# JinfengX/PointCloudPDF

Hardware: AMD Instinct MI355X
Metric: points/sec fwd+bwd (PT-v1 Seg50 + PDF U-decoder, 100k-pt scenes) (higher is better)
Workload: dtype f32

## Files before the change

include/pdfops.h:

```cpp
#ifndef PDFOPS_H
#define PDFOPS_H

#ifdef __cplusplus
extern "C" {
#endif

#define PDF_OK 0
#define PDF_ERR_BAD_ARG (-1)
#define PDF_ERR_NSAMPLE (-2)
#define PDF_ERR_UNSUPPORTED (-3)

#define PDF_ABI_VERSION 7
int pdf_abi_version(void);
const char *pdf_build_info(void);
int pdf_dist_fma_mode(void);
#define PDF_MMA_F32 0
#define PDF_MMA_F16 1
#define PDF_MMA_BF16 2

int pdf_knn_query(int m, int nsample, const float *xyz, const float *new_xyz,
                  const int *offset, const int *new_offset, int b,
                  int *idx, float *dist2, void *stream);

long pdf_knn_workspace_bytes(int b, int n, int m);
int pdf_knn_grid_supported(int nsample);
int pdf_knn_query_ws(int m, int nsample, int n, const float *xyz, const float *new_xyz, const int *offset,
                     const int *new_offset, int b, int *idx, float *dist2, void *workspace, long workspace_bytes,
                     void *stream);
int pdf_knn_grid_build(int n, const float *xyz, const int *offset, int b, void *workspace, long workspace_bytes, void *stream);
int pdf_knn_query_grid(int m, int nsample, int n, const float *xyz, const float *new_xyz, const int *offset, const int *new_offset, int b,
                       int *idx, float *dist2, void *workspace, long workspace_bytes, void *stream);
int pdf_knn_query_ws_counted(int m, int nsample, int n, const float *xyz, const float *new_xyz, const int *offset,
                             const int *new_offset, int b, int *idx, float *dist2, void *workspace, long workspace_bytes,
                             unsigned long long *pairs, void *stream);
int pdf_knn_query_list(int m, int nsample, const float *xyz, const float *new_xyz, const int *offset,
                       const int *new_offset, int b, int *idx, float *dist2, const int *qlist, const int *qcount,
                       void *stream);

int pdf_ball_query(int m, int nsample, float min_radius, float max_radius, const float *xyz, const float *new_xyz,
                   const int *offset, const int *new_offset, int b, int *idx, float *dist2, void *stream);

int pdf_random_ball_query(int m, int nsample, float min_radius, float max_radius, const int *order, const float *xyz,
                          const float *new_xyz, const int *offset, const int *new_offset, int b, int *idx, float *dist2,
                          void *stream);

int pdf_farthest_point_sampling(int b, int n, const float *xyz, const int *offset,
                                const int *new_offset, float *tmp, int *idx, void *stream);

int pdf_fps_reference_block_log2(int n);

long pdf_fps_workspace_bytes(int b, int n_total);
long pdf_fps_stats_offset(int b, int n_total);
int pdf_farthest_point_sampling_bucketed(int b, int n, int n_total, const float *xyz, const int *offset,
                                         const int *new_offset, void *workspace, long workspace_bytes,
                                         int *idx, void *stream);

int pdf_grouping_forward(int m, int nsample, int c, const float *input, const int *idx, float *output, void *stream);
int pdf_grouping_backward(int m, int nsample, int c, const float *grad_output, const int *idx, float *grad_input, void *stream);
int pdf_grouping_forward_ordered(int m, int nsample, int c, const float *input, const int *idx, const int *order, float *output, void *stream);
int pdf_group_forward_ordered(int m, int nsample, int c, int with_xyz, const float *feat, const float *xyz, const float *new_xyz,
                              const int *idx, const int *order, float *output, void *stream);
int pdf_interpolation_forward_ordered(int n, int c, int k, const float *input, const int *idx, const float *weight, const int *order,
                                      float *output, void *stream);
int pdf_subtraction_forward_ordered(int n, int nsample, int c, const float *input1, const float *input2, const int *idx, const int *order,
                                    float *output, void *stream);
int pdf_aggregation_forward_ordered(int n, int nsample, int c, int w_c, const float *input, const float *position, const float *weight,
                                    const int *idx, const int *order, float *output, void *stream);

int pdf_interpolation_forward(int n, int c, int k, const float *input, const int *idx, const float *weight, float *output, void *stream);
int pdf_interpolation_backward(int n, int c, int k, const float *grad_output, const int *idx, const float *weight, float *grad_input, void *stream);

int pdf_subtraction_forward(int n, int nsample, int c, const float *input1, const float *input2, const int *idx, float *output, void *stream);
int pdf_subtraction_backward(int n, int nsample, int c, const int *idx, const float *grad_output, float *grad_input1, float *grad_input2, void *stream);

int pdf_aggregation_forward(int n, int nsample, int c, int w_c, const float *input, const float *position,
                            const float *weight, const int *idx, float *output, void *stream);
int pdf_aggregation_backward(int n, int nsample, int c, int w_c, const float *input, const float *position,
                             const float *weight, const int *idx, const float *grad_output,
                             float *grad_input, float *grad_position, float *grad_weight, void *stream);

int pdf_attention_relation_step_forward(int m, int g, int c, const float *query, const float *key, const float *weight,
                                        const int *index_target, const int *index_refer, float *output, void *stream);
int pdf_attention_relation_step_backward(int m, int g, int c, const float *query, float *grad_query,
                                         const float *key, float *grad_key, const float *weight, float *grad_weight,
                                         const int *index_target, const int *index_refer, const float *grad_output, void *stream);
int pdf_attention_fusion_step_forward(int m, int g, int c, const float *weight, const float *value,
                                      const int *index_target, const int *index_refer, float *output, void *stream);
int pdf_attention_fusion_step_backward(int m, int g, int c, const float *weight, float *grad_weight,
                                       const float *value, float *grad_value,
                                       const int *index_target, const int *index_refer, const float *grad_output, void *stream);


int pdf_group_forward(int m, int nsample, int c, int with_xyz, const float *feat, const float *xyz,
                      const float *new_xyz, const int *idx, float *output, void *stream);
int pdf_group_backward(int m, int nsample, int c, int with_xyz, const float *grad_output, const int *idx,
                       float *grad_feat, void *stream);

int pdf_interpolation_weights(int n, int k, const float *dist2, float *weight, void *stream);

int pdf_pt_layer_supported(int nsample, int c);
long pdf_pt_layer_partial_floats(int n, int nsample, int c);
int pdf_pt_layer_forward(int n, int nsample, int c, const float *xq, const float *xk, const float *xv,
                         const float *p, const int *idx, const float *const *weights,
                         const float *const *bn_params, float *const *bn_buffers, int training, float eps,
                         float momentum, float *bn, float *saved, float *H, float *partial, float *out,
                         int storage_bf16, const int *order, void *stream);
int pdf_pt_layer_forward_m(int n, int nsample, int c, const float *xq, const float *xk, const float *xv,
                           const float *p, const int *idx, const float *const *weights,
                           const float *const *bn_params, float *const *bn_buffers, int training, float eps,
                           float momentum, float *bn, float *saved, float *H, float *partial, float *out,
                           int storage_bf16, const int *order, const double *moments, int *out_stat_rows, void *stream);

long pdf_pt_layer_bwd_partial_floats(int n, int nsample, int c);
long pdf_pt_layer_bwd_sums_floats(int c);
int pdf_pt_layer_backward(int n, int nsample, int c, const float *xq, const float *xk, const float *xv,
                          const float *p, const int *idx, const float *const *weights, const float *bn,
                          const float *saved, const float *H, const float *gout, float *gxq, float *gxk,
                          float *gxv, float *G2, float *G3, float *Wsm, float *GR, const int *inv_off, const int *inv_entry,
                          int entry_base, float *partial, float *sums, int storage_bf16, const int *order, const double *moments,
                          void *stream);

int pdf_bn_supported(int c);
long pdf_bn_partial_floats(long n, int c);
int pdf_bn_act_forward(long n, int c, const float *x, const float *res, const float *gamma, const float *beta,
                       float *running_mean, float *running_var, int training, float eps, float momentum, int relu,
                       float *coef, float *partial, float *y, void *stream);
int pdf_bn_act_backward(long n, int c, const float *gy, const float *x, const float *res, const float *coef,
                        int training, int relu, float *partial, float *sums, float *gx, float *gres, void *stream);
int pdf_bn_coef(long n, int c, const float *x, const float *gamma, const float *beta, float *running_mean,
                float *running_var, int training, float eps, float momentum, float *coef, float *partial, void *stream);
int pdf_bn_apply(long n, int c, const float *x, const float *res, const float *coef, int relu, float *y, void *stream);

long pdf_rowlin_partial_floats(long n, int o);
int pdf_rowlin_partial_rows(long n, int k, int o);
int pdf_rowlin_forward(long n, int k, int o, const float *x, long ldx, const float *w, int transpose_w,
                       const float *bias, const float *scale, const float *shift, int relu, float *y, long ldy,
                       int accumulate, float *partial, int mma_input, void *stream);
long pdf_rowlin_wgrad_ws_floats(long n, int k, int o, int ng);
int pdf_rowlin_wgrad(long n, int k, int o, const float *g, long ldg, const float *x, long ldx,
                     const float *scale, const float *shift, int relu, float *dw, float *db, float *ws, int mma_input, void *stream);
int pdf_bn_coef_from_partial(const float *partial, int rows, long n, int c, const float *gamma, const float *beta,
                             float *running_mean, float *running_var, float eps, float momentum, float *coef, void *stream);

int pdf_rowlin_multi(long n, int k, int o, int nin, int nout, const float *const *x, long ldx, const float *const *w,
                     int transpose_w, const float *const *bias, const float *scale, const float *shift, int relu,
                     float *const *y, long ldy, int accumulate, int mma_input, void *stream);
int pdf_rowlin_wgrad_multi(long n, int k, int o, int ng, const float *const *g, long ldg, const float *x, long ldx,
                           const float *scale, const float *shift, int relu, float *const *dw, float *const *db, float *ws, int mma_input, void *stream);
int pdf_rowlin_wgrad_group(long n, int k, int o, int ng, const float *const *g, long ldg, const float *const *x, long ldx,
                           const float *const *scale, const float *const *shift, const int *relu, float *const *dw,
                           float *const *db, float *ws, int mma_input, void *stream);

int pdf_kpconv_supported(int kp, int cin);
int pdf_kpconv_gather(int n, int m, int kp, int cin, const float *query, const float *support, const int *neighbors, const float *x,
                      const float *k_points, float extent, float *weighted, void *stream);
int pdf_kpconv_scatter(int n, int m, int kp, int cin, const float *query, const float *support, const int *neighbors,
                       const float *grad_weighted, const float *k_points, float extent, float *grad_x, void *stream);
int pdf_rowlin_dgrad_bstats(long n, int k, int o, int nin, const float *const *x, long ldx, const float *const *w, float *y, long ldy,
                            const float *bx, long ldb, const float *bcoef, int brelu, float *partial, int *partial_rows,
                            int mma_input, void *stream);
int pdf_rowlin_forward_bn(long n, int k, int o, const float *x, long ldx, const float *w, const float *bias, const float *scale,
                          const float *shift, int relu, float *y, long ldy, float *partial, const float *gamma, const float *beta,
                          float *running_mean, float *running_var, float eps, float momentum, float *coef, int mma_input, void *stream);
int pdf_bn_act_backward_presummed(long n, int c, const float *gy, const float *x, const float *coef, int training, int relu,
                                  const float *partial, int partial_rows, float *sums, float *gx, void *stream);

int pdf_bn_coef_eval_or_partial(const float *partial, int rows, long n, int c, const float *gamma, const float *beta,
                                float *running_mean, float *running_var, int training, float eps, float momentum,
                                float *coef, void *stream);
int pdf_block_pre_forward(long n, int c, void *const *p, int training, float eps, float momentum, int mma_input, void *stream);
int pdf_block_pre_backward(long n, int c, void *const *p, int training, int mma_input, void *stream);
int pdf_block_post_forward(long n, int c, void *const *p, int training, float eps, float momentum, int mma_input, void *stream);
int pdf_block_post_backward(long n, int c, void *const *p, int training, int mma_input, void *stream);
int pdf_bottleneck_forward(long n, int nsample, int c, void *const *p, int training, float eps, float momentum, int storage_bf16, int mma_input, void *stream);
int pdf_bottleneck_backward(long n, int nsample, int c, void *const *p, int training, int entry_base, int storage_bf16, int mma_input, void *stream);
int pdf_linbn_forward(long n, int k, int o, void *const *p, int training, int relu, float eps, float momentum, int mma_input, void *stream);
int pdf_linbn_backward(long n, int k, int o, void *const *p, int training, int relu, int mma_input, void *stream);

int pdf_rowlin_forward_roww(long n, int k, int o, const float *x, long ldx, const float *w, int transpose_w, float *y, long ldy,
                            int accumulate, const float *roww, long rws, int mma_input, void *stream);
int pdf_rowlin_wgrad_roww(long n, int k, int o, const float *g, long ldg, const float *x, long ldx, float *dw, const float *roww,
                          long rws, float *ws, int mma_input, void *stream);
int pdf_bn_bwd_sums(long n, int c, const float *gy, const float *x, const float *coef, int relu, float *partial, float *sums,
                    void *stream);

int pdf_td_supported(int nsample, int cin, int cout);
int pdf_td_tables(long m, int b, const float *p_src, const float *p_new, const int *idx, const int *new_offset, float *rel4, float *Z,
                  float *scene_sums, long n, const int *inv_off, const int *inv_entry, int entry_base,
                  void *stream);
long pdf_td_gram_floats(int cin);
long pdf_td_fwd_scratch_floats(long n, int cin);
long pdf_td_bwd_scratch_floats(long m, int cin, int cout);
int pdf_td_forward(long n, long m, int cin, int cout, void *const *p, int training, float eps, float momentum, int mma_input, void *stream);
int pdf_td_backward(long n, long m, int cin, int cout, void *const *p, int entry_base, int mma_input, void *stream);

int pdf_seg_sum_rows(long n, int c, const float *src, const int *inv_off, const int *inv_entry, int entry_base, float scale, float *out,
                     void *stream);
int pdf_seg_sum_rows_own(long n, int c, int nsample, const float *src, const int *inv_off, const int *inv_entry, int entry_base, float scale,
                         const int *order, float *out, float *out_own, void *stream);
int pdf_seg_sum_rows_strided(long n, int c, const float *src, long src_stride, const int *inv_off, const int *inv_entry, int entry_base,
                             float scale, float *out, void *stream);
int pdf_seg_sum_rows_x(long n, int c, const float *src, long src_stride, int src_bf16, const int *inv_off, const int *inv_entry, int entry_base,
                       float scale, float *out, void *stream);
int pdf_seg_sum_weighted_x(long n, int c, int nsample, int w_c, const float *src, const float *w, int w_bf16, const int *inv_off,
                           const int *inv_entry, int entry_base, const int *order, float *out, void *stream);
int pdf_seg_sum_weighted_ordered(long n, int c, int nsample, int w_c, const float *src, const float *w, const int *inv_off,
                                 const int *inv_entry, int entry_base, const int *order, float *out, void *stream);
int pdf_seg_sum_weighted(long n, int c, int nsample, int w_c, const float *src, const float *w, const int *inv_off, const int *inv_entry,
                         int entry_base, float *out, void *stream);

long pdf_ce_workspace_floats(void);
int pdf_ce_forward(long n, int c, const float *logits, const long *target, long ignore, float *grad, float *acc, float *loss,
                   void *stream);
int pdf_ce_backward(long n, int c, const float *dlogits, const float *acc, const float *gy, float *grad_out, void *stream);

long pdf_incr_kl_workspace_floats(void);
int pdf_incr_kl_forward(long n, int cs, int ct, const float *student, const float *teacher, const long *labels, long ignore, float inv_tp,
                        float inv_tt, float *grad, float *acc, float *loss, void *stream);
int pdf_incr_kl_backward(long n, int cs, const float *dgrad, const float *acc, const float *gy, float *grad_out, void *stream);

long pdf_knn_rel_moments_ws_doubles(int b, long m);
int pdf_knn_rel_moments(int b, long n, int nsample, const float *xyz, const int *offset, const int *idx, double *out, double *ws, void *stream);
int pdf_knn_rel_moments_q(int b, long m, int nsample, const float *xyz, const float *new_xyz, const int *new_offset, const int *idx,
                          double *out, double *ws, void *stream);

int pdf_scene_morton_keys(long n, int b, const float *xyz, const int *offset, float *bounds, long long *keys, void *stream);

int pdf_sgd_chunk(void);
int pdf_sgd_step(int nchunks, const void *tab, const int *chunks, float lr, float momentum, float weight_decay, const float *found_inf,
                 void *stream);
int pdf_grad_unscale(int nchunks, const void *tab, const int *chunks, const float *inv_scale, float *found_inf, void *stream);
int pdf_scaler_update(float *scale, float *inv_scale, int *growth_tracker, float *found_inf, float growth_factor, float backoff_factor,
                      int growth_interval, void *stream);
int pdf_adam_step(int nchunks, int ntensors, const void *tab, const int *chunks, double lr, double beta1, double beta2, double eps,
                  double weight_decay, int decoupled, const float *found_inf, void *stream);
int pdf_adam_grad_unscale(int nchunks, const void *tab, const int *chunks, const float *inv_scale, float *found_inf, void *stream);

int pdf_attention_step1_forward_v2(int N, int M, int h, int C, unsigned n_max, const float *q, const float *k,
                                   const int *index0_offsets, const int *index1, float *attn, void *stream);
int pdf_attention_step1_backward_v2(int N, int M, int h, int C, unsigned n_max, const float *grad_out, const int *index0_offsets,
                                    const int *index1, const float *q, const float *k, float *grad_q, float *grad_k, void *stream);
int pdf_dot_prod_with_idx_forward_v3(int N, int M, int h, int hdim, unsigned n_max, const float *q, const int *index_q_offsets,
                                     const float *k, const int *index_k, const float *table_q, const float *table_k,
                                     const int *rel_idx, float *output, void *stream);
int pdf_dot_prod_with_idx_backward_v3(int N, int M, int h, int hdim, unsigned n_max, const float *grad_out, const float *q,
                                      const int *index_q_offsets, const float *k, const int *index_k, const float *table_q,
                                      const float *table_k, const int *rel_idx, float *grad_q, float *grad_k, float *grad_table_q,
                                      float *grad_table_k, void *stream);
int pdf_attention_step2_with_rel_pos_value_forward_v2(int N, int M, int h, int hdim, unsigned n_max, const float *attn, const float *v,
                                                      const int *index0_offsets, const int *index1, const float *table,
                                                      const int *rel_idx, float *output, void *stream);
int pdf_attention_step2_with_rel_pos_value_backward_v2(int N, int M, int h, int hdim, unsigned n_max, const float *grad_out,
                                                       const int *index0_offsets, const int *index1, const float *attn, const float *v,
                                                       const float *table, const int *rel_idx, float *grad_attn, float *grad_v,
                                                       float *grad_table, void *stream);

int pdf_dot_prod_with_idx_forward_v3_l(int N, int M, int h, int hdim, int L, const float *q, const int *index_q_offsets, const float *k,
                                       const int *index_k, const float *table_q, const float *table_k, const int *rel_idx, float *output,
                                       void *stream);
int pdf_dot_prod_with_idx_backward_v3_l(int N, int M, int h, int hdim, int L, const float *grad_out, const float *q,
                                        const int *index_q_offsets, const float *k, const int *index_k, const float *table_q,
                                        const float *table_k, const int *rel_idx, float *grad_q, float *grad_k, float *grad_table_q,
                                        float *grad_table_k, void *stream);
int pdf_attention_step2_with_rel_pos_value_backward_v2_l(int N, int M, int h, int hdim, int L, const float *grad_out,
                                                         const int *index0_offsets, const int *index1, const float *attn, const float *v,
                                                         const float *table, const int *rel_idx, float *grad_attn, float *grad_v,
                                                         float *grad_table, void *stream);

int pdf_grid_hash(long n, int b, const float *coord, const int *offset, double gx, double gy, double gz, int f32,
                  const long long *min_grid, long long *grid, unsigned long long *key, void *stream);
int pdf_grid_hash_f64(long n, int b, const double *coord, const int *offset, double gx, double gy, double gz,
                      const long long *min_grid, long long *grid, unsigned long long *key, void *stream);

int pdf_philox4x64(long n, long key0, long key1, long ctr0, unsigned long long *out, void *stream);
int pdf_aug_bounds_workspace_doubles(int b);
int pdf_aug_bounds(int b, const long long *offset, const double *coord, const double *color, double *part, double *bounds, void *stream);
int pdf_aug_points(int b, long n, const long long *offset, int nop, const double *table, const double *bounds, const double *rec,
                   double *coord, double *color, double *normal, void *stream);
int pdf_aug_keys(int b, long n, const long long *offset, const unsigned long long *scene_keys, long stream_id, unsigned long long *out,
                 void *stream);
int pdf_aug_elastic_noise(int b, long total, const long long *vinfo, const unsigned long long *scene_keys, long stream_id, float *vol,
                          void *stream);
int pdf_aug_elastic_blur(int b, long total, const long long *vinfo, const float *in, float *out, int axis, void *stream);
int pdf_aug_elastic_apply(int b, long n, const long long *offset, const long long *vinfo, const double *axes, const float *vol,
                          const double *params, double magnitude, double *coord, double *disp, void *stream);

int pdf_vote_accumulate(long n, int c, const float *logits, const float *score, const long *index, float *pred,
                        float *score_sum, float *score_cnt, void *stream);

int pdf_radius_neighbors_self(int n, int nsample, float radius, const float *xyz, const int *offset, int b, int *idx, float *dist2,
                              void *workspace, long workspace_bytes, void *stream);

long pdf_graph_forest_workspace_bytes(long n, long E, long n_nodes);
int pdf_graph_forest(long n, int E, const long long *u, const long long *v, const float *w, const unsigned char *active,
                     const long long *nodes, int n_nodes, int *comp, unsigned char *chosen, void *workspace, long workspace_bytes,
                     void *stream);

int pdf_gmm2_1d(int m, const float *sorted_x, double *resp, double *out, int iters, double tol, double reg, void *stream);

int pdf_segment_softmax_forward(int N, int M, int h, const int *index0_offsets, const float *x, float *y, void *stream);
int pdf_segment_softmax_backward(int N, int M, int h, const int *index0_offsets, const float *y, const float *grad_y, float *grad_x,
                                 void *stream);

int pdf_wa_segment_rows(int N, int h, int d, int L, const int *seg_off, const int *seg_edge, const int *other, const int *rel,
                        const float *w, const float *X, long ldx, float xscale, const float *table, float *out, long ldo, float oscale, void *stream);
int pdf_wa_segment_rows_ordered(int N, int h, int d, int L, const int *seg_off, const int *seg_edge, const int *other, const int *rel,
                                const float *w, const float *X, long ldx, float xscale, const float *table, float *out, long ldo, float oscale,
                                const int *order, void *stream);
long pdf_wa_table_grad_ws_floats(int N, int h, int L);
int pdf_wa_table_grad(int N, int h, int d, int L, const int *seg_off, const int *seg_edge, const int *rel, const float *w,
                      const float *x, long ldx, float xscale, float *ws, float *grad_table, void *stream);
int pdf_wa_grad_attn(int N, int M, int h, int d, int L, const float *grad_out, long ldg, const int *offsets, const int *index1, const float *v,
                     long ldv, const float *table, const int *rel, float *grad_attn, void *stream);
int pdf_wa_logits_forward(int N, int M, int h, int d, int L, const float *q, const float *k, long ld, float qscale, const int *offsets,
                          const int *index1, const float *table_q, const float *table_k, const int *rel, float *out, void *stream);
int pdf_wa_permute_edges(int M, int h, const float *src, const int *edge, float *dst, void *stream);
int pdf_wa_logits_forward_ordered(int N, int M, int h, int d, int L, const float *q, const float *k, long ld, float qscale, const int *offsets,
                                  const int *index1, const float *table_q, const float *table_k, const int *rel, float *out, const int *order,
// ... 65 lines not shown
```

pointcloudpdf_amd/_native.py:

```python
import ctypes
import os
import threading

import torch

_HERE = os.path.dirname(os.path.abspath(__file__))
DIST_FMA = int(os.environ.get("PDFOPS_DIST_FMA", "0") or 0)
if DIST_FMA not in (0, 1, 2):
    raise RuntimeError(f"PDFOPS_DIST_FMA={DIST_FMA}: expected 0 (as written), 1 or 2 (csrc/pdfops_common.h)")


def library_path(dist_fma=0):
    return os.path.join(_HERE, "lib", "libpdfops.so" if not dist_fma else f"libpdfops_fma{int(dist_fma)}.so")


LIB_PATH = library_path(DIST_FMA)
ABI_VERSION = 7

c_int = ctypes.c_int
c_long = ctypes.c_long
c_void_p = ctypes.c_void_p
c_float = ctypes.c_float
c_double = ctypes.c_double

_PROTOS = {
    "knn_query": "iippppipp",
    "ball_query": "iiffppppipp",
    "random_ball_query": "iiffpppppipp",
    "farthest_point_sampling": "iippppp",
    "grouping_forward": "iiippp",
    "grouping_backward": "iiippp",
    "interpolation_forward": "iiipppp",
    "interpolation_backward": "iiipppp",
    "subtraction_forward": "iiipppp",
    "subtraction_backward": "iiipppp",
    "aggregation_forward": "iiiippppp",
    "aggregation_backward": "iiiipppppppp",
    "attention_relation_step_forward": "iiipppppp",
    "attention_relation_step_backward": "iiippppppppp",
    "attention_fusion_step_forward": "iiippppp",
    "attention_fusion_step_backward": "iiippppppp",
    "attention_step1_forward_v2": "iiiiippppp",
    "attention_step1_backward_v2": "iiiiippppppp",
    "dot_prod_with_idx_forward_v3": "iiiiipppppppp",
    "dot_prod_with_idx_backward_v3": "iiiiipppppppppppp",
    "attention_step2_with_rel_pos_value_forward_v2": "iiiiippppppp",
    "attention_step2_with_rel_pos_value_backward_v2": "iiiiipppppppppp",
    "segment_softmax_forward": "iiippp",
    "segment_softmax_backward": "iiipppp",
}
_HIP_ONLY_PROTOS = {
    "grid_hash": "lippdddippp",
    "grid_hash_f64": "lippdddppp",
    "philox4x64": "llllp",
    "aug_bounds": "ippppp",
    "aug_points": "ilpipppppp",
    "aug_keys": "ilpplp",
    "aug_elastic_noise": "ilpplp",
    "aug_elastic_blur": "ilpppi",
    "aug_elastic_apply": "ilpppppdpp",
    "radius_neighbors_self": "iifppipppl",
    "vote_accumulate": "lipppppp",
    "graph_forest": "lipppppipppl",
    "gmm2_1d": "ipppidd",
    "dot_prod_with_idx_forward_v3_l": "iiiiipppppppp",
    "dot_prod_with_idx_backward_v3_l": "iiiiipppppppppppp",
    "attention_step2_with_rel_pos_value_backward_v2_l": "iiiiipppppppppp",
    "scene_sum_rows": "ipiplip",
    "scene_repeat_rows": "iplipip",
    "region_stats": "ippppifppp",
    "region_seeds": "ippppip",
    "region_grow": "ippipppipiipppp",
    "region_edges": "ipppppippppppppppppl",
    "sort_floats_dev": "ipppppp",
    "gmm2_weak_dev": "ippppppppidd",
    "region_mask": "ippppppp",
    "region_tree": "ippipppppppp",
    "graph_forest_dev": "lipppppippppl",
    "gmm2_1d_dev": "ippppidd",
    "graph_forest_batch_dev": "ippippppppipppl",
    "wa_segment_rows": "iiiipppppplfpplf",
    "wa_segment_rows_ordered": "iiiipppppplfpplfp",
    "wa_table_grad": "iiiippppplfpp",
    "wa_grad_attn": "iiiiiplppplppp",
    "wa_logits_forward": "iiiiipplfpppppp",
    "wa_permute_edges": "iippp",
    "wa_logits_forward_ordered": "iiiiipplfppppppp",
    "wa_grad_attn_ordered": "iiiiiplppplpppp",
    "window_keys": "ippippfippp",
    "window_edges_count": "ippipppppp",
    "window_edges_fill": "ipppppppffipppp",
    "group_forward": "iiiippppp",
    "group_backward": "iiiippp",
    "interpolation_weights": "iipp",
    "farthest_point_sampling_bucketed": "iiipppplp",
    "grouping_forward_ordered": "iiipppp",
    "group_forward_ordered": "iiiipppppp",
    "interpolation_forward_ordered": "iiippppp",
    "subtraction_forward_ordered": "iiippppp",
    "aggregation_forward_ordered": "iiiipppppp",
    "seg_sum_rows": "lipppifp",
    "seg_sum_rows_strided": "liplppifp",
    "seg_sum_rows_own": "liipppifppp",
    "seg_sum_weighted": "liiippppip",
    "seg_sum_weighted_ordered": "liiippppipp",
}
_KIND = {"i": c_int, "l": c_long, "f": c_float, "d": c_double, "p": c_void_p}


class PdfOpsError(RuntimeError):
    pass


_RAW_STREAM = getattr(torch._C, "_cuda_getCurrentRawStream", None) if os.environ.get("PDFOPS_RAW_STREAM", "1") != "0" else None


def raw_stream():
    dev = torch.cuda.current_device()
    return _RAW_STREAM(dev) if _RAW_STREAM is not None else torch.cuda.current_stream().cuda_stream


def cu_masked_stream(first_cu, n_cus, device=None):
    if first_cu % 8 or n_cus % 8 or n_cus < 8:
        raise PdfOpsError("cu_masked_stream: first_cu and n_cus must be multiples of 8 (one CU of every XCD per step of 8)")
    dev = torch.cuda.current_device() if device is None else torch.device(device).index
    total = torch.cuda.get_device_properties(dev).multi_processor_count
    if first_cu + n_cus > total:
        raise PdfOpsError(f"cu_masked_stream: CUs [{first_cu}, {first_cu + n_cus}) of {total}")
    hip = ctypes.CDLL("libamdhip64.so")
    words = (total + 31) // 32
    mask = (ctypes.c_uint32 * words)()
    for cu in range(first_cu, first_cu + n_cus):
        mask[cu // 32] |= 1 << (cu % 32)
    handle = ctypes.c_void_p()
    with torch.cuda.device(dev):
        rc = hip.hipExtStreamCreateWithCUMask(ctypes.byref(handle), ctypes.c_uint32(words), mask)
    if rc != 0:
        raise PdfOpsError(f"hipExtStreamCreateWithCUMask failed with status {rc}")
    return torch.cuda.ExternalStream(handle.value, device=torch.device("cuda", dev))


def require_current_device(*tensors):
    cur = None
    for t in tensors:
        if t is None or not t.is_cuda:
            continue
        if cur is None:
            cur = torch.cuda.current_device()
        if t.device.index != cur:
            raise PdfOpsError(f"pointcloudpdf_amd: tensor on {t.device} but the current device is cuda:{cur}; call "
                              "torch.cuda.set_device(...) or wrap the call in torch.cuda.device(...)")


_INV = "_pdf_inverse"


def attach_inverse(idx, n, table):
    setattr(idx, _INV, (idx.data_ptr(), idx._version, int(n), table))
    return table


def inverse_table(idx, n):
    cached = getattr(idx, _INV, None)
    if cached is not None and cached[0] == idx.data_ptr() and cached[1] == idx._version and cached[2] == int(n):
        return cached[3]
    flat = idx.reshape(-1)
    vals, perm = torch.sort(flat, stable=True)
    off = torch.searchsorted(vals, torch.arange(int(n) + 1, device=idx.device, dtype=vals.dtype), out_int32=True)
    return attach_inverse(idx, n, (off, perm.to(torch.int32), 0))

# ... 349 lines not shown

    def attention_step2_with_rel_pos_value_v2_backward(self, grad_out, attn, v, offsets, n_max, index1, table, rel_idx):
        _check(grad_out, torch.float32, "grad_output")
        m, h = attn.shape
        n, _, d = v.shape
        ga = self._new(v, (m, h), torch.float32, zero=True)
        gv = self._new(v, (n, h, d), torch.float32, zero=True)
        gt = self._new(v, tuple(table.shape), torch.float32, zero=True)
        name, x = (("attention_step2_with_rel_pos_value_backward_v2_l", int(table.shape[0])) if self.use_stream
                   else ("attention_step2_with_rel_pos_value_backward_v2", int(n_max)))
        self._call(name, n, m, h, d, x, grad_out, offsets, index1, attn, v, table, rel_idx, ga, gv, gt)
        return ga, gv, gt


    def segment_softmax(self, x, offsets):
        _check(x, torch.float32, "src"); _check(offsets, torch.int32, "index0_offsets")
        m, h = x.shape
        if h > 64:
            raise ValueError("segment_softmax: at most 64 heads")
        y = self._new(x, (m, h), torch.float32)
        self._call("segment_softmax_forward", offsets.shape[0] - 1, m, h, offsets, x, y)
        return y

    def segment_softmax_backward(self, y, grad_y, offsets):
        _check(grad_y, torch.float32, "grad_output")
        m, h = y.shape
        gx = self._new(y, (m, h), torch.float32)
        self._call("segment_softmax_backward", offsets.shape[0] - 1, m, h, offsets, y, grad_y, gx)
        return gx


class HipBackend(CBackend):

    overwrites_outputs = True

    def __init__(self, lib):
        super().__init__(lib, "pdf_", "cuda", True, extra_protos=tuple(_HIP_ONLY_PROTOS))
        lib.pdf_fps_workspace_bytes.restype = c_long
        lib.pdf_fps_workspace_bytes.argtypes = [c_int, c_int]
        lib.pdf_wa_table_grad_ws_floats.restype = c_long
        lib.pdf_wa_table_grad_ws_floats.argtypes = [c_int, c_int, c_int]
        lib.pdf_layernorm_supported.restype = c_int
        lib.pdf_layernorm_supported.argtypes = [c_int]
        lib.pdf_layernorm_partial_floats.restype = c_long
        lib.pdf_layernorm_partial_floats.argtypes = [c_long, c_int]
        lib.pdf_layernorm_forward.restype = c_int
        lib.pdf_layernorm_forward.argtypes = [c_long, c_int, c_void_p, c_void_p, c_void_p, ctypes.c_float, c_void_p, c_void_p, c_void_p, c_void_p]
        lib.pdf_layernorm_backward.restype = c_int
        lib.pdf_layernorm_backward.argtypes = [c_long, c_int] + [c_void_p] * 10
        lib.pdf_fps_stats_offset.restype = c_long
        lib.pdf_fps_stats_offset.argtypes = [c_int, c_int]
        self.collect_fps_stats = False
        self.last_fps_stats = None
        lib.pdf_aug_bounds_workspace_doubles.restype = c_int
        lib.pdf_aug_bounds_workspace_doubles.argtypes = [c_int]
        lib.pdf_abi_version.restype = c_int
        lib.pdf_build_info.restype = ctypes.c_char_p
        got = int(lib.pdf_abi_version())
        if got != ABI_VERSION:
            raise PdfOpsError(f"libpdfops ABI {got} != {ABI_VERSION} expected by pointcloudpdf_amd/_native.py (include/pdfops.h: PDF_ABI_VERSION): "
                              "stale library -- rebuild with `python -m pointcloudpdf_amd.build --force`")
        for nm in ("pre_forward", "post_forward"):
            f = getattr(lib, "pdf_block_" + nm)
            f.restype = c_int
            f.argtypes = [c_long, c_int, c_void_p, c_int, ctypes.c_float, ctypes.c_float, c_int, c_void_p]
        lib.pdf_td_tables.restype = c_int
        lib.pdf_td_tables.argtypes = [c_long, c_int, c_void_p, c_void_p, c_void_p, c_void_p, c_void_p, c_void_p, c_void_p, c_long, c_void_p, c_void_p,
                                      c_int, c_void_p]
        lib.pdf_td_supported.restype = c_int
        lib.pdf_td_supported.argtypes = [c_int, c_int, c_int]
        lib.pdf_td_gram_floats.restype = c_long
        lib.pdf_td_gram_floats.argtypes = [c_int]
        lib.pdf_td_fwd_scratch_floats.restype = c_long
        lib.pdf_td_fwd_scratch_floats.argtypes = [c_long, c_int]
        lib.pdf_td_bwd_scratch_floats.restype = c_long
        lib.pdf_td_bwd_scratch_floats.argtypes = [c_long, c_int, c_int]
        lib.pdf_td_forward.restype = c_int
        lib.pdf_td_forward.argtypes = [c_long, c_long, c_int, c_int, c_void_p, c_int, ctypes.c_float, ctypes.c_float, c_int, c_void_p]
        lib.pdf_td_backward.restype = c_int
        lib.pdf_td_backward.argtypes = [c_long, c_long, c_int, c_int, c_void_p, c_int, c_int, c_void_p]
        lib.pdf_ce_workspace_floats.restype = c_long
        lib.pdf_ce_workspace_floats.argtypes = []
        lib.pdf_ce_forward.restype = c_int
        lib.pdf_ce_forward.argtypes = [c_long, c_int, c_void_p, c_void_p, c_long, c_void_p, c_void_p, c_void_p, c_void_p]
        lib.pdf_ce_backward.restype = c_int
        lib.pdf_ce_backward.argtypes = [c_long, c_int, c_void_p, c_void_p, c_void_p, c_void_p, c_void_p]
        lib.pdf_incr_kl_workspace_floats.restype = c_long
        lib.pdf_incr_kl_workspace_floats.argtypes = []
        lib.pdf_incr_kl_forward.restype = c_int
        lib.pdf_incr_kl_forward.argtypes = [c_long, c_int, c_int, c_void_p, c_void_p, c_void_p, c_long, ctypes.c_float, ctypes.c_float,
                                            c_void_p, c_void_p, c_void_p, c_void_p]
        lib.pdf_incr_kl_backward.restype = c_int
        lib.pdf_incr_kl_backward.argtypes = [c_long, c_int, c_void_p, c_void_p, c_void_p, c_void_p, c_void_p]
        lib.pdf_knn_rel_moments.restype = c_int
        lib.pdf_knn_rel_moments.argtypes = [c_int, c_long, c_int, c_void_p, c_void_p, c_void_p, c_void_p, c_void_p, c_void_p]
        lib.pdf_knn_rel_moments_ws_doubles.restype = c_long
        lib.pdf_knn_rel_moments_ws_doubles.argtypes = [c_int, c_long]
        lib.pdf_knn_rel_moments_q.restype = c_int
        lib.pdf_knn_rel_moments_q.argtypes = [c_int, c_long, c_int, c_void_p, c_void_p, c_void_p, c_void_p, c_void_p, c_void_p, c_void_p]
        class CopySeg(ctypes.Structure):
            _fields_ = [("src", c_void_p), ("dst", c_void_p), ("nbytes", c_long), ("src_offset", c_void_p), ("sub", c_void_p),
                        ("sub_const", c_int), ("src_elems", c_int)]

        self.CopySeg = CopySeg
        lib.pdf_stage_copy.restype = c_int
        lib.pdf_stage_copy.argtypes = [c_int, c_void_p, c_void_p]
        lib.pdf_scene_morton_keys.restype = c_int
        lib.pdf_scene_morton_keys.argtypes = [c_long, c_int, c_void_p, c_void_p, c_void_p, c_void_p, c_void_p]
        lib.pdf_sgd_chunk.restype = c_int
        lib.pdf_sgd_chunk.argtypes = []
        lib.pdf_sgd_step.restype = c_int
        lib.pdf_sgd_step.argtypes = [c_int, c_void_p, c_void_p, ctypes.c_float, ctypes.c_float, ctypes.c_float, c_void_p, c_void_p]
        lib.pdf_grad_unscale.restype = c_int
        lib.pdf_grad_unscale.argtypes = [c_int, c_void_p, c_void_p, c_void_p, c_void_p, c_void_p]
        lib.pdf_scaler_update.restype = c_int
        lib.pdf_scaler_update.argtypes = [c_void_p, c_void_p, c_void_p, c_void_p, ctypes.c_float, ctypes.c_float, c_int, c_void_p]
        lib.pdf_adam_step.restype = c_int
        lib.pdf_adam_step.argtypes = [c_int, c_int, c_void_p, c_void_p, ctypes.c_double, ctypes.c_double, ctypes.c_double, ctypes.c_double,
                                      ctypes.c_double, c_int, c_void_p, c_void_p]
        lib.pdf_adam_grad_unscale.restype = c_int
        lib.pdf_adam_grad_unscale.argtypes = [c_int, c_void_p, c_void_p, c_void_p, c_void_p, c_void_p]
        lib.pdf_linbn_forward.restype = c_int
        lib.pdf_linbn_forward.argtypes = [c_long, c_int, c_int, c_void_p, c_int, c_int, ctypes.c_float, ctypes.c_float, c_int, c_void_p]
        lib.pdf_linbn_backward.restype = c_int
        lib.pdf_linbn_backward.argtypes = [c_long, c_int, c_int, c_void_p, c_int, c_int, c_int, c_void_p]
        lib.pdf_bottleneck_forward.restype = c_int
        lib.pdf_bottleneck_forward.argtypes = [c_long, c_int, c_int, c_void_p, c_int, ctypes.c_float, ctypes.c_float, c_int, c_int, c_void_p]
        lib.pdf_bottleneck_backward.restype = c_int
        lib.pdf_bottleneck_backward.argtypes = [c_long, c_int, c_int, c_void_p, c_int, c_int, c_int, c_int, c_void_p]
        for nm in ("pre_backward", "post_backward"):
            f = getattr(lib, "pdf_block_" + nm)
            f.restype = c_int
            f.argtypes = [c_long, c_int, c_void_p, c_int, c_int, c_void_p]
        lib.pdf_rowlin_multi.restype = c_int
        lib.pdf_rowlin_multi.argtypes = [c_long, c_int, c_int, c_int, c_int, c_void_p, c_long, c_void_p, c_int, c_void_p, c_void_p, c_void_p,
                                         c_int, c_void_p, c_long, c_int, c_int, c_void_p]
        lib.pdf_kpconv_supported.restype = c_int
        lib.pdf_kpconv_supported.argtypes = [c_int, c_int]
        for nm in ("pdf_kpconv_gather", "pdf_kpconv_scatter"):
            f = getattr(lib, nm)
            f.restype = c_int
            f.argtypes = [c_int, c_int, c_int, c_int, c_void_p, c_void_p, c_void_p, c_void_p, c_void_p, ctypes.c_float, c_void_p, c_void_p]
        lib.pdf_rowlin_wgrad_group.restype = c_int
        lib.pdf_rowlin_wgrad_group.argtypes = [c_long, c_int, c_int, c_int, c_void_p, c_long, c_void_p, c_long, c_void_p, c_void_p, c_void_p,
                                               c_void_p, c_void_p, c_void_p, c_int, c_void_p]
        lib.pdf_rowlin_wgrad_multi.restype = c_int
        lib.pdf_rowlin_wgrad_multi.argtypes = [c_long, c_int, c_int, c_int, c_void_p, c_long, c_void_p, c_long, c_void_p, c_void_p, c_int,
                                               c_void_p, c_void_p, c_void_p, c_int, c_void_p]
        lib.pdf_rowlin_wgrad_ws_floats.restype = c_long
        lib.pdf_rowlin_wgrad_ws_floats.argtypes = [c_long, c_int, c_int, c_int]
        lib.pdf_rowlin_dgrad_bstats.restype = c_int
        lib.pdf_rowlin_dgrad_bstats.argtypes = [c_long, c_int, c_int, c_int, c_void_p, c_long, c_void_p, c_void_p, c_long, c_void_p, c_long,
                                                c_void_p, c_int, c_void_p, ctypes.POINTER(c_int), c_int, c_void_p]
        lib.pdf_bn_act_backward_presummed.restype = c_int
        lib.pdf_bn_act_backward_presummed.argtypes = [c_long, c_int, c_void_p, c_void_p, c_void_p, c_int, c_int, c_void_p, c_int, c_void_p,
                                                      c_void_p, c_void_p]
        lib.pdf_rowlin_partial_floats.restype = c_long
        lib.pdf_rowlin_partial_floats.argtypes = [c_long, c_int]
        lib.pdf_rowlin_partial_rows.restype = c_int
        lib.pdf_rowlin_partial_rows.argtypes = [c_long, c_int, c_int]
        lib.pdf_rowlin_forward.restype = c_int
        lib.pdf_rowlin_forward.argtypes = [c_long, c_int, c_int, c_void_p, c_long, c_void_p, c_int, c_void_p, c_void_p, c_void_p,
                                           c_int, c_void_p, c_long, c_int, c_void_p, c_int, c_void_p]
        lib.pdf_rowlin_wgrad.restype = c_int
        lib.pdf_rowlin_wgrad.argtypes = [c_long, c_int, c_int, c_void_p, c_long, c_void_p, c_long, c_void_p, c_void_p, c_int,
                                         c_void_p, c_void_p, c_void_p, c_int, c_void_p]
        lib.pdf_bn_coef_from_partial.restype = c_int
        lib.pdf_bn_coef_from_partial.argtypes = [c_void_p, c_int, c_long, c_int, c_void_p, c_void_p, c_void_p, c_void_p,
                                                 ctypes.c_float, ctypes.c_float, c_void_p, c_void_p]
        lib.pdf_bn_coef.restype = c_int
        lib.pdf_bn_coef.argtypes = [c_long, c_int, c_void_p, c_void_p, c_void_p, c_void_p, c_void_p, c_int, ctypes.c_float,
                                    ctypes.c_float, c_void_p, c_void_p, c_void_p]
        lib.pdf_bn_apply.restype = c_int
        lib.pdf_bn_apply.argtypes = [c_long, c_int, c_void_p, c_void_p, c_void_p, c_int, c_void_p, c_void_p]
        lib.pdf_bn_supported.restype = c_int
        lib.pdf_bn_supported.argtypes = [c_int]
        lib.pdf_bn_partial_floats.restype = c_long
        lib.pdf_bn_partial_floats.argtypes = [c_long, c_int]
        lib.pdf_bn_act_forward.restype = c_int
        lib.pdf_bn_act_forward.argtypes = [c_long, c_int] + [c_void_p] * 6 + [c_int, ctypes.c_float, ctypes.c_float, c_int] + [c_void_p] * 4
        lib.pdf_bn_act_backward.restype = c_int
        lib.pdf_bn_act_backward.argtypes = [c_long, c_int] + [c_void_p] * 4 + [c_int, c_int] + [c_void_p] * 5
        lib.pdf_pt_layer_supported.restype = c_int
        lib.pdf_pt_layer_supported.argtypes = [c_int, c_int]
        for fn in (lib.pdf_pt_layer_partial_floats, lib.pdf_pt_layer_bwd_partial_floats):
            fn.restype = c_long
            fn.argtypes = [c_int, c_int, c_int]
        lib.pdf_pt_layer_bwd_sums_floats.restype = c_long
        lib.pdf_pt_layer_bwd_sums_floats.argtypes = [c_int]
        lib.pdf_pt_layer_forward.restype = c_int
        lib.pdf_pt_layer_forward.argtypes = [c_int, c_int, c_int] + [c_void_p] * 8 + [c_int, ctypes.c_float, ctypes.c_float] + [c_void_p] * 5 + [c_int, c_void_p, c_void_p]
        lib.pdf_knn_grid_build.restype = c_int
        lib.pdf_knn_grid_build.argtypes = [c_int, c_void_p, c_void_p, c_int, c_void_p, c_long, c_void_p]
        lib.pdf_knn_query_grid.restype = c_int
        lib.pdf_knn_query_grid.argtypes = [c_int, c_int, c_int, c_void_p, c_void_p, c_void_p, c_void_p, c_int, c_void_p, c_void_p, c_void_p, c_long, c_void_p]
        lib.pdf_pt_layer_backward.restype = c_int
        lib.pdf_pt_layer_backward.argtypes = [c_int, c_int, c_int] + [c_void_p] * 19 + [c_int] + [c_void_p] * 2 + [c_int, c_void_p, c_void_p, c_void_p]
        self.fps_mode = os.environ.get("PDFOPS_FPS", "bucketed")
        self.knn_mode = os.environ.get("PDFOPS_KNN", "grid")
        lib.pdf_knn_workspace_bytes.restype = c_long
        lib.pdf_knn_workspace_bytes.argtypes = [c_int, c_int, c_int]
        lib.pdf_graph_forest_workspace_bytes.restype = c_long
        lib.pdf_region_grow_list_points.restype = c_long
        lib.pdf_region_grow_list_points.argtypes = []
        lib.pdf_graph_forest_workspace_bytes.argtypes = [c_long, c_long, c_long]
        lib.pdf_knn_grid_supported.restype = c_int
        lib.pdf_knn_grid_supported.argtypes = [c_int]
        lib.pdf_knn_query_ws.restype = c_int
        lib.pdf_knn_query_ws.argtypes = [c_int, c_int, c_int] + [c_void_p] * 4 + [c_int] + [c_void_p] * 3 + [c_long, c_void_p]
        lib.pdf_knn_query_ws_counted.restype = c_int
        lib.pdf_knn_query_ws_counted.argtypes = [c_int, c_int, c_int] + [c_void_p] * 4 + [c_int] + [c_void_p] * 3 + [c_long, c_void_p, c_void_p]

    KNN_GRID_MAX_SCENES = 64
    use_inverse = os.environ.get("PDFOPS_INVERSE", "1") != "0"
    storage_bf16 = os.environ.get("PDFOPS_STORAGE", "f32") == "bf16"

    def set_storage(self, kind):
        if kind not in ("f32", "bf16"):
            raise ValueError("storage: 'f32' or 'bf16'")
        self.storage_bf16 = kind == "bf16"

    def grouping_forward(self, input, idx):
        _check(input, torch.float32, "input"); _check(idx, torch.int32, "idx")
        m, ns = idx.shape
        c = input.shape[1]
        out = self._new(input, (m, ns, c), torch.float32)
        self._call("grouping_forward_ordered", m, ns, c, input, idx, order_of(idx), out)
        return out

    def interpolation_forward(self, input, idx, weight):
        _check(input, torch.float32, "input"); _check(idx, torch.int32, "idx"); _check(weight, torch.float32, "weight")
        n, k = idx.shape
        c = input.shape[1]
        out = self._new(input, (n, c), torch.float32)
        self._call("interpolation_forward_ordered", n, c, k, input, idx, weight, order_of(idx), out)
        return out

    def subtraction_forward(self, input1, input2, idx):
        _check(input1, torch.float32, "input1"); _check(input2, torch.float32, "input2"); _check(idx, torch.int32, "idx")
        n, c = input1.shape
        ns = idx.shape[-1]
        out = self._new(input1, (n, ns, c), torch.float32)
        self._call("subtraction_forward_ordered", n, ns, c, input1, input2, idx, order_of(idx), out)
        return out

    def aggregation_forward(self, input, position, weight, idx):
        for t, nm in ((input, "input"), (position, "position"), (weight, "weight")):
            _check(t, torch.float32, nm)
        _check(idx, torch.int32, "idx")
        n, ns, c = position.shape
        out = self._new(input, (n, c), torch.float32)
        self._call("aggregation_forward_ordered", n, ns, c, weight.shape[-1], input, position, weight, idx, order_of(idx), out)
        return out

    def grouping_backward(self, grad_output, idx, n):
        if not self.use_inverse:
            return super().grouping_backward(grad_output, idx, n)
        _check(grad_output, torch.float32, "grad_output"); _check(idx, torch.int32, "idx")
        m, ns, c = grad_output.shape
        if grad_output.numel() == 0 or n == 0:
            return self._new(grad_output, (n, c), torch.float32, zero=True)
        off, ent, base = inverse_table(idx, n)
        gi = self._new(grad_output, (n, c), torch.float32)
        self._call("seg_sum_rows", n, c, grad_output, off, ent, base, 1.0, gi)
        return gi

    def interpolation_backward(self, grad_output, idx, weight, m):
        if not self.use_inverse:
            return super().interpolation_backward(grad_output, idx, weight, m)
        _check(grad_output, torch.float32, "grad_output"); _check(idx, torch.int32, "idx"); _check(weight, torch.float32, "weight")
        n, c = grad_output.shape
        if grad_output.numel() == 0 or m == 0:
            return self._new(grad_output, (m, c), torch.float32, zero=True)
        off, ent, base = inverse_table(idx, m)
        gi = self._new(grad_output, (m, c), torch.float32)
        self._call("seg_sum_weighted_ordered", m, c, idx.shape[1], 1, grad_output, weight, off, ent, base, src_order_of(idx, m), gi)
        return gi

    def subtraction_backward(self, idx, grad_output, n2=None):
        if not self.use_inverse:
            return super().subtraction_backward(idx, grad_output, n2)
        _check(grad_output, torch.float32, "grad_output"); _check(idx, torch.int32, "idx")
        n, ns, c = grad_output.shape
        n2 = n if n2 is None else n2
        if grad_output.numel() == 0 or n2 == 0:
            return super().subtraction_backward(idx, grad_output, n2)
        off, ent, base = inverse_table(idx, n2)
        g2 = self._new(grad_output, (n2, c), torch.float32)
        if n == n2 and c % 4 == 0 and self.fuse_own_rows:
            g1 = self._new(grad_output, (n, c), torch.float32)
            self._call("seg_sum_rows_own", n2, c, ns, grad_output, off, ent, base, -1.0, src_order_of(idx, n2), g2, g1)
            return g1, g2
        g1 = self._new(grad_output, (n, c), torch.float32, zero=True)
        self._call("subtraction_backward", n, ns, c, idx, grad_output, g1, None)
        self._call("seg_sum_rows", n2, c, grad_output, off, ent, base, -1.0, g2)
        return g1, g2

    fuse_own_rows = os.environ.get("PDFOPS_FUSE_OWN_ROWS", "1") != "0"

    def aggregation_backward(self, input, position, weight, idx, grad_output):
        if not self.use_inverse:
            return super().aggregation_backward(input, position, weight, idx, grad_output)
        _check(grad_output, torch.float32, "grad_output")
        n, ns, c = position.shape
        w_c = weight.shape[-1]
        if position.numel() == 0 or input.shape[0] == 0:
# ... 284 lines not shown
        count = torch.empty(n, **i32)
        seg = torch.empty((n, 4), **i32)
        self._call("window_edges_count", n, kf_sorted, kf, m, kcd_sorted, kc, wk, wkd, count, seg)
        offsets = torch.zeros(n + 1, **i32)
        torch.cumsum(count, 0, dtype=torch.int32, out=offsets[1:])
        e, n_max = (int(v) for v in torch.stack([offsets[-1], count.max() if n else offsets[-1]]).tolist())
        index0 = torch.empty(e, dtype=torch.int64, device=dev)
        index1 = torch.empty(e, **i32)
        rel = torch.empty((e, 3), **i32)
        flag = torch.zeros(1, **i32)
        order32 = order_f.int()
        self._call("window_edges_fill", n, offsets, seg, order32, order_cd.int(), wk, wkd, xyz.contiguous(), float(c2w), float(qs), int(vmax),
                   index0, index1, rel, flag)
        setattr(offsets, _WORDER, (offsets.data_ptr(), offsets._version, order32))
        return index0, index1, offsets, n_max, rel, flag

    def window_logits_supported(self, q, k, table_q):
        return self.wa_atomic_free and q.shape[0] == k.shape[0] and self._wa_ok(q.shape[2], int(table_q.shape[0]), q, k)

    def window_logits(self, q, k, index1, offsets, table_q, table_k, rel_idx):
        n, h, d = q.shape
        m = index1.shape[0]
        out = torch.empty((m, h), dtype=torch.float32, device=q.device)
        self._call("wa_logits_forward", n, m, h, d, int(table_q.shape[0]), q, k, h * d, 1.0, offsets, index1, table_q, table_k, rel_idx, out)
        return out

    def window_logits_backward(self, g, q, k, index1, offsets, table_q, table_k, rel_idx):
        n, h, d = q.shape
        L = int(table_q.shape[0])
        key_off, key_edge, key_q, key_rel = window_csc(index1, offsets, rel_idx, n_keys=n)
        g_key = self._wa_permute(g, key_edge)
        gq, gk = torch.empty_like(q), torch.empty_like(k)
        self._wa_rows(n, h, d, L, offsets, None, index1, rel_idx, g, k, table_q, gq)
        self._wa_rows(n, h, d, L, key_off, None, key_q, key_rel, g_key, q, table_k, gk)
        gtq = self._wa_table_grad(n, h, d, L, offsets, None, rel_idx, g, q, q)
        gtk = self._wa_table_grad(n, h, d, L, key_off, None, key_rel, g_key, k, q)
        return gq, gk, gtq, gtk

    def attention_step2_with_rel_pos_value_v2_backward(self, grad_out, attn, v, offsets, n_max, index1, table, rel_idx):
        m, h = attn.shape
        n, _, d = v.shape
        L = int(table.shape[0])
        if m == 0 or offsets.shape[0] != n + 1 or not self._wa_ok(d, L, v, grad_out):
            return super().attention_step2_with_rel_pos_value_v2_backward(grad_out, attn, v, offsets, n_max, index1, table, rel_idx)
        _check(grad_out, torch.float32, "grad_output")
        c = h * d
        key_off, key_edge, key_q = window_csc(index1, offsets, n_keys=n)
        ga = torch.empty((m, h), dtype=torch.float32, device=v.device)
        gv = torch.empty_like(v)
        self._call("wa_grad_attn", n, m, h, d, L, grad_out, c, offsets, index1, v, c, table, rel_idx, ga)
        self._wa_rows(n, h, d, 0, key_off, key_edge, key_q, None, attn, grad_out, None, gv)
        gt = self._wa_table_grad(n, h, d, L, offsets, None, rel_idx, attn, grad_out, v)
        return ga, gv, gt

    wa_core = os.environ.get("PDFOPS_WA_CORE", "1") != "0"

    def window_attention_core_supported(self, qkv, table_q, table_k, table_v):
        L, h, d, _ = table_q.shape
        return (self.wa_core and self.wa_atomic_free and qkv.dim() == 2 and qkv.shape[1] == 3 * h * d and table_k.shape == table_q.shape == table_v.shape
                and qkv.dtype == torch.float32 and qkv.is_contiguous() and self._wa_ok(d, L, qkv) and (h * d) % 4 == 0)

    def window_attention_core(self, qkv, index1, offsets, table_q, table_k, table_v, rel_idx, scale):
        n = qkv.shape[0]
        L, h, d, _ = table_q.shape
        c, m = h * d, index1.shape[0]
        q, k, v = qkv[:, :c], qkv[:, c:2 * c], qkv[:, 2 * c:]
        logits = torch.empty((m, h), dtype=torch.float32, device=qkv.device)
        self._call("wa_logits_forward_ordered", n, m, h, d, L, q, k, 3 * c, float(scale), offsets, index1, table_q, table_k, rel_idx, logits,
                   self._wa_order(offsets))
        attn = self.segment_softmax(logits, offsets)
        out = torch.empty((n, c), dtype=torch.float32, device=qkv.device)
        self._wa_rows(n, h, d, L, offsets, None, index1, rel_idx, attn, v, table_v, out, ldx=3 * c, order=self._wa_order(offsets))
        return out, attn

    def window_attention_core_backward(self, go, qkv, attn, index1, offsets, table_q, table_k, table_v, rel_idx, scale):
        n = qkv.shape[0]
        L, h, d, _ = table_q.shape
        c, m = h * d, index1.shape[0]
        q, k, v = qkv[:, :c], qkv[:, c:2 * c], qkv[:, 2 * c:]
        key_off, key_edge, key_q, key_rel = window_csc(index1, offsets, rel_idx, n_keys=n)
        gqkv = torch.empty_like(qkv)
        ga = torch.empty((m, h), dtype=torch.float32, device=qkv.device)
        order = self._wa_order(offsets)
        self._call("wa_grad_attn_ordered", n, m, h, d, L, go, c, offsets, index1, v, 3 * c, table_v, rel_idx, ga, order)
        attn_key = self._wa_permute(attn, key_edge)
        korder = window_key_order(index1) if self.wa_window_order else None
        self._wa_rows(n, h, d, 0, key_off, None, key_q, None, attn_key, go, None, gqkv[:, 2 * c:], ldo=3 * c, order=korder)
        gtv = self._wa_table_grad(n, h, d, L, offsets, None, rel_idx, attn, go, qkv)
        g = self.segment_softmax_backward(attn, ga, offsets)
        g_key = self._wa_permute(g, key_edge)
        self._wa_rows(n, h, d, L, offsets, None, index1, rel_idx, g, k, table_q, gqkv[:, :c], ldx=3 * c, ldo=3 * c, oscale=scale, order=order)
        self._wa_rows(n, h, d, L, key_off, None, key_q, key_rel, g_key, q, table_k, gqkv[:, c:2 * c], ldx=3 * c, xscale=scale, ldo=3 * c, order=korder)
        gtq = self._wa_table_grad(n, h, d, L, offsets, None, rel_idx, g, q, qkv, ldx=3 * c, xscale=scale)
        gtk = self._wa_table_grad(n, h, d, L, key_off, None, key_rel, g_key, k, qkv, ldx=3 * c)
        return gqkv, gtq, gtk, gtv

    def _stream(self):
        return c_void_p(raw_stream())

    def rowlin(self, x, w, bias=None, coef=None, relu=False, transpose_w=False, out=None, accumulate=False, stats=False):
        n, k = x.shape
        o = w.shape[1] if transpose_w else w.shape[0]
        y = out if out is not None else torch.empty((n, o), dtype=torch.float32, device=x.device)
        partial = None
        if stats:
            partial = torch.empty((int(self.lib.pdf_rowlin_partial_floats(n, o)),), dtype=torch.float32, device=x.device)
            partial._pdf_rows = int(self.lib.pdf_rowlin_partial_rows(n, k, o))
        rc = self.lib.pdf_rowlin_forward(n, k, o, x.data_ptr(), x.stride(0), w.data_ptr(), int(transpose_w),
                                         None if bias is None else bias.data_ptr(),
                                         None if coef is None else coef.data_ptr(),
                                         None if coef is None else coef.data_ptr() + 4 * k, int(relu), y.data_ptr(), y.stride(0),
                                         int(accumulate), None if partial is None else partial.data_ptr(), current_mma_input(), self._stream())
        if rc != 0:
            raise PdfOpsError(f"pdf_rowlin_forward failed with status {rc}")
        return y, partial

    @staticmethod
    def _ptrs(tensors, n=3):
        return (c_void_p * n)(*[t.data_ptr() if t is not None else None for t in list(tensors) + [None] * (n - len(tensors))])

    def rowlin_multi(self, xs, ws, biases=None, coef=None, relu=False, transpose_w=False, nout=1):
        n, k = xs[0].shape
        o = ws[0].shape[1] if transpose_w else ws[0].shape[0]
        ys = [torch.empty((n, o), dtype=torch.float32, device=xs[0].device) for _ in range(nout)]
        rc = self.lib.pdf_rowlin_multi(n, k, o, len(xs), nout, self._ptrs(xs), xs[0].stride(0), self._ptrs(ws), int(transpose_w),
                                       None if biases is None else self._ptrs(biases),
                                       None if coef is None else coef.data_ptr(), None if coef is None else coef.data_ptr() + 4 * k,
                                       int(relu), self._ptrs(ys), o, 0, current_mma_input(), self._stream())
        if rc != 0:
            raise PdfOpsError(f"pdf_rowlin_multi failed with status {rc}")
        return ys

    def rowlin_dgrad_bn_backward(self, gs, ws, bx, coef, training=True, relu=True):
        n, k = gs[0].shape
        o = ws[0].shape[1]
        require_current_device(bx, *gs)
        dy = self._new(bx, (n, o), torch.float32)
        partial = self._new(bx, (int(self.lib.pdf_rowlin_partial_floats(n, o)),), torch.float32)
        rows = c_int(0)
        sums = self._new(bx, (2 * o,), torch.float32)
        rc = self.lib.pdf_rowlin_dgrad_bstats(n, k, o, len(gs), self._ptrs(gs), gs[0].stride(0), self._ptrs(ws), dy.data_ptr(), o,
                                              bx.data_ptr(), bx.stride(0), coef.data_ptr(), int(bool(relu)), partial.data_ptr(),
                                              ctypes.byref(rows), current_mma_input(), self._stream())
        if rc == -3:
            return None
        if rc != 0:
            raise PdfOpsError(f"pdf_rowlin_dgrad_bstats failed with status {rc}")
        rc = self.lib.pdf_bn_act_backward_presummed(n, o, dy.data_ptr(), bx.data_ptr(), coef.data_ptr(), int(bool(training)), int(bool(relu)),
                                                    partial.data_ptr(), rows.value, sums.data_ptr(), dy.data_ptr(), self._stream())
        if rc != 0:
            raise PdfOpsError(f"pdf_bn_act_backward_presummed failed with status {rc}")
        return dy, sums[o:], sums[:o]

    def wgrad_workspace(self, n, k, o, ng, device):
        return torch.empty((max(int(self.lib.pdf_rowlin_wgrad_ws_floats(int(n), int(k), int(o), int(ng))), 1),), dtype=torch.float32, device=device)

    def rowlin_wgrad_multi(self, gs, x, coef, relu):
        n, o = gs[0].shape
        k = x.shape[1]
        dws = [torch.empty((o, k), dtype=torch.float32, device=x.device) for _ in gs]
        dbs = [torch.empty((o,), dtype=torch.float32, device=x.device) for _ in gs]
        ws = self.wgrad_workspace(n, k, o, len(gs), x.device)
        rc = self.lib.pdf_rowlin_wgrad_multi(n, k, o, len(gs), self._ptrs(gs), gs[0].stride(0), x.data_ptr(), x.stride(0),
                                             None if coef is None else coef.data_ptr(), None if coef is None else coef.data_ptr() + 4 * k,
                                             int(relu), self._ptrs(dws), self._ptrs(dbs), ws.data_ptr(), current_mma_input(), self._stream())
        if rc != 0:
            raise PdfOpsError(f"pdf_rowlin_wgrad_multi failed with status {rc}")
        return dws, dbs

    def kpconv_supported(self, kp, cin):
        return bool(self.lib.pdf_kpconv_supported(int(kp), int(cin)))

    def kpconv_gather(self, query, support, neighbors, x, k_points, extent):
        n, m = neighbors.shape
        kp, cin = k_points.shape[0], x.shape[1]
        out = torch.empty((n, kp * cin), dtype=torch.float32, device=x.device)
        rc = self.lib.pdf_kpconv_gather(n, m, kp, cin, query.data_ptr(), support.data_ptr(), neighbors.data_ptr(), x.data_ptr(),
                                        k_points.data_ptr(), ctypes.c_float(extent), out.data_ptr(), self._stream())
        if rc != 0:
            raise PdfOpsError(f"pdf_kpconv_gather failed with status {rc}")
        return out

    def kpconv_scatter(self, query, support, neighbors, grad_weighted, k_points, extent, rows, cin):
        n, m = neighbors.shape
        gx = torch.zeros((rows, cin), dtype=torch.float32, device=grad_weighted.device)
        rc = self.lib.pdf_kpconv_scatter(n, m, k_points.shape[0], cin, query.data_ptr(), support.data_ptr(), neighbors.data_ptr(),
                                         grad_weighted.data_ptr(), k_points.data_ptr(), ctypes.c_float(extent), gx.data_ptr(), self._stream())
        if rc != 0:
            raise PdfOpsError(f"pdf_kpconv_scatter failed with status {rc}")
        return gx

    def rowlin_wgrad_group(self, gs, xs, coefs, relus, need_bias):
        n, o = gs[0].shape
        k = xs[0].shape[1]
        dev = gs[0].device
        dws = [torch.empty((o, k), dtype=torch.float32, device=dev) for _ in gs]
        dbs = [torch.empty((o,), dtype=torch.float32, device=dev) if nb else None for nb in need_bias]
        ws = self.wgrad_workspace(n, k, o, len(gs), dev)
        P = lambda ts: (c_void_p * len(ts))(*[None if t is None else (t if isinstance(t, int) else t.data_ptr()) for t in ts])
        sc = [None if cf is None else cf.data_ptr() for cf in coefs]
        sh = [None if cf is None else cf.data_ptr() + 4 * k for cf in coefs]
        rc = self.lib.pdf_rowlin_wgrad_group(n, k, o, len(gs), P(gs), gs[0].stride(0), P(xs), xs[0].stride(0), P(sc), P(sh),
                                             (c_int * len(gs))(*[int(bool(r)) for r in relus]), P(dws), P(dbs), ws.data_ptr(), current_mma_input(), self._stream())
        if rc == -3:
            return None
        if rc != 0:
            raise PdfOpsError(f"pdf_rowlin_wgrad_group failed with status {rc}")
        return dws, dbs

    def rowlin_wgrad(self, g, x, coef, relu, need_bias):
        n, o = g.shape
        k = x.shape[1]
        dw = torch.empty((o, k), dtype=torch.float32, device=x.device)
        db = torch.empty((o,), dtype=torch.float32, device=x.device) if need_bias else None
        ws = self.wgrad_workspace(n, k, o, 1, x.device)
        rc = self.lib.pdf_rowlin_wgrad(n, k, o, g.data_ptr(), g.stride(0), x.data_ptr(), x.stride(0),
                                       None if coef is None else coef.data_ptr(),
                                       None if coef is None else coef.data_ptr() + 4 * k, int(relu), dw.data_ptr(),
                                       None if db is None else db.data_ptr(), ws.data_ptr(), current_mma_input(), self._stream())
        if rc != 0:
            raise PdfOpsError(f"pdf_rowlin_wgrad failed with status {rc}")
        return dw, db

    def bn_coef_from_partial(self, partial, n, c, bn, training):
        coef = torch.empty((4 * c,), dtype=torch.float32, device=partial.device if partial is not None else bn.weight.device)
        if training:
            rows = partial._pdf_rows
            rc = self.lib.pdf_bn_coef_from_partial(partial.data_ptr(), rows, n, c, bn.weight.data_ptr(), bn.bias.data_ptr(),
                                                   bn.running_mean.data_ptr(), bn.running_var.data_ptr(), ctypes.c_float(bn.eps),
                                                   ctypes.c_float(bn.momentum),
                                                   coef.data_ptr(), self._stream())
            if rc != 0:
                raise PdfOpsError(f"pdf_bn_coef_from_partial failed with status {rc}")
        else:
            rstd = torch.rsqrt(bn.running_var + bn.eps)
            sc = bn.weight.detach() * rstd
            coef = torch.cat([sc, bn.bias.detach() - bn.running_mean * sc, bn.running_mean, rstd])
        return coef

    def bn_coef(self, x, bn, training):
        n, c = x.shape
        coef = torch.empty((4 * c,), dtype=torch.float32, device=x.device)
        partial = torch.empty((int(self.lib.pdf_bn_partial_floats(n, c)),), dtype=torch.float32, device=x.device) if training else None
        rc = self.lib.pdf_bn_coef(n, c, x.data_ptr(), bn.weight.data_ptr(), bn.bias.data_ptr(), bn.running_mean.data_ptr(),
                                  bn.running_var.data_ptr(), int(bool(training)), ctypes.c_float(bn.eps),
                                  ctypes.c_float(bn.momentum), coef.data_ptr(),
                                  None if partial is None else partial.data_ptr(), self._stream())
        if rc != 0:
            raise PdfOpsError(f"pdf_bn_coef failed with status {rc}")
        return coef

    def bn_apply(self, x, res, coef, relu):
        n, c = x.shape
        y = torch.empty_like(x)
        rc = self.lib.pdf_bn_apply(n, c, x.data_ptr(), None if res is None else res.data_ptr(), coef.data_ptr(), int(relu),
                                   y.data_ptr(), self._stream())
        if rc != 0:
            raise PdfOpsError(f"pdf_bn_apply failed with status {rc}")
        return y

    def td_tables(self, p_src, p_new, idx, new_offset, inverse=None):
        m, n, b = p_new.shape[0], p_src.shape[0], new_offset.shape[0]
        rel4 = torch.empty((m, 16, 4), dtype=torch.float32, device=p_src.device)
        Z = torch.zeros((n, 32), dtype=torch.float32, device=p_src.device)
        sums = torch.zeros((b, 16), dtype=torch.float32, device=p_src.device)
        off, ent, base = inverse if inverse is not None else (None, None, 0)
        rc = self.lib.pdf_td_tables(m, b, p_src.data_ptr(), p_new.data_ptr(), idx.data_ptr(), new_offset.data_ptr(), rel4.data_ptr(), Z.data_ptr(),
                                    sums.data_ptr(), n, None if off is None else off.data_ptr(), None if ent is None else ent.data_ptr(), int(base),
                                    self._stream())
        if rc != 0:
            raise PdfOpsError(f"pdf_td_tables failed with status {rc}")
        return rel4, Z, sums

    def bottleneck_forward(self, n, k, c, ptrs, training, eps, momentum, storage_bf16=0):
        rc = self.lib.pdf_bottleneck_forward(n, k, c, (c_void_p * len(ptrs))(*ptrs), int(training), ctypes.c_float(eps),
                                             ctypes.c_float(momentum), self.layer_flags(storage_bf16), current_mma_input(), self._stream())
        if rc != 0:
            raise PdfOpsError(f"pdf_bottleneck_forward failed with status {rc}")

    def bottleneck_backward(self, n, k, c, ptrs, training, entry_base=0, storage_bf16=0):
        rc = self.lib.pdf_bottleneck_backward(n, k, c, (c_void_p * len(ptrs))(*ptrs), int(training), int(entry_base), self.layer_flags(storage_bf16), current_mma_input(), self._stream())
        if rc != 0:
            raise PdfOpsError(f"pdf_bottleneck_backward failed with status {rc}")

    def _ptable(self, tensors):
        return (c_void_p * len(tensors))(*[None if t is None else t.data_ptr() for t in tensors])

    def block_call(self, name, n, c, tensors, training, eps=None, momentum=None):
        fn = getattr(self.lib, "pdf_block_" + name)
        if eps is None:
            rc = fn(n, c, self._ptable(tensors), int(bool(training)), current_mma_input(), self._stream())
        else:
            rc = fn(n, c, self._ptable(tensors), int(bool(training)), ctypes.c_float(eps), ctypes.c_float(momentum), current_mma_input(), self._stream())
        if rc != 0:
            raise PdfOpsError(f"pdf_block_{name} failed with status {rc}")

    def bn_supported(self, c):
        return bool(self.lib.pdf_bn_supported(int(c)))

    def bn_act_forward(self, x, res, gamma, beta, running_mean, running_var, training, eps, momentum, relu):
        n, c = x.shape
        require_current_device(x, res, gamma)
        coef = self._new(x, (4 * c,), torch.float32)
        partial = self._new(x, (int(self.lib.pdf_bn_partial_floats(n, c)),), torch.float32)
        y = self._new(x, (n, c), torch.float32)
        P = lambda t: None if t is None else self._ptr(t)
# ... 278 lines not shown
```

pointcloudpdf_amd/csrc/block.hip:

```cpp
#include "pdfops_common.h"

namespace {
struct Err {
    int rc = 0;
    Err &operator<<(int r) { if (rc == 0 && r != 0) rc = r; return *this; }
};

}

extern "C" int pdf_bn_coef_eval_or_partial(const float *partial, int rows, long n, int c, const float *gamma, const float *beta,
                                           float *running_mean, float *running_var, int training, float eps, float momentum,
                                           float *coef, void *stream) {
    if (training) return pdf_bn_coef_from_partial(partial, rows, n, c, gamma, beta, running_mean, running_var, eps, momentum, coef, stream);
    return pdf_bn_coef(n, c, nullptr, gamma, beta, running_mean, running_var, 0, eps, momentum, coef, nullptr, stream);
}

extern "C" int pdf_block_pre_forward(long n, int c, void *const *p, int training, float eps, float momentum, int mma_input, void *stream) {
    if (n < 1 || !p) return PDF_ERR_BAD_ARG;
    if (!pdf_bn_supported(c)) return PDF_ERR_UNSUPPORTED;
    const float *x = (const float *)p[0], *W1 = (const float *)p[1], *g1 = (const float *)p[2], *b1 = (const float *)p[3];
    float *rm1 = (float *)p[4], *rv1 = (float *)p[5];
    float *z1 = (float *)p[12], *coef1 = (float *)p[13], *partial = (float *)p[17];
    Err e;
    if (training) {
        e << pdf_rowlin_forward_bn(n, c, c, x, c, W1, nullptr, nullptr, nullptr, 0, z1, c, partial, g1, b1, rm1, rv1, eps, momentum, coef1, mma_input, stream);
    } else {
        e << pdf_rowlin_forward(n, c, c, x, c, W1, 0, nullptr, nullptr, nullptr, 0, z1, c, 0, nullptr, mma_input, stream);
        e << pdf_bn_coef_eval_or_partial(partial, 0, n, c, g1, b1, rm1, rv1, 0, eps, momentum, coef1, stream);
    }
    const float *xs[1] = {z1}, *ws[3] = {(const float *)p[6], (const float *)p[8], (const float *)p[10]};
    const float *bs[3] = {(const float *)p[7], (const float *)p[9], (const float *)p[11]};
    float *ys[3] = {(float *)p[14], (float *)p[15], (float *)p[16]};
    e << pdf_rowlin_multi(n, c, c, 1, 3, xs, c, ws, 0, bs, coef1, coef1 + c, 1, ys, c, 0, mma_input, stream);
    return e.rc;
}

static bool inkernel_bn() {
    static const bool on = [] { const char *v = getenv("PDFOPS_INKERNEL_BN"); return !(v && v[0] == '0'); }();
    return on;
}
static bool dgrad_bstats() {
    static const bool on = [] { const char *v = getenv("PDFOPS_DGRAD_BSTATS"); return !(v && v[0] == '0'); }();
    return on;
}

static int block_pre_backward(long n, int c, void *const *p, int training, int accumulate_gx, int mma_input, void *stream, bool defer_wgrad = false) {
    if (n < 1 || !p || !p[14]) return PDF_ERR_BAD_ARG;
    const float *x = (const float *)p[0], *z1 = (const float *)p[1], *coef1 = (const float *)p[2], *W1 = (const float *)p[3];
    float *gx = (float *)p[10], *grads = (float *)p[11], *dy = (float *)p[12], *partial = (float *)p[13], *wslab = (float *)p[14];
    const long cc = (long)c * c;
    float *dW1 = grads, *db1 = grads + cc, *dqkv = db1 + 2 * c;
    Err e;
    const float *gs[3] = {(const float *)p[7], (const float *)p[8], (const float *)p[9]};
    const float *ws[3] = {(const float *)p[4], (const float *)p[5], (const float *)p[6]};
    float *dws[3] = {dqkv, dqkv + (cc + c), dqkv + 2 * (cc + c)}, *dbs[3] = {dqkv + cc, dqkv + (cc + c) + cc, dqkv + 2 * (cc + c) + cc};
    float *ys[1] = {dy};
    if (!defer_wgrad) e << pdf_rowlin_wgrad_multi(n, c, c, 3, gs, c, z1, c, coef1, coef1 + c, 1, dws, dbs, wslab, mma_input, stream);
    int prow = 0;
    const int rc1 = dgrad_bstats() ? pdf_rowlin_dgrad_bstats(n, c, c, 3, gs, c, ws, dy, c, z1, c, coef1, 1, partial, &prow, mma_input, stream) : PDF_ERR_UNSUPPORTED;
    if (rc1 == PDF_ERR_UNSUPPORTED) {
        e << pdf_rowlin_multi(n, c, c, 3, 1, gs, c, ws, 1, nullptr, nullptr, nullptr, 0, ys, c, 0, mma_input, stream);
        e << pdf_bn_act_backward(n, c, dy, z1, nullptr, coef1, training, 1, partial, db1, dy, nullptr, stream);
    } else {
        e << rc1;
        e << pdf_bn_act_backward_presummed(n, c, dy, z1, coef1, training, 1, partial, prow, db1, dy, stream);
    }
    if (!defer_wgrad) e << pdf_rowlin_wgrad(n, c, c, dy, c, x, c, nullptr, nullptr, 0, dW1, nullptr, wslab, mma_input, stream);
    e << pdf_rowlin_forward(n, c, c, dy, c, W1, 1, nullptr, nullptr, nullptr, 0, gx, c, accumulate_gx, nullptr, mma_input, stream);
    return e.rc;
}

extern "C" int pdf_block_pre_backward(long n, int c, void *const *p, int training, int mma_input, void *stream) {
    return block_pre_backward(n, c, p, training, 0, mma_input, stream, false);
}

static int block_post_forward(long n, int c, void *const *p, int training, float eps, float momentum, int t_stat_rows, int mma_input, void *stream) {
    if (n < 1 || !p) return PDF_ERR_BAD_ARG;
    if (!pdf_bn_supported(c)) return PDF_ERR_UNSUPPORTED;
    const float *t = (const float *)p[0], *x = (const float *)p[1];
    float *coef2 = (float *)p[11], *z3 = (float *)p[12], *coef3 = (float *)p[13], *y = (float *)p[14], *partial = (float *)p[15];
    Err e;
    if (training && t_stat_rows > 0)
        e << pdf_bn_coef_from_partial(partial, t_stat_rows, n, c, (const float *)p[2], (const float *)p[3], (float *)p[4], (float *)p[5], eps, momentum, coef2, stream);
    else
        e << pdf_bn_coef(n, c, t, (const float *)p[2], (const float *)p[3], (float *)p[4], (float *)p[5], training, eps, momentum, coef2, partial, stream);
    bool applied = false;
    if (training && inkernel_bn()) {
        int rows = 0;
        const int rc = pdf_rowlin_forward_stats_ho(n, c, c, t, c, (const float *)p[6], nullptr, coef2, coef2 + c, 1, z3, c, partial + PDF_HO_FLOATS, partial,
                                                   &rows, mma_input, stream);
        if (rc == PDF_OK) {
            e << pdf_bn_apply_rows(n, c, z3, x, partial + PDF_HO_FLOATS, rows, (const float *)p[7], (const float *)p[8], (float *)p[9], (float *)p[10], eps,
                                   momentum, coef3, partial, 1, y, stream);
            applied = true;
        } else if (rc != PDF_ERR_UNSUPPORTED) {
            e << rc;
        }
    }
    if (applied) return e.rc;
    if (training) {
        e << pdf_rowlin_forward_bn(n, c, c, t, c, (const float *)p[6], nullptr, coef2, coef2 + c, 1, z3, c, partial, (const float *)p[7], (const float *)p[8],
                                   (float *)p[9], (float *)p[10], eps, momentum, coef3, mma_input, stream);
    } else {
        e << pdf_rowlin_forward(n, c, c, t, c, (const float *)p[6], 0, nullptr, coef2, coef2 + c, 1, z3, c, 0, nullptr, mma_input, stream);
        e << pdf_bn_coef_eval_or_partial(partial, 0, n, c, (const float *)p[7], (const float *)p[8], (float *)p[9], (float *)p[10], 0, eps, momentum, coef3, stream);
    }
    e << pdf_bn_apply(n, c, z3, x, coef3, 1, y, stream);
    return e.rc;
}
extern "C" int pdf_block_post_forward(long n, int c, void *const *p, int training, float eps, float momentum, int mma_input, void *stream) {
    return block_post_forward(n, c, p, training, eps, momentum, 0, mma_input, stream);
}

static int block_post_backward(long n, int c, void *const *p, int training, int mma_input, void *stream, bool defer_wgrad = false) {
    if (n < 1 || !p || !p[12]) return PDF_ERR_BAD_ARG;
    const float *gy = (const float *)p[0], *t = (const float *)p[1], *x = (const float *)p[2], *z3 = (const float *)p[3];
    const float *coef2 = (const float *)p[4], *coef3 = (const float *)p[5], *W3 = (const float *)p[6];
    float *gt = (float *)p[7], *gres = (float *)p[8], *grads = (float *)p[9], *da = (float *)p[10], *partial = (float *)p[11];
    const long cc = (long)c * c;
    float *dW3 = grads, *db2 = grads + cc, *db3 = db2 + 2 * c;
    Err e;
    e << pdf_bn_act_backward(n, c, gy, z3, x, coef3, training, 1, partial, db3, da, gres, stream);
    if (!defer_wgrad) e << pdf_rowlin_wgrad(n, c, c, da, c, t, c, coef2, coef2 + c, 1, dW3, nullptr, (float *)p[12], mma_input, stream);
    int prow = 0;
    const float *das[1] = {da}, *w3s[1] = {W3};
    const int rc2 = dgrad_bstats() ? pdf_rowlin_dgrad_bstats(n, c, c, 1, das, c, w3s, gt, c, t, c, coef2, 1, partial, &prow, mma_input, stream) : PDF_ERR_UNSUPPORTED;
    if (rc2 == PDF_ERR_UNSUPPORTED) {
        e << pdf_rowlin_forward(n, c, c, da, c, W3, 1, nullptr, nullptr, nullptr, 0, gt, c, 0, nullptr, mma_input, stream);
        e << pdf_bn_act_backward(n, c, gt, t, nullptr, coef2, training, 1, partial, db2, gt, nullptr, stream);
    } else {
        e << rc2;
        e << pdf_bn_act_backward_presummed(n, c, gt, t, coef2, training, 1, partial, prow, db2, gt, stream);
    }
    return e.rc;
}

extern "C" int pdf_block_post_backward(long n, int c, void *const *p, int training, int mma_input, void *stream) {
    return block_post_backward(n, c, p, training, mma_input, stream, false);
}

extern "C" int pdf_bottleneck_forward(long n, int nsample, int c, void *const *p, int training, float eps, float momentum, int storage_bf16, int mma_input, void *stream) {
    if (n < 1 || !p) return PDF_ERR_BAD_ARG;
    Err e;
    void *pre[18] = {p[0], p[1], p[2], p[3], p[4], p[5], p[6], p[7], p[8], p[9], p[10], p[11], p[43], p[44], p[45], p[46], p[47], p[56]};
    e << pdf_block_pre_forward(n, c, pre, training, eps, momentum, mma_input, stream);
    const float *weights[8], *bn_params[6];
    float *bn_buffers[6];
    for (int i = 0; i < 8; ++i) weights[i] = (const float *)p[14 + i];
    for (int i = 0; i < 6; ++i) { bn_params[i] = (const float *)p[22 + i]; bn_buffers[i] = (float *)p[28 + i]; }
    static const bool p4_stats = [] { const char *v = getenv("PDFOPS_P4_STATS"); return !(v && v[0] == '0'); }();
    int t_rows = 0;
    e << pdf_pt_layer_forward_m((int)n, nsample, c, (const float *)p[45], (const float *)p[46], (const float *)p[47], (const float *)p[12],
                                (const int *)p[13], weights, bn_params, bn_buffers, training, eps, momentum, (float *)p[48], (float *)p[49],
                                (float *)p[50], (float *)p[56], (float *)p[51], storage_bf16, (const int *)p[57], (const double *)p[58],
                                p4_stats ? &t_rows : nullptr, stream);
    void *post[16] = {p[51], p[0], p[34], p[35], p[36], p[37], p[38], p[39], p[40], p[41], p[42], p[52], p[53], p[54], p[55], p[56]};
    e << block_post_forward(n, c, post, training, eps, momentum, e.rc == 0 ? t_rows : 0, mma_input, stream);
    return e.rc;
}

extern "C" int pdf_bottleneck_backward(long n, int nsample, int c, void *const *p, int training, int entry_base, int storage_bf16, int mma_input, void *stream) {
    if (n < 1 || !p) return PDF_ERR_BAD_ARG;
    Err e;
    if (!p[50]) return PDF_ERR_BAD_ARG;
    static const bool group = [] { const char *v = getenv("PDFOPS_WGRAD_GROUP"); return !(v && v[0] == '0'); }();
    float *ws_post = (float *)p[50], *ws_pre = ws_post + pdf_rowlin_wgrad_ws_floats(n, c, c, 1);
    void *post[13] = {p[0], p[24], p[1], p[25], p[26], p[27], p[28], p[33], p[29], p[31], p[34], p[40], ws_post};
    e << block_post_backward(n, c, post, training, mma_input, stream, group);
    const float *weights[8];
    for (int i = 0; i < 8; ++i) weights[i] = (const float *)p[10 + i];
    e << pdf_pt_layer_backward((int)n, nsample, c, (const float *)p[21], (const float *)p[22], (const float *)p[23], (const float *)p[8],
                               (const int *)p[9], weights, (const float *)p[18], (const float *)p[19], (const float *)p[20],
                               (const float *)p[33], (float *)p[35], (float *)p[36], (float *)p[37], (float *)p[38], (float *)p[39],
                               (float *)p[41], (float *)p[42], (const int *)p[43], (const int *)p[44], entry_base,
                               (float *)p[40], (float *)p[32], storage_bf16, (const int *)p[49], (const double *)p[46], stream);
    void *pre[15] = {p[1], p[2], p[3], p[4], p[5], p[6], p[7], p[35], p[36], p[37], p[29], p[30], p[45], p[40], ws_pre};
    e << block_pre_backward(n, c, pre, training, 1, mma_input, stream, group);
    if (group && e.rc == 0) {
        const long cc = (long)c * c;
        float *gpre = (float *)p[30], *gpost = (float *)p[31];
        float *dW1 = gpre, *dqkv = gpre + cc + 2 * c, *dW3 = gpost;
        const float *coef1 = (const float *)p[3], *coef2 = (const float *)p[26];
        const float *g[5] = {(const float *)p[34], (const float *)p[35], (const float *)p[36], (const float *)p[37], (const float *)p[45]};
        const float *x[5] = {(const float *)p[24], (const float *)p[2], (const float *)p[2], (const float *)p[2], (const float *)p[1]};
        const float *sc[5] = {coef2, coef1, coef1, coef1, nullptr}, *sh[5] = {coef2 + c, coef1 + c, coef1 + c, coef1 + c, nullptr};
        const int relu[5] = {1, 1, 1, 1, 0};
        float *dw[5] = {dW3, dqkv, dqkv + (cc + c), dqkv + 2 * (cc + c), dW1};
        float *db[5] = {nullptr, dqkv + cc, dqkv + (cc + c) + cc, dqkv + 2 * (cc + c) + cc, nullptr};
        const int rc = pdf_rowlin_wgrad_group(n, c, c, 5, g, c, x, c, sc, sh, relu, dw, db, ws_post, mma_input, stream);
        if (rc == PDF_ERR_UNSUPPORTED) {
            e << pdf_rowlin_wgrad(n, c, c, g[0], c, x[0], c, sc[0], sh[0], 1, dw[0], nullptr, ws_post, mma_input, stream);
            e << pdf_rowlin_wgrad_multi(n, c, c, 3, g + 1, c, x[1], c, sc[1], sh[1], 1, dw + 1, db + 1, ws_pre, mma_input, stream);
            e << pdf_rowlin_wgrad(n, c, c, g[4], c, x[4], c, nullptr, nullptr, 0, dw[4], nullptr, ws_pre, mma_input, stream);
        } else {
            e << rc;
        }
    }
    return e.rc;
}

extern "C" int pdf_linbn_forward(long n, int k, int o, void *const *p, int training, int relu, float eps, float momentum, int mma_input, void *stream) {
    if (n < 1 || !p) return PDF_ERR_BAD_ARG;
    if (!pdf_bn_supported(o)) return PDF_ERR_UNSUPPORTED;
    Err e;
    float *z = (float *)p[7], *coef = (float *)p[8], *partial = (float *)p[10];
    if (training) {
        e << pdf_rowlin_forward_bn(n, k, o, (const float *)p[0], k, (const float *)p[1], (const float *)p[2], nullptr, nullptr, 0, z, o, partial,
                                   (const float *)p[3], (const float *)p[4], (float *)p[5], (float *)p[6], eps, momentum, coef, mma_input, stream);
    } else {
        e << pdf_rowlin_forward(n, k, o, (const float *)p[0], k, (const float *)p[1], 0, (const float *)p[2], nullptr, nullptr, 0, z, o, 0, nullptr, mma_input, stream);
        e << pdf_bn_coef_eval_or_partial(partial, 0, n, o, (const float *)p[3], (const float *)p[4], (float *)p[5], (float *)p[6], 0, eps, momentum, coef, stream);
    }
    e << pdf_bn_apply(n, o, z, nullptr, coef, relu, (float *)p[9], stream);
    return e.rc;
}

extern "C" int pdf_linbn_backward(long n, int k, int o, void *const *p, int training, int relu, int mma_input, void *stream) {
    if (n < 1 || !p || !p[9]) return PDF_ERR_BAD_ARG;
    float *grads = (float *)p[6], *gz = (float *)p[7];
    const long ok = (long)o * k;
    Err e;
    e << pdf_bn_act_backward(n, o, (const float *)p[0], (const float *)p[2], nullptr, (const float *)p[3], training, relu, (float *)p[8],
                             grads + ok + o, gz, nullptr, stream);
    if (p[5]) e << pdf_rowlin_forward(n, o, k, gz, o, (const float *)p[4], 1, nullptr, nullptr, nullptr, 0, (float *)p[5], k, 0, nullptr, mma_input, stream);
    e << pdf_rowlin_wgrad(n, k, o, gz, o, (const float *)p[1], k, nullptr, nullptr, 0, grads, grads + ok, (float *)p[9], mma_input, stream);
    return e.rc;
}
```

pointcloudpdf_amd/csrc/pdfops_common.h:

```cpp
#pragma once
#include <hip/hip_runtime.h>
#include <stdint.h>
#include <atomic>
#include "../../include/pdfops.h"

#define PDF_WAVE 64
#define PDF_MAX_DEVICES_LDS 64

static inline int pdf_launch_status() {
    hipError_t e = hipGetLastError();
    return e == hipSuccess ? PDF_OK : (int)e;
}

struct PdfLdsLimit { std::atomic<int> state[PDF_MAX_DEVICES_LDS]; };
static inline bool pdf_lds_limit_raised(PdfLdsLimit &site, const void *kernel, int bytes) {
    int dev = 0;
    if (hipGetDevice(&dev) != hipSuccess || dev < 0 || dev >= PDF_MAX_DEVICES_LDS) return hipFuncSetAttribute(kernel, hipFuncAttributeMaxDynamicSharedMemorySize, bytes) == hipSuccess;
    int st = site.state[dev].load(std::memory_order_acquire);
    if (st == 0) {
        st = hipFuncSetAttribute(kernel, hipFuncAttributeMaxDynamicSharedMemorySize, bytes) == hipSuccess ? 1 : 2;
        if (st == 2) (void)hipGetLastError();
        site.state[dev].store(st, std::memory_order_release);
    }
    return st == 1;
}

static inline int pdf_divup(long a, long b) { return (int)((a + b - 1) / b); }

#define PDF_MAX_BLOCKS 2048

__device__ __forceinline__ int pdf_lane() { return (int)(threadIdx.x & 63); }

__device__ __forceinline__ int pdf_wave_min_i32(int v) {
#pragma unroll
    for (int o = 32; o >= 1; o >>= 1) v = min(v, __shfl_xor(v, o, 64));
    return v;
}
__device__ __forceinline__ int pdf_wave_max_i32(int v) {
#pragma unroll
    for (int o = 32; o >= 1; o >>= 1) v = max(v, __shfl_xor(v, o, 64));
    return v;
}
__device__ __forceinline__ unsigned long long pdf_wave_max_u64(unsigned long long v) {
#pragma unroll
    for (int o = 32; o >= 1; o >>= 1) {
        unsigned long long w = __shfl_xor(v, o, 64);
        v = w > v ? w : v;
    }
    return v;
}
__device__ __forceinline__ float pdf_wave_sum_f32(float v) {
#pragma unroll
    for (int o = 32; o >= 1; o >>= 1) v += __shfl_xor(v, o, 64);
    return v;
}

#ifndef PDF_DIST_FMA
#define PDF_DIST_FMA 0
#endif
__host__ __device__ __forceinline__ float pdf_sqdist3(float dx, float dy, float dz) {
#if PDF_DIST_FMA == 1
    return __builtin_fmaf(dz, dz, __builtin_fmaf(dy, dy, dx * dx));
#elif PDF_DIST_FMA == 2
    return __builtin_fmaf(dz, dz, __builtin_fmaf(dx, dx, dy * dy));
#else
    return dx * dx + dy * dy + dz * dz;
#endif
}

__device__ __forceinline__ unsigned pdf_f32_ordered(float f) {
    unsigned u = __float_as_uint(f);
    return (u & 0x80000000u) ? ~u : (u | 0x80000000u);
}

__device__ __forceinline__ void pdf_atomic_add(float *p, float v) {
    __hip_atomic_fetch_add(p, v, __ATOMIC_RELAXED, __HIP_MEMORY_SCOPE_AGENT);
}

#define PDF_XCDS 8
__device__ __forceinline__ unsigned pdf_xcd_chunked_block(unsigned b, unsigned g) {
    const unsigned q = g / PDF_XCDS, r = g % PDF_XCDS, x = b % PDF_XCDS;
    return (x < r ? x * (q + 1) : r * (q + 1) + (x - r) * q) + b / PDF_XCDS;
}

struct PdfRowsBn {
    const float *rows; int nrows; int c; double count;
    const float *gamma, *beta; float *running_mean, *running_var; float eps, momentum;
    float *coef;
    unsigned long long *gran;
    unsigned *sync;
};
#define PDF_HO_WORDS(c) (2 * (size_t)(c) * 2 + 4)
#define PDF_HO_FLOATS PDF_HO_WORDS(1024)
int pdf_rowlin_forward_stats_ho(long n, int k, int o, const float *x, long ldx, const float *w, const float *bias, const float *scale,
                                const float *shift, int relu, float *y, long ldy, float *rows_out, void *handoff, int *rows, int mma_input,
                                void *stream);
int pdf_bn_apply_rows(long n, int c, const float *x, const float *res, const float *rows, int nrows, const float *gamma, const float *beta,
                      float *running_mean, float *running_var, float eps, float momentum, float *coef, void *handoff, int relu, float *y,
                      void *stream);

__device__ __forceinline__ void pdf_handoff_zero(unsigned long long *gran, int c, unsigned *sync) {
    for (int e = threadIdx.x; e < 2 * c; e += blockDim.x) gran[e] = 0ull;
    if (threadIdx.x == 0) sync[0] = 0u;
}

template <int NT>
__device__ __forceinline__ void pdf_bn_reduce_slice(const PdfRowsBn &b, int sl, double *lds_red) {
    constexpr int RL = NT / 16;
    const int c = b.c, cl = threadIdx.x & 15, rl = threadIdx.x >> 4;
    const int ch = sl * 16 + cl;
    double s = 0.0, ss = 0.0;
    if (ch < c) {
        const float *p0 = b.rows + ch, *p1 = b.rows + c + ch;
        const size_t stride = 2 * (size_t)c;
        for (int r = rl; r < b.nrows; r += 8 * RL) {
            float v0[8], v1[8];
#pragma unroll
            for (int t = 0; t < 8; ++t) {
                const int rr = r + t * RL < b.nrows ? r + t * RL : b.nrows - 1;
                v0[t] = p0[(size_t)rr * stride]; v1[t] = p1[(size_t)rr * stride];
            }
#pragma unroll
            for (int t = 0; t < 8; ++t) {
                const bool ok = r + t * RL < b.nrows;
                s += ok ? (double)v0[t] : 0.0; ss += ok ? (double)v1[t] : 0.0;
            }
        }
    }
    __syncthreads();
    lds_red[(0 * RL + rl) * 17 + cl] = s;
    lds_red[(1 * RL + rl) * 17 + cl] = ss;
    __syncthreads();
    if (rl == 0 && ch < c) {
        double a = 0.0, q = 0.0;
        for (int k = 0; k < RL; ++k) { a += lds_red[(0 * RL + k) * 17 + cl]; q += lds_red[(1 * RL + k) * 17 + cl]; }
        const double mean = a / b.count;
        double var = q / b.count - mean * mean;
        if (var < 0.0) var = 0.0;
        const float rstd = (float)(1.0 / sqrt(var + (double)b.eps));
        const float sc = b.gamma[ch] * rstd, sh = b.beta[ch] - (float)mean * sc;
        b.coef[ch] = sc; b.coef[c + ch] = sh; b.coef[2 * c + ch] = (float)mean; b.coef[3 * c + ch] = rstd;
        if (b.running_mean && b.sync != nullptr) {
            const double unbiased = b.count > 1.0 ? var * b.count / (b.count - 1.0) : var;
            b.running_mean[ch] = (1.f - b.momentum) * b.running_mean[ch] + b.momentum * (float)mean;
            b.running_var[ch] = (1.f - b.momentum) * b.running_var[ch] + b.momentum * (float)unbiased;
        }
        __hip_atomic_store(b.gran + ch, (1ull << 32) | (unsigned long long)__float_as_uint(sc), __ATOMIC_RELAXED, __HIP_MEMORY_SCOPE_AGENT);
        __hip_atomic_store(b.gran + c + ch, (1ull << 32) | (unsigned long long)__float_as_uint(sh), __ATOMIC_RELAXED, __HIP_MEMORY_SCOPE_AGENT);
    }
}

template <int NT>
__device__ __forceinline__ void pdf_bn_coef_inkernel(const PdfRowsBn &b, float *lds_coef, double *lds_red, unsigned *lds_word) {
    (void)lds_word;
    const int c = b.c, nsl = (c + 15) / 16;
    const unsigned me = blockIdx.x + gridDim.x * (blockIdx.y + gridDim.y * blockIdx.z), nblk = gridDim.x * gridDim.y * gridDim.z;
    for (unsigned sl = me; sl < (unsigned)nsl; sl += nblk) pdf_bn_reduce_slice<NT>(b, (int)sl, lds_red);
    for (unsigned spins = 0;; ++spins) {
        bool ok = true;
        for (int e = threadIdx.x; e < 2 * c; e += NT) {
            const unsigned long long g = __hip_atomic_load(b.gran + e, __ATOMIC_RELAXED, __HIP_MEMORY_SCOPE_AGENT);
            ok = ok && (g >> 32) == 1ull;
            lds_coef[e] = __uint_as_float((unsigned)g);
        }
        if (__syncthreads_and(ok)) break;
        if (spins == (1u << 14)) {
            PdfRowsBn mine = b;
            mine.sync = nullptr;
            for (int sl = 0; sl < nsl; ++sl) pdf_bn_reduce_slice<NT>(mine, sl, lds_red);
        }
        __builtin_amdgcn_s_sleep(8);
    }
}
```

pointcloudpdf_amd/csrc/pointwise.hip:

```cpp
#include "pdfops_common.h"
#include <cstdlib>

namespace pw {

constexpr int PB = 256;
constexpr int MAXB = 1024;

static inline int grid_rows(long n, int c) {
    const long rows_per_block = (long)PB * 4 / c > 0 ? (long)PB * 4 / c : 1;
    static const int short_rows = [] { const char *v = getenv("PDFOPS_BN_ROWS_SHORT"); const int x = v ? atoi(v) : 0; return x > 0 ? x : 4; }();
    const long per = n * c >= (1L << 22) ? 8 : short_rows;
    long g = (n + rows_per_block * per - 1) / (rows_per_block * per);
    if (g > MAXB) g = MAXB;
    if (g < 1) g = 1;
    return (int)g;
}

__global__ __launch_bounds__(PB) void k_bn_stats(long n, int c, const float *__restrict__ x, float *partial) {
    extern __shared__ float red[];
    const int tpr = c / 4;
    const int rpb = PB / tpr;
    const int tr = threadIdx.x / tpr, tc = threadIdx.x % tpr;
    float s[4] = {0.f, 0.f, 0.f, 0.f}, ss[4] = {0.f, 0.f, 0.f, 0.f};
    if (tr < rpb) {
        for (long r = (long)blockIdx.x * rpb + tr; r < n; r += (long)gridDim.x * rpb) {
            const float4 v = *reinterpret_cast<const float4 *>(x + r * c + tc * 4);
            s[0] += v.x; s[1] += v.y; s[2] += v.z; s[3] += v.w;
            ss[0] += v.x * v.x; ss[1] += v.y * v.y; ss[2] += v.z * v.z; ss[3] += v.w * v.w;
        }
    }
#pragma unroll
    for (int k = 0; k < 4; ++k) { red[threadIdx.x * 8 + k] = s[k]; red[threadIdx.x * 8 + 4 + k] = ss[k]; }
    __syncthreads();
    if (threadIdx.x < tpr) {
#pragma unroll
        for (int k = 0; k < 8; ++k) {
            float a = 0.f;
            for (int rr = 0; rr < rpb; ++rr) a += red[(rr * tpr + threadIdx.x) * 8 + k];
            const int ch = threadIdx.x * 4 + (k & 3);
            partial[(size_t)blockIdx.x * 2 * c + (k < 4 ? ch : c + ch)] = a;
        }
    }
}

template <bool RES>
__global__ __launch_bounds__(PB) void k_bn_apply(long n4, int c4, const float4 *__restrict__ x, const float4 *__restrict__ scale,
                                                 const float4 *__restrict__ shift, const float4 *__restrict__ res, int relu,
                                                 float4 *__restrict__ y) {
    for (long e = (long)blockIdx.x * PB + threadIdx.x; e < n4; e += (long)gridDim.x * PB) {
        const int cc = (int)(e % c4);
        const float4 v = x[e], sc = scale[cc], sh = shift[cc];
        const float4 r = RES ? res[e] : make_float4(0.f, 0.f, 0.f, 0.f);
        float4 o = make_float4(v.x * sc.x + sh.x + r.x, v.y * sc.y + sh.y + r.y, v.z * sc.z + sh.z + r.z, v.w * sc.w + sh.w + r.w);
        if (relu) { o.x = fmaxf(o.x, 0.f); o.y = fmaxf(o.y, 0.f); o.z = fmaxf(o.z, 0.f); o.w = fmaxf(o.w, 0.f); }
        y[e] = o;
    }
}

template <bool RES>
__global__ __launch_bounds__(PB) void k_bn_apply_rows(long n4, int c4, const float4 *__restrict__ x, PdfRowsBn b, const float4 *__restrict__ res,
                                                      int relu, float4 *__restrict__ y) {
    extern __shared__ __attribute__((aligned(16))) float lds[];
    const int c = 4 * c4;
    double *red = reinterpret_cast<double *>(lds + 2 * c);
    unsigned *word = reinterpret_cast<unsigned *>(red + 2 * (PB / 16) * 17);
    pdf_bn_coef_inkernel<PB>(b, lds, red, word);
    const float4 *scale = reinterpret_cast<const float4 *>(lds), *shift = reinterpret_cast<const float4 *>(lds + c);
    for (long e = (long)blockIdx.x * PB + threadIdx.x; e < n4; e += (long)gridDim.x * PB) {
        const int cc = (int)(e % c4);
        const float4 v = x[e], sc = scale[cc], sh = shift[cc];
        const float4 r = RES ? res[e] : make_float4(0.f, 0.f, 0.f, 0.f);
        float4 o = make_float4(v.x * sc.x + sh.x + r.x, v.y * sc.y + sh.y + r.y, v.z * sc.z + sh.z + r.z, v.w * sc.w + sh.w + r.w);
        if (relu) { o.x = fmaxf(o.x, 0.f); o.y = fmaxf(o.y, 0.f); o.z = fmaxf(o.z, 0.f); o.w = fmaxf(o.w, 0.f); }
        y[e] = o;
    }
}

template <bool RES>
__global__ __launch_bounds__(PB) void k_bn_bwd_reduce(long n, int c, const float *__restrict__ gy, const float *__restrict__ x,
                                                      const float *__restrict__ res, const float *__restrict__ scale,
                                                      const float *__restrict__ shift, const float *__restrict__ mean,
                                                      const float *__restrict__ rstd, int relu, float *partial) {
    extern __shared__ float red[];
    const int tpr = c / 4, rpb = PB / tpr;
    const int tr = threadIdx.x / tpr, tc = threadIdx.x % tpr;
    float s[4] = {0.f, 0.f, 0.f, 0.f}, sx[4] = {0.f, 0.f, 0.f, 0.f};
    if (tr < rpb) {
        float sc[4], sh[4], mu[4], rs[4];
#pragma unroll
        for (int k = 0; k < 4; ++k) { sc[k] = scale[tc * 4 + k]; sh[k] = shift[tc * 4 + k]; mu[k] = mean[tc * 4 + k]; rs[k] = rstd[tc * 4 + k]; }
        for (long r = (long)blockIdx.x * rpb + tr; r < n; r += (long)gridDim.x * rpb) {
            const float4 g4 = *reinterpret_cast<const float4 *>(gy + r * c + tc * 4);
            const float4 x4 = *reinterpret_cast<const float4 *>(x + r * c + tc * 4);
            const float4 r4 = RES ? *reinterpret_cast<const float4 *>(res + r * c + tc * 4) : make_float4(0.f, 0.f, 0.f, 0.f);
            const float g[4] = {g4.x, g4.y, g4.z, g4.w}, xv[4] = {x4.x, x4.y, x4.z, x4.w}, rv[4] = {r4.x, r4.y, r4.z, r4.w};
#pragma unroll
            for (int k = 0; k < 4; ++k) {
                const float pre = xv[k] * sc[k] + sh[k] + rv[k];
                const float gm = (!relu || pre > 0.f) ? g[k] : 0.f;
                s[k] += gm;
                sx[k] += gm * ((xv[k] - mu[k]) * rs[k]);
            }
        }
    }
#pragma unroll
    for (int k = 0; k < 4; ++k) { red[threadIdx.x * 8 + k] = s[k]; red[threadIdx.x * 8 + 4 + k] = sx[k]; }
    __syncthreads();
    if (threadIdx.x < tpr) {
#pragma unroll
        for (int k = 0; k < 8; ++k) {
            float a = 0.f;
            for (int rr = 0; rr < rpb; ++rr) a += red[(rr * tpr + threadIdx.x) * 8 + k];
            const int ch = threadIdx.x * 4 + (k & 3);
            partial[(size_t)blockIdx.x * 2 * c + (k < 4 ? ch : c + ch)] = a;
        }
    }
}

template <bool RES>
__global__ __launch_bounds__(PB) void k_bn_bwd_apply(long n4, int c4, const float4 *__restrict__ gy, const float4 *__restrict__ x,
                                                     const float4 *__restrict__ res, const float4 *__restrict__ scale,
                                                     const float4 *__restrict__ shift, const float4 *__restrict__ mean,
                                                     const float4 *__restrict__ rstd, const float4 *__restrict__ sums, float inv_n,
                                                     int relu, float4 *__restrict__ gx, float4 *__restrict__ gres) {
    for (long e = (long)blockIdx.x * PB + threadIdx.x; e < n4; e += (long)gridDim.x * PB) {
        const int cc = (int)(e % c4);
        const float4 g4 = gy[e], x4 = x[e], sc = scale[cc], sh = shift[cc], mu = mean[cc], rs = rstd[cc];
        const float4 s1 = sums[cc], s2 = sums[c4 + cc];
        const float4 r4 = RES ? res[e] : make_float4(0.f, 0.f, 0.f, 0.f);
        float4 gm, o;
#define PW_ONE(f)                                                                     \
        {                                                                             \
            const float pre = x4.f * sc.f + sh.f + r4.f;                              \
            gm.f = (!relu || pre > 0.f) ? g4.f : 0.f;                                 \
            const float xh = (x4.f - mu.f) * rs.f;                                    \
            o.f = sc.f * (gm.f - s1.f * inv_n - xh * s2.f * inv_n);                   \
        }
        PW_ONE(x) PW_ONE(y) PW_ONE(z) PW_ONE(w)
#undef PW_ONE
        gx[e] = o;
        if (gres) gres[e] = gm;
    }
}

template <bool RES>
__global__ __launch_bounds__(PB) void k_bn_bwd_eval(long n4, int c4, const float4 *__restrict__ gy, const float4 *__restrict__ x,
                                                    const float4 *__restrict__ res, const float4 *__restrict__ scale,
                                                    const float4 *__restrict__ shift, int relu, float4 *__restrict__ gx,
                                                    float4 *__restrict__ gres) {
    for (long e = (long)blockIdx.x * PB + threadIdx.x; e < n4; e += (long)gridDim.x * PB) {
        const int cc = (int)(e % c4);
        const float4 g4 = gy[e], x4 = x[e], sc = scale[cc], sh = shift[cc];
        const float4 r4 = RES ? res[e] : make_float4(0.f, 0.f, 0.f, 0.f);
        float4 gm;
        gm.x = (!relu || x4.x * sc.x + sh.x + r4.x > 0.f) ? g4.x : 0.f;
        gm.y = (!relu || x4.y * sc.y + sh.y + r4.y > 0.f) ? g4.y : 0.f;
        gm.z = (!relu || x4.z * sc.z + sh.z + r4.z > 0.f) ? g4.z : 0.f;
        gm.w = (!relu || x4.w * sc.w + sh.w + r4.w > 0.f) ? g4.w : 0.f;
        gx[e] = make_float4(gm.x * sc.x, gm.y * sc.y, gm.z * sc.z, gm.w * sc.w);
        if (gres) gres[e] = gm;
    }
}

static inline int grid_elems(long n4) {
    long g = (n4 + PB - 1) / PB;
    if (g > 2048) g = 2048;
    if (g < 1) g = 1;
    return (int)g;
}

}

namespace fl {
void launch_bn_finalize(const float *partial, int rows, int nch, double count, const float *gamma, const float *beta, float eps,
                        float momentum, float *running_mean, float *running_var, float *scale, float *shift, float *mean_out,
                        float *rstd_out, hipStream_t s);
void launch_bn_eval(int nch, const float *gamma, const float *beta, float eps, const float *running_mean, const float *running_var,
                    float *scale, float *shift, float *mean_out, float *rstd_out, hipStream_t s);
void launch_colsum(const float *partial, int rows, int width, float *out, hipStream_t s);
}

extern "C" int pdf_bn_supported(int c) { return c >= 4 && c % 4 == 0 && c <= 1024 && (1024 % c == 0); }
extern "C" long pdf_bn_partial_floats(long n, int c) { return (long)pw::grid_rows(n, c) * 2 * c + (long)PDF_HO_FLOATS; }

extern "C" int pdf_bn_act_forward(long n, int c, const float *x, const float *res, const float *gamma, const float *beta,
                                  float *running_mean, float *running_var, int training, float eps, float momentum,
                                  int relu, float *coef, float *partial, float *y, void *stream) {
    if (n < 1 || !x || !gamma || !beta || !coef || !y) return PDF_ERR_BAD_ARG;
    if (!pdf_bn_supported(c)) return PDF_ERR_UNSUPPORTED;
    hipStream_t s = static_cast<hipStream_t>(stream);
    float *scale = coef, *shift = coef + c, *mean = coef + 2 * c, *rstd = coef + 3 * c;
    if (training) {
        if (!partial) return PDF_ERR_BAD_ARG;
        const int g = pw::grid_rows(n, c);
        pw::k_bn_stats<<<g, pw::PB, pw::PB * 8 * sizeof(float), s>>>(n, c, x, partial);
        fl::launch_bn_finalize(partial, g, c, (double)n, gamma, beta, eps, momentum, running_mean, running_var, scale, shift, mean, rstd, s);
    } else {
        if (!running_mean || !running_var) return PDF_ERR_BAD_ARG;
        fl::launch_bn_eval(c, gamma, beta, eps, running_mean, running_var, scale, shift, mean, rstd, s);
    }
    const long n4 = n * (c / 4);
    (res ? pw::k_bn_apply<true> : pw::k_bn_apply<false>)<<<pw::grid_elems(n4), pw::PB, 0, s>>>(n4, c / 4, reinterpret_cast<const float4 *>(x),
                                                        reinterpret_cast<const float4 *>(scale), reinterpret_cast<const float4 *>(shift),
                                                        reinterpret_cast<const float4 *>(res), relu, reinterpret_cast<float4 *>(y));
    return pdf_launch_status();
}

static int bn_act_backward(long n, int c, const float *gy, const float *x, const float *res, const float *coef,
                           int training, int relu, float *partial, float *sums, int sums_zeroed, float *gx, float *gres, void *stream,
                           int presummed = 0) {
    (void)sums_zeroed;
    if (n < 1 || !gy || !x || !coef || !partial || !sums || !gx) return PDF_ERR_BAD_ARG;
    if (!pdf_bn_supported(c)) return PDF_ERR_UNSUPPORTED;
    hipStream_t s = static_cast<hipStream_t>(stream);
    const float *scale = coef, *shift = coef + c, *mean = coef + 2 * c, *rstd = coef + 3 * c;
    const int g = pw::grid_rows(n, c);
    const long n4 = n * (c / 4);
    if (presummed > 0) {
        fl::launch_colsum(partial, presummed, 2 * c, sums, s);
    } else {
        (res ? pw::k_bn_bwd_reduce<true> : pw::k_bn_bwd_reduce<false>)<<<g, pw::PB, pw::PB * 8 * sizeof(float), s>>>(
            n, c, gy, x, res, scale, shift, mean, rstd, relu, partial);
        fl::launch_colsum(partial, g, 2 * c, sums, s);
    }
#define F4(p) reinterpret_cast<const float4 *>(p)
    if (training)
        (res ? pw::k_bn_bwd_apply<true> : pw::k_bn_bwd_apply<false>)<<<pw::grid_elems(n4), pw::PB, 0, s>>>(n4, c / 4, F4(gy), F4(x), F4(res), F4(scale), F4(shift), F4(mean), F4(rstd),
                                                                F4(sums), (float)(1.0 / (double)n), relu, reinterpret_cast<float4 *>(gx),
                                                                reinterpret_cast<float4 *>(gres));
    else
        (res ? pw::k_bn_bwd_eval<true> : pw::k_bn_bwd_eval<false>)<<<pw::grid_elems(n4), pw::PB, 0, s>>>(n4, c / 4, F4(gy), F4(x), F4(res), F4(scale), F4(shift), relu,
                                                               reinterpret_cast<float4 *>(gx), reinterpret_cast<float4 *>(gres));
#undef F4
    return pdf_launch_status();
}

extern "C" int pdf_bn_act_backward(long n, int c, const float *gy, const float *x, const float *res, const float *coef,
                                   int training, int relu, float *partial, float *sums, float *gx, float *gres, void *stream) {
    return bn_act_backward(n, c, gy, x, res, coef, training, relu, partial, sums, 0, gx, gres, stream);
}
extern "C" int pdf_bn_act_backward_presummed(long n, int c, const float *gy, const float *x, const float *coef, int training, int relu,
                                             const float *partial, int partial_rows, float *sums, float *gx, void *stream) {
    if (partial_rows < 1 || !partial) return PDF_ERR_BAD_ARG;
    return bn_act_backward(n, c, gy, x, nullptr, coef, training, relu, const_cast<float *>(partial), sums, 0, gx, nullptr, stream, partial_rows);
}
extern "C" int pdf_bn_coef_from_partial(const float *partial, int rows, long n, int c, const float *gamma, const float *beta,
                                        float *running_mean, float *running_var, float eps, float momentum, float *coef,
                                        void *stream) {
    if (!partial || rows < 1 || n < 1 || c < 1 || !gamma || !beta || !coef) return PDF_ERR_BAD_ARG;
    fl::launch_bn_finalize(partial, rows, c, (double)n, gamma, beta, eps, momentum, running_mean, running_var, coef, coef + c,
                           coef + 2 * c, coef + 3 * c, static_cast<hipStream_t>(stream));
    return pdf_launch_status();
}

extern "C" int pdf_bn_apply(long n, int c, const float *x, const float *res, const float *coef, int relu, float *y, void *stream) {
    if (n < 1 || !x || !coef || !y) return PDF_ERR_BAD_ARG;
    if (!pdf_bn_supported(c)) return PDF_ERR_UNSUPPORTED;
    const long n4 = n * (c / 4);
    (res ? pw::k_bn_apply<true> : pw::k_bn_apply<false>)<<<pw::grid_elems(n4), pw::PB, 0, static_cast<hipStream_t>(stream)>>>(
        n4, c / 4, reinterpret_cast<const float4 *>(x), reinterpret_cast<const float4 *>(coef), reinterpret_cast<const float4 *>(coef + c),
        reinterpret_cast<const float4 *>(res), relu, reinterpret_cast<float4 *>(y));
    return pdf_launch_status();
}

int pdf_bn_apply_rows(long n, int c, const float *x, const float *res, const float *rows, int nrows, const float *gamma, const float *beta,
                      float *running_mean, float *running_var, float eps, float momentum, float *coef, void *handoff, int relu, float *y,
                      void *stream) {
    if (n < 1 || !x || !rows || nrows < 1 || !gamma || !beta || !coef || !handoff || !y) return PDF_ERR_BAD_ARG;
    if (!pdf_bn_supported(c)) return PDF_ERR_UNSUPPORTED;
    PdfRowsBn b;
    b.rows = rows; b.nrows = nrows; b.c = c; b.count = (double)n; b.gamma = gamma; b.beta = beta; b.running_mean = running_mean;
    b.running_var = running_var; b.eps = eps; b.momentum = momentum; b.coef = coef;
    b.gran = static_cast<unsigned long long *>(handoff); b.sync = reinterpret_cast<unsigned *>(b.gran + 2 * (size_t)c);
    const long n4 = n * (c / 4);
    const size_t lds = sizeof(float) * 2 * c + sizeof(double) * 2 * (pw::PB / 16) * 17 + 16;
    (res ? pw::k_bn_apply_rows<true> : pw::k_bn_apply_rows<false>)<<<pw::grid_elems(n4), pw::PB, lds, static_cast<hipStream_t>(stream)>>>(
        n4, c / 4, reinterpret_cast<const float4 *>(x), b, reinterpret_cast<const float4 *>(res), relu, reinterpret_cast<float4 *>(y));
    return pdf_launch_status();
}

extern "C" int pdf_bn_coef(long n, int c, const float *x, const float *gamma, const float *beta, float *running_mean,
                           float *running_var, int training, float eps, float momentum, float *coef, float *partial, void *stream) {
    if (n < 1 || !gamma || !beta || !coef) return PDF_ERR_BAD_ARG;
    if (!pdf_bn_supported(c)) return PDF_ERR_UNSUPPORTED;
    hipStream_t s = static_cast<hipStream_t>(stream);
    if (training) {
        if (!partial || !x) return PDF_ERR_BAD_ARG;
        const int g = pw::grid_rows(n, c);
        pw::k_bn_stats<<<g, pw::PB, pw::PB * 8 * sizeof(float), s>>>(n, c, x, partial);
        fl::launch_bn_finalize(partial, g, c, (double)n, gamma, beta, eps, momentum, running_mean, running_var, coef, coef + c, coef + 2 * c, coef + 3 * c, s);
    } else {
        if (!running_mean || !running_var) return PDF_ERR_BAD_ARG;
        fl::launch_bn_eval(c, gamma, beta, eps, running_mean, running_var, coef, coef + c, coef + 2 * c, coef + 3 * c, s);
    }
    return pdf_launch_status();
}

extern "C" int pdf_bn_bwd_sums(long n, int c, const float *gy, const float *x, const float *coef, int relu, float *partial, float *sums,
                               void *stream) {
    if (n < 1 || !gy || !x || !coef || !partial || !sums) return PDF_ERR_BAD_ARG;
    if (!pdf_bn_supported(c)) return PDF_ERR_UNSUPPORTED;
    hipStream_t s = static_cast<hipStream_t>(stream);
    const int g = pw::grid_rows(n, c);
    pw::k_bn_bwd_reduce<false><<<g, pw::PB, pw::PB * 8 * sizeof(float), s>>>(n, c, gy, x, nullptr, coef, coef + c, coef + 2 * c, coef + 3 * c, relu, partial);
    fl::launch_colsum(partial, g, 2 * c, sums, s);
    return pdf_launch_status();
}
```

pointcloudpdf_amd/csrc/rowlin.hip:

```cpp
#include "pdfops_common.h"
#include <cstdlib>

namespace rl {

typedef float f32x16 __attribute__((ext_vector_type(16)));
constexpr int BM = 128, BN = 64, BK = 32, LDT = 33;

struct FwdArgs {
    long N;
    int K, O;
    const float *X; long ldx;
    const float *W; long wso, wsk;
    const float *bias;
    const float *scale, *shift;
    int relu;
    float *Y; long ldy;
    int accumulate;
    float *partial;
};

template <bool PRE, bool STATS>
__global__ __launch_bounds__(256) void k_rowlin(FwdArgs a) {
    __shared__ float xs[BM * LDT];
    __shared__ float ws[BN * LDT];
    __shared__ float red[4][2][BN];
    const int tid = threadIdx.x, lane = tid & 63, wave = tid >> 6;
    const long row0 = (long)blockIdx.x * BM;
    const int o0 = blockIdx.y * BN;
    f32x16 acc0, acc1;
#pragma unroll
    for (int r = 0; r < 16; ++r) { acc0[r] = 0.f; acc1[r] = 0.f; }
    const int kk = tid & 31, rr = tid >> 5;
    for (int k0 = 0; k0 < a.K; k0 += BK) {
        const int k = k0 + kk;
        float sc = 1.f, sh = 0.f;
        if (PRE && k < a.K) { sc = a.scale[k]; sh = a.shift[k]; }
#pragma unroll
        for (int i = 0; i < BM / 8; ++i) {
            const int r = rr + 8 * i;
            const long row = row0 + r;
            float v = 0.f;
            if (row < a.N && k < a.K) {
                v = a.X[row * a.ldx + k];
                if (PRE) { v = v * sc + sh; if (a.relu) v = fmaxf(v, 0.f); }
            }
            xs[r * LDT + kk] = v;
        }
#pragma unroll
        for (int i = 0; i < BN / 8; ++i) {
            const int o = rr + 8 * i;
            float v = 0.f;
            if (o0 + o < a.O && k < a.K) v = a.W[(long)(o0 + o) * a.wso + (long)k * a.wsk];
            ws[o * LDT + kk] = v;
        }
        __syncthreads();
        const float *xa = xs + (wave * 32 + (lane & 31)) * LDT + (lane >> 5);
        const float *wb0 = ws + (lane & 31) * LDT + (lane >> 5);
        const float *wb1 = ws + (32 + (lane & 31)) * LDT + (lane >> 5);
#pragma unroll
        for (int q = 0; q < BK; q += 2) {
            const float av = xa[q];
            acc0 = __builtin_amdgcn_mfma_f32_32x32x2f32(av, wb0[q], acc0, 0, 0, 0);
            acc1 = __builtin_amdgcn_mfma_f32_32x32x2f32(av, wb1[q], acc1, 0, 0, 0);
        }
        __syncthreads();
    }
#pragma unroll
    for (int half = 0; half < 2; ++half) {
        const int col = o0 + half * 32 + (lane & 31);
        const float bv = (a.bias && col < a.O) ? a.bias[col] : 0.f;
        float s = 0.f, ss = 0.f;
#pragma unroll
        for (int r = 0; r < 16; ++r) {
            const int i = (r & 3) + 8 * (r >> 2) + 4 * (lane >> 5);
            const long row = row0 + wave * 32 + i;
            if (row < a.N && col < a.O) {
                float v = (half ? acc1[r] : acc0[r]) + bv;
                float *dst = a.Y + row * a.ldy + col;
                if (a.accumulate) v += *dst;
                *dst = v;
                s += v;
                ss += v * v;
            }
        }
        if (STATS) {
            s += __shfl_xor(s, 32, 64);
            ss += __shfl_xor(ss, 32, 64);
            if (lane < 32) { red[wave][0][half * 32 + lane] = s; red[wave][1][half * 32 + lane] = ss; }
        }
    }
    if (STATS) {
        __syncthreads();
        if (tid < BN && o0 + tid < a.O) {
            const float s = red[0][0][tid] + red[1][0][tid] + red[2][0][tid] + red[3][0][tid];
            const float ss = red[0][1][tid] + red[1][1][tid] + red[2][1][tid] + red[3][1][tid];
            a.partial[(size_t)blockIdx.x * 2 * a.O + o0 + tid] = s;
            a.partial[(size_t)blockIdx.x * 2 * a.O + a.O + o0 + tid] = ss;
        }
    }
}

struct WArgs {
    long N;
    int K, O;
    const float *G; long ldg;
    const float *X; long ldx;
    const float *scale, *shift;
    int relu;
    float *dW;
    float *db;
    long rows_per_block;
    float *slab;
    float *bslab;
};

template <bool PRE>
__global__ __launch_bounds__(256) void k_wgrad(WArgs a) {
    const int lane = threadIdx.x & 63, wave = threadIdx.x >> 6;
    const int kblocks = (a.K + 31) / 32;
    const int o0 = (blockIdx.y / kblocks) * 32, c0 = (blockIdx.y % kblocks) * 32;
    const int ch = lane & 31, par = lane >> 5;
    const int oc = o0 + ch, cc = c0 + ch;
    const bool ov = oc < a.O, cv = cc < a.K;
    float sc = 1.f, sh = 0.f;
    if (PRE && cv) { sc = a.scale[cc]; sh = a.shift[cc]; }
    const long rb = (long)blockIdx.x * a.rows_per_block;
    const long re = min(rb + a.rows_per_block, a.N);
    f32x16 acc;
#pragma unroll
    for (int r = 0; r < 16; ++r) acc[r] = 0.f;
    float gsum = 0.f;
    for (long r0 = rb + 8 * wave; r0 < re; r0 += 32) {
        float g[4], x[4];
#pragma unroll
        for (int u = 0; u < 4; ++u) {
            const long r = r0 + 2 * u + par;
            g[u] = (r < re && ov) ? a.G[r * a.ldg + oc] : 0.f;
            float v = 0.f;
            if (r < re && cv) {
                v = a.X[r * a.ldx + cc];
                if (PRE) { v = v * sc + sh; if (a.relu) v = fmaxf(v, 0.f); }
            }
            x[u] = v;
        }
#pragma unroll
        for (int u = 0; u < 4; ++u) {
            acc = __builtin_amdgcn_mfma_f32_32x32x2f32(g[u], x[u], acc, 0, 0, 0);
            gsum += g[u];
        }
    }
    __shared__ float comb[4][1024 + 32];
#pragma unroll
    for (int r = 0; r < 16; ++r) {
        const int i = (r & 3) + 8 * (r >> 2) + 4 * (lane >> 5);
        comb[wave][i * 32 + ch] = acc[r];
    }
    gsum += __shfl_xor(gsum, 32, 64);
    if (lane < 32) comb[wave][1024 + ch] = gsum;
    __syncthreads();
    const size_t sidx = blockIdx.x, nsl = gridDim.x;
    float *slab = a.slab + ((size_t)blockIdx.y * nsl + sidx) * 1024;
#pragma unroll
    for (int e = threadIdx.x; e < 1024; e += 256) slab[e] = ((comb[0][e] + comb[1][e]) + comb[2][e]) + comb[3][e];
    if (a.db && c0 == 0 && threadIdx.x < 32)
        a.bslab[((size_t)(o0 / 32) * nsl + sidx) * 32 + threadIdx.x] =
            ((comb[0][1024 + threadIdx.x] + comb[1][1024 + threadIdx.x]) + comb[2][1024 + threadIdx.x]) + comb[3][1024 + threadIdx.x];
}

}

namespace rl2 {
int try_forward(long n, int k, int o, int nin, int nout, const float *const *x, long ldx, const float *const *w, int transpose_w,
                const float *const *bias, const float *scale, const float *shift, int relu, float *const *y, long ldy,
                int accumulate, float *partial, int mma, hipStream_t s, const float *roww = nullptr, long rws = 0, const float *bx = nullptr,
                long ldb = 0, const float *bcoef = nullptr, int brelu = 0, int *partial_rows = nullptr, long ldw = 0, void *handoff = nullptr);
long stats_rows_floats(long n, int o);
int try_wgrad(long n, int k, int o, int ng, const float *const *g, long ldg, const float *x, long ldx, const float *scale,
              const float *shift, int relu, float *const *dw, float *const *db, float *ws, int mma, hipStream_t s, const float *roww = nullptr, long rws = 0);
long wgrad_ws_floats(long n, int k, int o, int ng);
constexpr int WG_MAXG = 5;
struct RArgs {
    const float *slab, *bslab;
    float *dW[WG_MAXG], *db[WG_MAXG];
    int B, tiles_k, tiles, otiles, split, K, O;
};
int try_wgrad_group(long n, int k, int o, int ng, const float *const *g, long ldg, const float *const *x, long ldx, const float *const *scale,
                    const float *const *shift, const int *relu, float *const *dw, float *const *db, float *ws, int mma, hipStream_t s);
void launch_slab_reduce(const RArgs &a, int ng, bool any_bias, hipStream_t s);
int stats_rows(long n);
}

static inline void tiled_wg_plan(long n, int k, int o, int *blocks_oc, long *split, long *rows_per_block) {
    *blocks_oc = ((o + 31) / 32) * ((k + 31) / 32);
    long sp = (2048 + *blocks_oc - 1) / *blocks_oc;
    const long max_split = (n + 255) / 256;
    if (sp > max_split) sp = max_split;
    if (sp < 1) sp = 1;
    *rows_per_block = ((n + sp - 1) / sp + 31) / 32 * 32;
    *split = (n + *rows_per_block - 1) / *rows_per_block;
}

static inline bool rowlin_streams(int k, int o) {
    return (k == 32 || k == 64 || k == 128 || k == 256 || k == 512) && o % 16 == 0 && getenv("PDFOPS_ROWLIN_TILED") == nullptr;
}

extern "C" int pdf_rowlin_partial_rows(long n, int k, int o) {
    return rowlin_streams(k, o) ? rl2::stats_rows(n) : (int)((n + rl::BM - 1) / rl::BM);
}
extern "C" long pdf_rowlin_partial_floats(long n, int o) {
    const long a = (n + rl::BM - 1) / rl::BM * 2 * (long)o, b = rl2::stats_rows_floats(n, o);
    return (a > b ? a : b) + (long)PDF_HO_FLOATS;
}

extern "C" int pdf_rowlin_forward(long n, int k, int o, const float *x, long ldx, const float *w, int transpose_w,
                                  const float *bias, const float *scale, const float *shift, int relu, float *y, long ldy,
                                  int accumulate, float *partial, int mma_input, void *stream) {
    if (mma_input < 0 || mma_input > 2) return PDF_ERR_BAD_ARG;
    if (n < 1 || k < 1 || o < 1 || !x || !w || !y || ldx < k || ldy < o) return PDF_ERR_BAD_ARG;
    if (rowlin_streams(k, o)) {
        if (rl2::try_forward(n, k, o, 1, 1, &x, ldx, &w, transpose_w, &bias, scale, shift, relu, &y, ldy, accumulate, partial,
                             mma_input, static_cast<hipStream_t>(stream)))
            return pdf_launch_status();
        if (partial) return PDF_ERR_BAD_ARG;
    }
    if (!transpose_w && !partial && !scale && k == 1024 && rowlin_streams(512, o) && !(ldx & 3) && !(ldy & 3)) {
        const float *xs[2] = {x, x + 512}, *ws[2] = {w, w + 512};
        if (rl2::try_forward(n, 512, o, 2, 1, xs, ldx, ws, 0, &bias, nullptr, nullptr, 0, &y, ldy, accumulate, nullptr, mma_input, static_cast<hipStream_t>(stream),
                             nullptr, 0, nullptr, 0, nullptr, 0, nullptr, k))
            return pdf_launch_status();
    }
    rl::FwdArgs a;
    a.N = n; a.K = k; a.O = o; a.X = x; a.ldx = ldx; a.W = w;
    a.wso = transpose_w ? 1 : k; a.wsk = transpose_w ? o : 1;
    a.bias = bias; a.scale = scale; a.shift = shift; a.relu = relu; a.Y = y; a.ldy = ldy; a.accumulate = accumulate;
    a.partial = partial;
    const dim3 grid((unsigned)((n + rl::BM - 1) / rl::BM), (unsigned)((o + rl::BN - 1) / rl::BN));
    hipStream_t s = static_cast<hipStream_t>(stream);
    const bool pre = scale != nullptr, stats = partial != nullptr;
    if (pre && stats) rl::k_rowlin<true, true><<<grid, 256, 0, s>>>(a);
    else if (pre) rl::k_rowlin<true, false><<<grid, 256, 0, s>>>(a);
    else if (stats) rl::k_rowlin<false, true><<<grid, 256, 0, s>>>(a);
    else rl::k_rowlin<false, false><<<grid, 256, 0, s>>>(a);
    return pdf_launch_status();
}

extern "C" long pdf_rowlin_wgrad_ws_floats(long n, int k, int o, int ng) {
    if (n < 1 || k < 1 || o < 1 || ng < 1) return 0;
    int blocks_oc; long split, rpb;
    tiled_wg_plan(n, k, o, &blocks_oc, &split, &rpb);
    const long tiled = (long)blocks_oc * split * 4 * 1024 + (long)((o + 31) / 32) * split * 4 * 32;
    const long streaming = rowlin_streams(k, o) ? rl2::wgrad_ws_floats(n, k, o, ng) : 0;
    return tiled > streaming ? tiled : streaming;
}

extern "C" int pdf_bn_coef_from_partial(const float *partial, int rows, long n, int c, const float *gamma, const float *beta,
                                        float *running_mean, float *running_var, float eps, float momentum, float *coef, void *stream);

extern "C" int pdf_rowlin_forward_bn(long n, int k, int o, const float *x, long ldx, const float *w, const float *bias, const float *scale,
                                     const float *shift, int relu, float *y, long ldy, float *partial, const float *gamma, const float *beta,
                                     float *running_mean, float *running_var, float eps, float momentum, float *coef, int mma_input, void *stream) {
    if (mma_input < 0 || mma_input > 2) return PDF_ERR_BAD_ARG;
    if (n < 1 || k < 1 || o < 1 || !x || !w || !y || !partial || !gamma || !beta || !coef || ldx < k || ldy < o) return PDF_ERR_BAD_ARG;
    if (rowlin_streams(k, o)) {
        int rows = 0;
        if (rl2::try_forward(n, k, o, 1, 1, &x, ldx, &w, 0, &bias, scale, shift, relu, &y, ldy, 0, partial, mma_input, static_cast<hipStream_t>(stream),
                             nullptr, 0, nullptr, 0, nullptr, 0, &rows)) {
            return pdf_bn_coef_from_partial(partial, rows, n, o, gamma, beta, running_mean, running_var, eps, momentum, coef, stream);
        }
    }
    const int rc = pdf_rowlin_forward(n, k, o, x, ldx, w, 0, bias, scale, shift, relu, y, ldy, 0, partial, mma_input, stream);
    if (rc) return rc;
    return pdf_bn_coef_from_partial(partial, pdf_rowlin_partial_rows(n, k, o), n, o, gamma, beta, running_mean, running_var, eps, momentum, coef, stream);
}

int pdf_rowlin_forward_stats_ho(long n, int k, int o, const float *x, long ldx, const float *w, const float *bias, const float *scale,
                                const float *shift, int relu, float *y, long ldy, float *rows_out, void *handoff, int *rows, int mma_input,
                                void *stream) {
    if (!rowlin_streams(k, o)) return PDF_ERR_UNSUPPORTED;
    if (!rl2::try_forward(n, k, o, 1, 1, &x, ldx, &w, 0, &bias, scale, shift, relu, &y, ldy, 0, rows_out, mma_input, static_cast<hipStream_t>(stream),
                          nullptr, 0, nullptr, 0, nullptr, 0, rows, 0, handoff))
        return PDF_ERR_UNSUPPORTED;
    return pdf_launch_status();
}

extern "C" int pdf_rowlin_wgrad(long n, int k, int o, const float *g, long ldg, const float *x, long ldx,
                                const float *scale, const float *shift, int relu, float *dw, float *db, float *ws, int mma_input, void *stream) {
    if (mma_input < 0 || mma_input > 2) return PDF_ERR_BAD_ARG;
    if (n < 1 || k < 1 || o < 1 || !g || !x || !dw || !ws || ldg < o || ldx < k) return PDF_ERR_BAD_ARG;
    if (rowlin_streams(k, o) && rl2::try_wgrad(n, k, o, 1, &g, ldg, x, ldx, scale, shift, relu, &dw, &db, ws, mma_input, static_cast<hipStream_t>(stream)))
        return pdf_launch_status();
    rl::WArgs a;
    a.N = n; a.K = k; a.O = o; a.G = g; a.ldg = ldg; a.X = x; a.ldx = ldx; a.scale = scale; a.shift = shift; a.relu = relu;
    a.dW = dw; a.db = db;
    int blocks_oc; long split;
    tiled_wg_plan(n, k, o, &blocks_oc, &split, &a.rows_per_block);
    a.slab = ws;
    a.bslab = ws + (size_t)blocks_oc * split * 1024;
    const dim3 grid((unsigned)split, (unsigned)blocks_oc);
    hipStream_t s = static_cast<hipStream_t>(stream);
    if (scale) rl::k_wgrad<true><<<grid, 256, 0, s>>>(a);
    else rl::k_wgrad<false><<<grid, 256, 0, s>>>(a);
    rl2::RArgs r;
    r.slab = a.slab; r.bslab = a.bslab; r.B = 32; r.tiles_k = (k + 31) / 32; r.tiles = blocks_oc; r.otiles = (o + 31) / 32; r.split = (int)split;
    r.K = k; r.O = o;
    r.dW[0] = dw; r.db[0] = db; r.dW[1] = r.dW[2] = nullptr; r.db[1] = r.db[2] = nullptr;
    rl2::launch_slab_reduce(r, 1, db != nullptr, s);
    return pdf_launch_status();
}

extern "C" int pdf_rowlin_multi(long n, int k, int o, int nin, int nout, const float *const *x, long ldx, const float *const *w,
                                int transpose_w, const float *const *bias, const float *scale, const float *shift, int relu,
                                float *const *y, long ldy, int accumulate, int mma_input, void *stream) {
    if (mma_input < 0 || mma_input > 2) return PDF_ERR_BAD_ARG;
    if (n < 1 || k < 1 || o < 1 || !x || !w || !y || nin < 1 || nout < 1 || nin > 3 || nout > 3 || (nin > 1 && nout > 1)) return PDF_ERR_BAD_ARG;
    if (rowlin_streams(k, o) && rl2::try_forward(n, k, o, nin, nout, x, ldx, w, transpose_w, bias, scale, shift, relu, y, ldy, accumulate,
                                                 nullptr, mma_input, static_cast<hipStream_t>(stream)))
        return pdf_launch_status();
    int rc = 0;
    if (nin == 1) {
        for (int i = 0; i < nout && rc == 0; ++i)
            rc = pdf_rowlin_forward(n, k, o, x[0], ldx, w[i], transpose_w, bias ? bias[i] : nullptr, scale, shift, relu, y[i], ldy, accumulate, nullptr, mma_input, stream);
    } else {
        for (int i = 0; i < nin && rc == 0; ++i)
            rc = pdf_rowlin_forward(n, k, o, x[i], ldx, w[i], transpose_w, (i == 0 && bias) ? bias[0] : nullptr, scale, shift, relu, y[0], ldy,
                                    accumulate || i > 0, nullptr, mma_input, stream);
    }
    return rc;
}

extern "C" int pdf_rowlin_dgrad_bstats(long n, int k, int o, int nin, const float *const *x, long ldx, const float *const *w, float *y, long ldy,
                                       const float *bx, long ldb, const float *bcoef, int brelu, float *partial, int *partial_rows,
                                       int mma_input, void *stream) {
    if (mma_input < 0 || mma_input > 2) return PDF_ERR_BAD_ARG;
    if (n < 1 || k < 1 || o < 1 || !x || !w || !y || nin < 1 || nin > 3 || !bx || !bcoef || !partial || !partial_rows) return PDF_ERR_BAD_ARG;
    if (!rowlin_streams(k, o)) return PDF_ERR_UNSUPPORTED;
    float *ys[1] = {y};
    if (!rl2::try_forward(n, k, o, nin, 1, x, ldx, w, 1, nullptr, nullptr, nullptr, 0, ys, ldy, 0, partial, mma_input, static_cast<hipStream_t>(stream),
                          nullptr, 0, bx, ldb, bcoef, brelu, partial_rows))
        return PDF_ERR_UNSUPPORTED;
    return pdf_launch_status();
}

extern "C" int pdf_rowlin_wgrad_multi(long n, int k, int o, int ng, const float *const *g, long ldg, const float *x, long ldx,
                                      const float *scale, const float *shift, int relu, float *const *dw, float *const *db,
                                      float *ws, int mma_input, void *stream) {
    if (mma_input < 0 || mma_input > 2) return PDF_ERR_BAD_ARG;
    if (n < 1 || k < 1 || o < 1 || ng < 1 || ng > 3 || !g || !x || !dw || !ws) return PDF_ERR_BAD_ARG;
    if (rowlin_streams(k, o) && rl2::try_wgrad(n, k, o, ng, g, ldg, x, ldx, scale, shift, relu, dw, db, ws, mma_input, static_cast<hipStream_t>(stream)))
        return pdf_launch_status();
    int rc = 0;
    for (int i = 0; i < ng && rc == 0; ++i) rc = pdf_rowlin_wgrad(n, k, o, g[i], ldg, x, ldx, scale, shift, relu, dw[i], db ? db[i] : nullptr, ws, mma_input, stream);
    return rc;
}

extern "C" int pdf_rowlin_wgrad_group(long n, int k, int o, int ng, const float *const *g, long ldg, const float *const *x, long ldx,
                                      const float *const *scale, const float *const *shift, const int *relu, float *const *dw,
                                      float *const *db, float *ws, int mma_input, void *stream) {
    if (mma_input < 0 || mma_input > 2) return PDF_ERR_BAD_ARG;
    if (n < 1 || k < 1 || o < 1 || ng < 1 || ng > rl2::WG_MAXG || !g || !x || !scale || !shift || !relu || !dw || !ws) return PDF_ERR_BAD_ARG;
    for (int i = 0; i < ng; ++i) if (!g[i] || !x[i] || !dw[i] || (scale[i] && !shift[i])) return PDF_ERR_BAD_ARG;
    if (!rowlin_streams(k, o) || !rl2::try_wgrad_group(n, k, o, ng, g, ldg, x, ldx, scale, shift, relu, dw, db, ws, mma_input, static_cast<hipStream_t>(stream)))
        return PDF_ERR_UNSUPPORTED;
    return pdf_launch_status();
}

extern "C" int pdf_rowlin_forward_roww(long n, int k, int o, const float *x, long ldx, const float *w, int transpose_w, float *y, long ldy,
                                       int accumulate, const float *roww, long rws, int mma_input, void *stream) {
    if (mma_input < 0 || mma_input > 2) return PDF_ERR_BAD_ARG;
    if (n < 1 || !x || !w || !y || !rowlin_streams(k, o)) return PDF_ERR_UNSUPPORTED;
    const float *bias = nullptr;
    if (!rl2::try_forward(n, k, o, 1, 1, &x, ldx, &w, transpose_w, &bias, nullptr, nullptr, 0, &y, ldy, accumulate, nullptr,
                          mma_input, static_cast<hipStream_t>(stream), roww, rws))
        return PDF_ERR_UNSUPPORTED;
    return pdf_launch_status();
}
extern "C" int pdf_rowlin_wgrad_roww(long n, int k, int o, const float *g, long ldg, const float *x, long ldx, float *dw, const float *roww,
                                     long rws, float *ws, int mma_input, void *stream) {
    if (mma_input < 0 || mma_input > 2) return PDF_ERR_BAD_ARG;
    if (n < 1 || !g || !x || !dw || !ws || !rowlin_streams(k, o)) return PDF_ERR_UNSUPPORTED;
    float *db = nullptr;
    if (!rl2::try_wgrad(n, k, o, 1, &g, ldg, x, ldx, nullptr, nullptr, 0, &dw, &db, ws, mma_input, static_cast<hipStream_t>(stream), roww, rws))
        return PDF_ERR_UNSUPPORTED;
    return pdf_launch_status();
}
```

pointcloudpdf_amd/csrc/rowlin2.hip:

```cpp
#define RL2_MAIN_TU
#include "rowlin2_impl.h"

namespace rl2 {
template int try_forward_mp<0>(long, int, int, int, int, const float *const *, long, const float *const *, int, const float *const *, const float *,
                               const float *, int, float *const *, long, int, float *, hipStream_t, const float *, long, const float *, long,
                               const float *, int, int *, long, void *);
template int try_wgrad_mp<0>(long, int, int, int, const float *const *, long, const float *, long, const float *, const float *, int,
                             float *const *, float *const *, float *, hipStream_t, const float *, long);
template int try_wgrad_group_mp<0>(long, int, int, int, const float *const *, long, const float *const *, long, const float *const *, const float *const *, const int *,
                                   float *const *, float *const *, float *, hipStream_t);
extern template int try_wgrad_group_mp<1>(long, int, int, int, const float *const *, long, const float *const *, long, const float *const *, const float *const *, const int *,
                                   float *const *, float *const *, float *, hipStream_t);
extern template int try_wgrad_group_mp<2>(long, int, int, int, const float *const *, long, const float *const *, long, const float *const *, const float *const *, const int *,
                                   float *const *, float *const *, float *, hipStream_t);
extern template int try_forward_mp<1>(long, int, int, int, int, const float *const *, long, const float *const *, int, const float *const *, const float *,
                                      const float *, int, float *const *, long, int, float *, hipStream_t, const float *, long, const float *, long,
                                      const float *, int, int *, long, void *);
extern template int try_forward_mp<2>(long, int, int, int, int, const float *const *, long, const float *const *, int, const float *const *, const float *,
                                      const float *, int, float *const *, long, int, float *, hipStream_t, const float *, long, const float *, long,
                                      const float *, int, int *, long, void *);
extern template int try_wgrad_mp<1>(long, int, int, int, const float *const *, long, const float *, long, const float *, const float *, int,
                                    float *const *, float *const *, float *, hipStream_t, const float *, long);
extern template int try_wgrad_mp<2>(long, int, int, int, const float *const *, long, const float *, long, const float *, const float *, int,
                                    float *const *, float *const *, float *, hipStream_t, const float *, long);

int try_forward(long n, int k, int o, int nin, int nout, const float *const *x, long ldx, const float *const *w, int transpose_w,
                const float *const *bias, const float *scale, const float *shift, int relu, float *const *y, long ldy,
                int accumulate, float *partial, int mma, hipStream_t s, const float *roww, long rws, const float *bx, long ldb, const float *bcoef,
                int brelu, int *partial_rows, long ldw, void *handoff) {
#define RL2_FWD(MP_) try_forward_mp<MP_>(n, k, o, nin, nout, x, ldx, w, transpose_w, bias, scale, shift, relu, y, ldy, accumulate, partial, s, roww, rws, \
                                         bx, ldb, bcoef, brelu, partial_rows, ldw, handoff)
    switch (mma) {
    case 1: return RL2_FWD(1);
    case 2: return RL2_FWD(2);
    default: return RL2_FWD(0);
    }
#undef RL2_FWD
}

int try_wgrad(long n, int k, int o, int ng, const float *const *g, long ldg, const float *x, long ldx, const float *scale,
              const float *shift, int relu, float *const *dw, float *const *db, float *ws, int mma, hipStream_t s, const float *roww, long rws) {
    switch (mma) {
    case 1: return try_wgrad_mp<1>(n, k, o, ng, g, ldg, x, ldx, scale, shift, relu, dw, db, ws, s, roww, rws);
    case 2: return try_wgrad_mp<2>(n, k, o, ng, g, ldg, x, ldx, scale, shift, relu, dw, db, ws, s, roww, rws);
    default: return try_wgrad_mp<0>(n, k, o, ng, g, ldg, x, ldx, scale, shift, relu, dw, db, ws, s, roww, rws);
    }
}

int try_wgrad_group(long n, int k, int o, int ng, const float *const *g, long ldg, const float *const *x, long ldx, const float *const *scale,
                    const float *const *shift, const int *relu, float *const *dw, float *const *db, float *ws, int mma, hipStream_t s) {
    switch (mma) {
    case 1: return try_wgrad_group_mp<1>(n, k, o, ng, g, ldg, x, ldx, scale, shift, relu, dw, db, ws, s);
    case 2: return try_wgrad_group_mp<2>(n, k, o, ng, g, ldg, x, ldx, scale, shift, relu, dw, db, ws, s);
    default: return try_wgrad_group_mp<0>(n, k, o, ng, g, ldg, x, ldx, scale, shift, relu, dw, db, ws, s);
    }
}
}
```

pointcloudpdf_amd/csrc/rowlin2_bf16.hip:

```cpp
#include "rowlin2_impl.h"

namespace rl2 {
template int try_forward_mp<2>(long, int, int, int, int, const float *const *, long, const float *const *, int, const float *const *, const float *,
                               const float *, int, float *const *, long, int, float *, hipStream_t, const float *, long, const float *, long,
                               const float *, int, int *, long, void *);
template int try_wgrad_mp<2>(long, int, int, int, const float *const *, long, const float *, long, const float *, const float *, int,
                             float *const *, float *const *, float *, hipStream_t, const float *, long);
template int try_wgrad_group_mp<2>(long, int, int, int, const float *const *, long, const float *const *, long, const float *const *, const float *const *, const int *,
                                   float *const *, float *const *, float *, hipStream_t);
}
```

pointcloudpdf_amd/csrc/rowlin2_f16.hip:

```cpp
#include "rowlin2_impl.h"

namespace rl2 {
template int try_forward_mp<1>(long, int, int, int, int, const float *const *, long, const float *const *, int, const float *const *, const float *,
                               const float *, int, float *const *, long, int, float *, hipStream_t, const float *, long, const float *, long,
                               const float *, int, int *, long, void *);
template int try_wgrad_mp<1>(long, int, int, int, const float *const *, long, const float *, long, const float *, const float *, int,
                             float *const *, float *const *, float *, hipStream_t, const float *, long);
template int try_wgrad_group_mp<1>(long, int, int, int, const float *const *, long, const float *const *, long, const float *const *, const float *const *, const int *,
                                   float *const *, float *const *, float *, hipStream_t);
}
```

pointcloudpdf_amd/csrc/rowlin2_impl.h:

```cpp
#pragma once
#include "pdfops_common.h"
#include <algorithm>
#include <cstdlib>

namespace rl2 {

typedef float f32x4 __attribute__((ext_vector_type(4)));

typedef _Float16 h16x4 __attribute__((ext_vector_type(4)));
typedef __bf16 b16x4 __attribute__((ext_vector_type(4)));
typedef short s16x4 __attribute__((ext_vector_type(4)));
template <int MP> struct Mma;
template <> struct Mma<0> {
    typedef f32x4 frag;
    static __device__ __forceinline__ frag cvt(f32x4 v) { return v; }
};
template <> struct Mma<1> {
    typedef h16x4 frag;
    static __device__ __forceinline__ frag cvt(f32x4 v) { return __builtin_convertvector(v, h16x4); }
    static __device__ __forceinline__ f32x4 mma(frag a, frag b, f32x4 acc) { return __builtin_amdgcn_mfma_f32_16x16x16f16(a, b, acc, 0, 0, 0); }
};
template <> struct Mma<2> {
    typedef s16x4 frag;
    static __device__ __forceinline__ frag cvt(f32x4 v) { return __builtin_bit_cast(s16x4, __builtin_convertvector(v, b16x4)); }
    static __device__ __forceinline__ f32x4 mma(frag a, frag b, f32x4 acc) { return __builtin_amdgcn_mfma_f32_16x16x16bf16_1k(a, b, acc, 0, 0, 0); }
};

long stats_rows_floats(long n, int o);

struct FwdArgs {
    long N;
    int O;
    const float *X[3]; long ldx;
    const float *W[3]; long wso, wsk;
    const float *bias[3];
    const float *scale, *shift; int relu;
    float *Y[3]; long ldy;
    int accumulate;
    float *partial;
    const float *bx; long ldb; const float *bcoef; int brelu;
    const float *roww; long rws;
    unsigned long long *ho_gran; unsigned *ho_sync;
};

constexpr int FWD_CAP = 1024;
static inline int fwd_row_blocks(long n) {
    const long tiles = (n + 15) / 16, b = (tiles + 3) / 4;
    return (int)(b < 1 ? 1 : (b > FWD_CAP ? FWD_CAP : b));
}

template <int K, int NOB, int NIN, bool PRE, int ST, int MP>
__global__ __launch_bounds__(256) void k_fwd(FwdArgs a) {
    typedef typename Mma<MP>::frag wfrag;
    constexpr bool STATS = ST != 0;
    constexpr int NJ = K / 16;
    constexpr bool COEF_REGS = K <= 64;
    const int lane = threadIdx.x & 63, wave = threadIdx.x >> 6;
    const int li = lane & 15, kq = lane >> 4;
    if (ST == 1 && a.ho_gran && blockIdx.x == 0 && blockIdx.y == 0) pdf_handoff_zero(a.ho_gran, a.O, a.ho_sync);
    const int gcol0 = blockIdx.y * NOB * 16;
    int outi[NOB], colb[NOB];
#pragma unroll
    for (int ob = 0; ob < NOB; ++ob) { outi[ob] = (gcol0 + ob * 16) / a.O; colb[ob] = gcol0 + ob * 16 - outi[ob] * a.O; }
    wfrag Wr[NIN][NOB][NJ];
#pragma unroll
    for (int in = 0; in < NIN; ++in) {
#pragma unroll
        for (int ob = 0; ob < NOB; ++ob) {
            const float *W = a.W[NIN > 1 ? in : outi[ob]];
            const long o = colb[ob] + li;
#pragma unroll
            for (int j = 0; j < NJ; ++j) {
                f32x4 w4;
                if (a.wsk == 1) {
                    w4 = *reinterpret_cast<const f32x4 *>(W + o * a.wso + 16 * j + 4 * kq);
                } else {
#pragma unroll
                    for (int c = 0; c < 4; ++c) w4[c] = W[o * a.wso + (long)(16 * j + 4 * kq + c) * a.wsk];
                }
                Wr[in][ob][j] = Mma<MP>::cvt(w4);
            }
        }
    }
    f32x4 bias4[NOB];
#pragma unroll
    for (int ob = 0; ob < NOB; ++ob) {
        const float *b = a.bias[NIN > 1 ? 0 : outi[ob]];
#pragma unroll
        for (int r = 0; r < 4; ++r) bias4[ob][r] = b ? b[colb[ob] + 4 * kq + r] : 0.f;
    }
    f32x4 sc4[COEF_REGS && PRE ? NJ : 1], sh4[COEF_REGS && PRE ? NJ : 1];
    if (PRE && COEF_REGS) {
#pragma unroll
        for (int j = 0; j < NJ; ++j) {
            sc4[j] = *reinterpret_cast<const f32x4 *>(a.scale + 16 * j + 4 * kq);
            sh4[j] = *reinterpret_cast<const f32x4 *>(a.shift + 16 * j + 4 * kq);
        }
    }
    f32x4 s4[STATS ? NOB : 1], ss4[STATS ? NOB : 1];
    if (STATS) {
#pragma unroll
        for (int ob = 0; ob < NOB; ++ob) { s4[ob] = f32x4{0.f, 0.f, 0.f, 0.f}; ss4[ob] = f32x4{0.f, 0.f, 0.f, 0.f}; }
    }
    __shared__ float bco[ST == 2 ? 3 : 1][NOB * 16];
    if (ST == 2) {
        if (threadIdx.x < 3 * NOB * 16) {
            const int v = threadIdx.x / (NOB * 16), t = threadIdx.x % (NOB * 16);
            bco[ST == 2 ? v : 0][t] = a.bcoef[(long)v * a.O + gcol0 + t];
        }
        __syncthreads();
    }
    __shared__ float pco[PRE && !COEF_REGS ? 2 : 1][PRE && !COEF_REGS ? K : 1];
    if (PRE && !COEF_REGS) {
        for (int t = threadIdx.x; t < K; t += 256) { pco[0][t] = a.scale[t]; pco[PRE && !COEF_REGS ? 1 : 0][t] = a.shift[t]; }
        __syncthreads();
    }
    const float relu_lo = a.relu ? 0.f : -INFINITY;
    constexpr int XB0 = NJ < 16 ? NJ : 16;
    constexpr int XB = (K == 256 && NIN == 3) ? 4 : ((ST != 0 && NOB > 1 && NIN * NOB * NJ * 4 >= 128) ? ((PRE && K == 128) ? 2 : XB0 / 2) : XB0);
    const long ntiles = (a.N + 15) / 16;
    for (long tile = (long)blockIdx.x * 4 + wave; tile < ntiles; tile += (long)gridDim.x * 4) {
        const long n = tile * 16 + li;
        const bool valid = n < a.N;
        f32x4 acc[NOB];
#pragma unroll
        for (int ob = 0; ob < NOB; ++ob) acc[ob] = f32x4{0.f, 0.f, 0.f, 0.f};
#pragma unroll
        for (int in = 0; in < NIN; ++in) {
            const float *xr = a.X[in] + (valid ? n : 0) * a.ldx + 4 * kq;
#pragma unroll
            for (int j0 = 0; j0 < NJ; j0 += XB) {
                f32x4 xb[XB];
#pragma unroll
                for (int t = 0; t < XB; ++t) xb[t] = *reinterpret_cast<const f32x4 *>(xr + 16 * (j0 + t));
                __builtin_amdgcn_sched_barrier(0);
#pragma unroll
                for (int t = 0; t < XB; ++t) {
                    const int j = j0 + t;
                    f32x4 x4 = xb[t];
                    if (PRE) {
                        const f32x4 sc = COEF_REGS ? sc4[COEF_REGS ? j : 0] : *reinterpret_cast<const f32x4 *>(&pco[0][16 * j + 4 * kq]);
                        const f32x4 sh = COEF_REGS ? sh4[COEF_REGS ? j : 0] : *reinterpret_cast<const f32x4 *>(&pco[PRE && !COEF_REGS ? 1 : 0][16 * j + 4 * kq]);
                        x4 = x4 * sc + sh;
#pragma unroll
                        for (int c = 0; c < 4; ++c) x4[c] = fmaxf(x4[c], relu_lo);
                    }
                    if constexpr (MP == 0) {
#pragma unroll
                        for (int c = 0; c < 4; ++c)
#pragma unroll
                            for (int ob = 0; ob < NOB; ++ob)
                                acc[ob] = __builtin_amdgcn_mfma_f32_16x16x4f32(Wr[in][ob][j][c], x4[c], acc[ob], 0, 0, 0);
                    } else {
                        const wfrag xh = Mma<MP>::cvt(x4);
#pragma unroll
                        for (int ob = 0; ob < NOB; ++ob) acc[ob] = Mma<MP>::mma(Wr[in][ob][j], xh, acc[ob]);
                    }
                }
            }
        }
#pragma unroll
        for (int ob = 0; ob < NOB; ++ob) {
            f32x4 v = acc[ob];
            if (a.roww) v *= a.roww[(valid ? n : 0) * a.rws];
            v += bias4[ob];
            float *dst = a.Y[outi[ob]] + (valid ? n : 0) * a.ldy + colb[ob] + 4 * kq;
            if (a.accumulate && valid) v += *reinterpret_cast<const f32x4 *>(dst);
            if (valid) *reinterpret_cast<f32x4 *>(dst) = v;
            if (ST == 1 && valid) { s4[ob] += v; ss4[ob] += v * v; }
            if (ST == 2) {
                const f32x4 x4 = *reinterpret_cast<const f32x4 *>(a.bx + (valid ? n : 0) * a.ldb + colb[ob] + 4 * kq);
                const f32x4 sc = *reinterpret_cast<const f32x4 *>(&bco[0][ob * 16 + 4 * kq]);
                const f32x4 sh = *reinterpret_cast<const f32x4 *>(&bco[ST == 2 ? 1 : 0][ob * 16 + 4 * kq]);
                const f32x4 mu = *reinterpret_cast<const f32x4 *>(&bco[ST == 2 ? 2 : 0][ob * 16 + 4 * kq]);
                const f32x4 pre = x4 * sc + sh;
                f32x4 gm;
#pragma unroll
                for (int c = 0; c < 4; ++c) gm[c] = (valid && (!a.brelu || pre[c] > 0.f)) ? v[c] : 0.f;
                s4[ob] += gm;
                ss4[ob] += gm * (x4 - mu);
            }
        }
    }
    if (STATS) {
        __shared__ float red[4][2][NOB * 16];
#pragma unroll
        for (int ob = 0; ob < NOB; ++ob)
#pragma unroll
            for (int r = 0; r < 4; ++r) {
                float s = s4[ob][r], ss = ss4[ob][r];
#pragma unroll
                for (int m = 1; m < 16; m <<= 1) { s += __shfl_xor(s, m, 64); ss += __shfl_xor(ss, m, 64); }
                if (li == 0) { red[wave][0][ob * 16 + 4 * kq + r] = s; red[wave][1][ob * 16 + 4 * kq + r] = ss; }
            }
        __syncthreads();
        const int t = threadIdx.x;
        if (t < NOB * 16) {
            float *row = a.partial + (size_t)blockIdx.x * 2 * a.O;
            row[gcol0 + t] = red[0][0][t] + red[1][0][t] + red[2][0][t] + red[3][0][t];
            const float ss = red[0][1][t] + red[1][1][t] + red[2][1][t] + red[3][1][t];
            row[a.O + gcol0 + t] = ST == 2 ? ss * a.bcoef[3 * (long)a.O + gcol0 + t] : ss;
        }
    }
}

constexpr int WG_MAXG = 5;
struct WArgs {
    long N;
    int K, O;
    const float *G[WG_MAXG]; long ldg;
    const float *X; long ldx;
    const float *scale, *shift; int relu;
    int per_z; const float *Xz[WG_MAXG]; const float *scalez[WG_MAXG], *shiftz[WG_MAXG]; int reluz[WG_MAXG];
    float *dW[WG_MAXG], *db[WG_MAXG];
    long rows_per_block;
    const float *roww; long rws;
    float *slab;
    float *bslab;
};

template <int VW> struct Vec;
template <> struct Vec<2> { typedef float type __attribute__((ext_vector_type(2))); };
template <> struct Vec<4> { typedef float type __attribute__((ext_vector_type(4))); };

template <int VW, bool PRE, bool RW, int MP>
__global__ __launch_bounds__(256) void k_wg(WArgs a) {
    typedef typename Vec<VW>::type vec;
    constexpr int B = 16 * VW;
    __shared__ float red[4][B * B];
    __shared__ float redb[4][B];
    const int lane = threadIdx.x & 63, wave = threadIdx.x >> 6;
    const int li = lane & 15, nq = lane >> 4;
    const int nkb = a.K / B;
    const int ob = (blockIdx.y / nkb) * B, kb = (blockIdx.y % nkb) * B;
    const float *G = a.G[blockIdx.z];
    const float *X = (PRE && a.per_z) ? a.Xz[blockIdx.z] : a.X;
    vec sc, sh;
    bool relu = a.relu != 0;
    if (PRE) {
        const float *scp = a.per_z ? a.scalez[blockIdx.z] : a.scale, *shp = a.per_z ? a.shiftz[blockIdx.z] : a.shift;
        if (a.per_z) relu = scp != nullptr && a.reluz[blockIdx.z] != 0;
        if (scp) {
            sc = *reinterpret_cast<const vec *>(scp + kb + VW * li);
            sh = *reinterpret_cast<const vec *>(shp + kb + VW * li);
        } else {
#pragma unroll
            for (int c = 0; c < VW; ++c) { sc[c] = 1.f; sh[c] = 0.f; }
        }
    }
    const float relu_lo = relu ? 0.f : -INFINITY;
    f32x4 acc[VW][VW];
    float gsum[VW];
#pragma unroll
    for (int c = 0; c < VW; ++c) {
        gsum[c] = 0.f;
#pragma unroll
        for (int c2 = 0; c2 < VW; ++c2) acc[c][c2] = f32x4{0.f, 0.f, 0.f, 0.f};
    }
    const long rb = (long)blockIdx.x * a.rows_per_block;
    const long re = rb + a.rows_per_block < a.N ? rb + a.rows_per_block : a.N;
    for (long r0 = rb + 16 * wave; r0 < re; r0 += 64) {
        vec gv[4], xv[4];
        float rw[RW ? 4 : 1];
        bool ok[4];
#pragma unroll
        for (int t = 0; t < 4; ++t) {
            const long n = r0 + 4 * t + nq;
            ok[t] = n < re;
            const long nn = ok[t] ? n : rb;
            gv[t] = *reinterpret_cast<const vec *>(G + nn * a.ldg + ob + VW * li);
            xv[t] = *reinterpret_cast<const vec *>(X + nn * a.ldx + kb + VW * li);
            if (RW) rw[RW ? t : 0] = a.roww[nn * a.rws];
        }
        __builtin_amdgcn_sched_barrier(0);
#pragma unroll
        for (int t = 0; t < 4; ++t) {
            if (RW) gv[t] *= rw[RW ? t : 0];
            if (PRE) {
                xv[t] = xv[t] * sc + sh;
#pragma unroll
                for (int c = 0; c < VW; ++c) xv[t][c] = fmaxf(xv[t][c], relu_lo);
            }
#pragma unroll
            for (int c = 0; c < VW; ++c) { gv[t][c] = ok[t] ? gv[t][c] : 0.f; xv[t][c] = ok[t] ? xv[t][c] : 0.f; }
        }
        if constexpr (MP == 0) {
#pragma unroll
            for (int t = 0; t < 4; ++t)
#pragma unroll
                for (int c = 0; c < VW; ++c) {
                    gsum[c] += gv[t][c];
#pragma unroll
                    for (int c2 = 0; c2 < VW; ++c2)
                        acc[c][c2] = __builtin_amdgcn_mfma_f32_16x16x4f32(gv[t][c], xv[t][c2], acc[c][c2], 0, 0, 0);
                }
        } else {
            typename Mma<MP>::frag ga[VW], xa[VW];
#pragma unroll
            for (int c = 0; c < VW; ++c) {
                gsum[c] += (gv[0][c] + gv[1][c]) + (gv[2][c] + gv[3][c]);
                ga[c] = Mma<MP>::cvt(f32x4{gv[0][c], gv[1][c], gv[2][c], gv[3][c]});
                xa[c] = Mma<MP>::cvt(f32x4{xv[0][c], xv[1][c], xv[2][c], xv[3][c]});
            }
#pragma unroll
            for (int c = 0; c < VW; ++c)
#pragma unroll
                for (int c2 = 0; c2 < VW; ++c2) acc[c][c2] = Mma<MP>::mma(ga[c], xa[c2], acc[c][c2]);
        }
    }
#pragma unroll
    for (int c = 0; c < VW; ++c)
#pragma unroll
        for (int c2 = 0; c2 < VW; ++c2)
#pragma unroll
            for (int r = 0; r < 4; ++r) red[wave][(VW * (4 * nq + r) + c) * B + VW * li + c2] = acc[c][c2][r];
    float *db = a.db[blockIdx.z];
    const bool want_db = db && kb == 0;
    if (want_db) {
#pragma unroll
        for (int c = 0; c < VW; ++c) {
            float g = gsum[c];
            g += __shfl_xor(g, 16, 64);
            g += __shfl_xor(g, 32, 64);
            if (nq == 0) redb[wave][VW * li + c] = g;
        }
    }
    __syncthreads();
    float *slab = a.slab + (((size_t)blockIdx.z * gridDim.y + blockIdx.y) * gridDim.x + blockIdx.x) * (B * B);
    for (int e = threadIdx.x; e < B * B; e += 256) slab[e] = (red[0][e] + red[1][e]) + (red[2][e] + red[3][e]);
    if (want_db && threadIdx.x < B)
        a.bslab[(((size_t)blockIdx.z * (a.O / B) + ob / B) * gridDim.x + blockIdx.x) * B + threadIdx.x] =
            (redb[0][threadIdx.x] + redb[1][threadIdx.x]) + (redb[2][threadIdx.x] + redb[3][threadIdx.x]);
}

struct RArgs {
    const float *slab, *bslab;
    float *dW[WG_MAXG], *db[WG_MAXG];
    int B, tiles_k, tiles, otiles, split, K, O;
};
void launch_slab_reduce(const RArgs &a, int ng, bool any_bias, hipStream_t s);
template <int L>
__global__ __launch_bounds__(64 * L) void k_slab_reduce(RArgs a) {
    __shared__ float red[L][64];
    const int e = threadIdx.x & 63, l = threadIdx.x >> 6, z = blockIdx.z;
    const int ei = blockIdx.x * 64 + e;
    const bool bias = (int)blockIdx.y >= a.tiles;
    const int t = bias ? (int)blockIdx.y - a.tiles : (int)blockIdx.y;
    const int len = bias ? a.B : a.B * a.B;
    if (bias && (int)blockIdx.x * 64 >= len) return;
    const float *src = bias ? a.bslab + ((size_t)z * a.otiles + t) * a.split * a.B : a.slab + ((size_t)z * a.tiles + t) * a.split * (size_t)(a.B * a.B);
    float s = 0.f;
    if (ei < len) {
        int k = l;
        for (; k + 3 * L < a.split; k += 4 * L) {
            const float v0 = src[(size_t)k * len + ei], v1 = src[(size_t)(k + L) * len + ei];
            const float v2 = src[(size_t)(k + 2 * L) * len + ei], v3 = src[(size_t)(k + 3 * L) * len + ei];
            s = (((s + v0) + v1) + v2) + v3;
        }
        for (; k < a.split; k += L) s += src[(size_t)k * len + ei];
    }
    red[l][e] = s;
    __syncthreads();
    if (l != 0 || ei >= len) return;
#pragma unroll
    for (int k = 1; k < L; ++k) s += red[k][e];
    if (bias) {
        const int o = t * a.B + ei;
        if (a.db[z] && o < a.O) a.db[z][o] = s;
    } else {
        const int o = (t / a.tiles_k) * a.B + ei / a.B, kk = (t % a.tiles_k) * a.B + ei % a.B;
        if (o < a.O && kk < a.K) a.dW[z][(size_t)o * a.K + kk] = s;
    }
}

#ifdef RL2_MAIN_TU
void launch_slab_reduce(const RArgs &a, int ng, bool any_bias, hipStream_t s) {
    const dim3 grid((unsigned)((a.B * a.B + 63) / 64), (unsigned)(a.tiles + (any_bias ? a.otiles : 0)), (unsigned)ng);
    if (a.split > 32) k_slab_reduce<16><<<grid, 64 * 16, 0, s>>>(a);
    else if (a.split > 4) k_slab_reduce<4><<<grid, 64 * 4, 0, s>>>(a);
    else k_slab_reduce<1><<<grid, 64, 0, s>>>(a);
}
#endif

struct WgPlan { int vw, b, nblk; long split, rows_per_block; };
static WgPlan wg_plan(long n, int k, int o, int ng) {
    WgPlan p;
    p.vw = (k % 64 == 0 && o % 64 == 0) ? 4 : ((k % 32 == 0 && o % 32 == 0) ? 2 : 0);
    p.b = 16 * p.vw;
    if (!p.vw) { p.nblk = 0; p.split = 0; p.rows_per_block = 0; return p; }
    p.nblk = (o / p.b) * (k / p.b) * ng;
    static const int target = [] { const char *v = getenv("PDFOPS_WG_BLOCKS"); const int x = v ? atoi(v) : 0; return x > 0 ? x : 512; }();
    long split = (target + p.nblk - 1) / p.nblk;
    const long max_split = (n + 255) / 256;
    if (split > max_split) split = max_split;
    if (split < 1) split = 1;
    p.rows_per_block = ((n + split - 1) / split + 63) / 64 * 64;
    p.split = (n + p.rows_per_block - 1) / p.rows_per_block;
    return p;
}
#ifdef RL2_MAIN_TU
long wgrad_ws_floats(long n, int k, int o, int ng) {
    const WgPlan p = wg_plan(n, k, o, ng);
    if (!p.vw) return 0;
    return (long)p.nblk * p.split * p.b * p.b + (long)ng * (o / p.b) * p.split * p.b;
}
#endif

static inline bool aligned16(const void *p) { return (reinterpret_cast<uintptr_t>(p) & 15) == 0; }

template <int K, int NOB, int NIN, int MP>
static int launch_fwd(const FwdArgs &a, int nslabs, hipStream_t s) {
    const bool pre = a.scale != nullptr, stats = a.partial != nullptr, bst = stats && a.bx != nullptr;
    static const int total = [] { const char *v = getenv("PDFOPS_RL_BLOCKS"); const int x = v ? atoi(v) : 0; return x > 0 ? x : 512; }();
    int gx = fwd_row_blocks(a.N);
    if (!stats || bst) gx = std::max(1, std::min(gx, std::max(8, total / std::max(nslabs, 1))));
    const dim3 grid((unsigned)gx, (unsigned)nslabs);
    if (bst) {
        k_fwd<K, NOB, NIN, false, 2, MP><<<grid, 256, 0, s>>>(a);
    } else if (NIN == 1 && stats) {
        if (pre) k_fwd<K, NOB, 1, true, 1, MP><<<grid, 256, 0, s>>>(a);
        else k_fwd<K, NOB, 1, false, 1, MP><<<grid, 256, 0, s>>>(a);
    } else {
        if (pre) k_fwd<K, NOB, NIN, true, 0, MP><<<grid, 256, 0, s>>>(a);
        else k_fwd<K, NOB, NIN, false, 0, MP><<<grid, 256, 0, s>>>(a);
    }
    return gx;
}

#ifdef RL2_MAIN_TU
long stats_rows_floats(long n, int o) { return (long)fwd_row_blocks(n) * 2 * o; }
#endif

template <int MP>
int try_forward_mp(long n, int k, int o, int nin, int nout, const float *const *x, long ldx, const float *const *w, int transpose_w,
                   const float *const *bias, const float *scale, const float *shift, int relu, float *const *y, long ldy,
                   int accumulate, float *partial, hipStream_t s, const float *roww, long rws, const float *bx, long ldb, const float *bcoef,
                   int brelu, int *partial_rows, long ldw, void *handoff) {
    if (nin < 1 || nout < 1 || (nin > 1 && nout > 1) || nin > 3 || nout > 3) return 0;
    if (nin == 2 && (scale || bx)) return 0;
    if (partial && !bx && (nin != 1 || nout != 1)) return 0;
    if (bx && (!partial || nout != 1 || scale || !bcoef || (ldb & 3) || !aligned16(bx) || !aligned16(bcoef))) return 0;
    if ((ldx & 3) || (ldy & 3) || (o & 15)) return 0;
    for (int i = 0; i < (nin > 1 ? nin : nout); ++i) if (!aligned16(w[i])) return 0;
    if (scale && (!aligned16(scale) || !aligned16(shift))) return 0;
    for (int i = 0; i < nin; ++i) if (!aligned16(x[i])) return 0;
    for (int i = 0; i < nout; ++i) if (!aligned16(y[i])) return 0;
    FwdArgs a;
    a.N = n; a.O = o; a.ldx = ldx; a.ldy = ldy; a.scale = scale; a.shift = shift; a.relu = relu; a.accumulate = accumulate;
    a.partial = partial; a.roww = roww; a.rws = rws;
    a.bx = bx; a.ldb = ldb; a.bcoef = bcoef; a.brelu = brelu;
    a.ho_gran = static_cast<unsigned long long *>(handoff);
    a.ho_sync = handoff ? reinterpret_cast<unsigned *>(a.ho_gran + 2 * (size_t)o) : nullptr;
    a.wso = transpose_w ? 1 : (ldw ? ldw : k); a.wsk = transpose_w ? o : 1;
    for (int i = 0; i < 3; ++i) {
        a.X[i] = i < nin ? x[i] : nullptr;
        a.W[i] = i < (nin > 1 ? nin : nout) ? w[i] : nullptr;
        a.bias[i] = (bias && i < nout) ? bias[i] : nullptr;
        a.Y[i] = i < nout ? y[i] : nullptr;
    }
    const int cols = o * nout;
#define PDF_RL2(K_, NOB_, NIN_) do { if (cols % (NOB_ * 16) == 0) { \
        const int r_ = launch_fwd<K_, NOB_, NIN_, MP>(a, cols / (NOB_ * 16), s); \
        if (partial_rows) *partial_rows = r_; \
        return 1; } } while (0)
    if (nin == 1) {
        switch (k) {
        case 32: if (!partial) PDF_RL2(32, 6, 1); PDF_RL2(32, 2, 1); PDF_RL2(32, 1, 1); break;
        case 64: PDF_RL2(64, 4, 1); PDF_RL2(64, 1, 1); break;
        case 128: if (!bx) PDF_RL2(128, 4, 1); else PDF_RL2(128, 2, 1); PDF_RL2(128, 1, 1); break;
        case 256: PDF_RL2(256, 2, 1); PDF_RL2(256, 1, 1); break;
        case 512: PDF_RL2(512, 1, 1); break;
        default: break;
        }
    } else if (nin == 2) {
        if (k == 512) PDF_RL2(512, 1, 2);
    } else if (nin == 3) {
        switch (k) {
        case 32: PDF_RL2(32, 2, 3); break;
        case 64: PDF_RL2(64, 2, 3); break;
        case 128: PDF_RL2(128, 1, 3); break;
        case 256: PDF_RL2(256, 1, 3); break;
        default: break;
        }
    }
#undef PDF_RL2
    return 0;
}

template <int MP>
int try_wgrad_mp(long n, int k, int o, int ng, const float *const *g, long ldg, const float *x, long ldx, const float *scale,
                 const float *shift, int relu, float *const *dw, float *const *db, float *ws, hipStream_t s, const float *roww, long rws) {
    if (ng < 1 || ng > 3 || !ws) return 0;
    const WgPlan p = wg_plan(n, k, o, ng);
    const int vw = p.vw;
    if (!vw) return 0;
    if ((ldg % vw) || (ldx % vw) || !aligned16(x)) return 0;
    if (scale && (!aligned16(scale) || !aligned16(shift))) return 0;
    for (int i = 0; i < ng; ++i) if (!aligned16(g[i])) return 0;
    WArgs a;
    a.N = n; a.K = k; a.O = o; a.ldg = ldg; a.X = x; a.ldx = ldx; a.scale = scale; a.shift = shift; a.relu = relu; a.roww = roww; a.rws = rws;
    a.per_z = 0;
    bool any_bias = false;
    for (int i = 0; i < WG_MAXG; ++i) {
        a.G[i] = i < ng ? g[i] : nullptr; a.dW[i] = i < ng ? dw[i] : nullptr; a.db[i] = (db && i < ng) ? db[i] : nullptr;
        a.Xz[i] = nullptr; a.scalez[i] = a.shiftz[i] = nullptr; a.reluz[i] = 0;
        any_bias = any_bias || a.db[i] != nullptr;
    }
    const int b = p.b;
    a.rows_per_block = p.rows_per_block;
    a.slab = ws;
    a.bslab = ws + (size_t)p.nblk * p.split * b * b;
    const dim3 grid((unsigned)p.split, (unsigned)((o / b) * (k / b)), (unsigned)ng);
#define PDF_WG(VW_) do { \
        if (roww) { if (scale) k_wg<VW_, true, true, MP><<<grid, 256, 0, s>>>(a); else k_wg<VW_, false, true, MP><<<grid, 256, 0, s>>>(a); } \
        else      { if (scale) k_wg<VW_, true, false, MP><<<grid, 256, 0, s>>>(a); else k_wg<VW_, false, false, MP><<<grid, 256, 0, s>>>(a); } } while (0)
    if (vw == 4) PDF_WG(4); else PDF_WG(2);
#undef PDF_WG
    RArgs r;
    r.slab = a.slab; r.bslab = a.bslab; r.B = b; r.tiles_k = k / b; r.tiles = (o / b) * (k / b); r.otiles = o / b; r.split = (int)p.split; r.K = k; r.O = o;
    for (int i = 0; i < WG_MAXG; ++i) { r.dW[i] = a.dW[i]; r.db[i] = a.db[i]; }
    launch_slab_reduce(r, ng, any_bias, s);
    return 1;
}

template <int MP>
int try_wgrad_group_mp(long n, int k, int o, int ng, const float *const *g, long ldg, const float *const *x, long ldx,
                       const float *const *scale, const float *const *shift, const int *relu, float *const *dw, float *const *db,
                       float *ws, hipStream_t s) {
    if (ng < 1 || ng > WG_MAXG || !ws) return 0;
    const WgPlan p = wg_plan(n, k, o, ng);
    const int vw = p.vw;
    if (!vw) return 0;
    if ((ldg % vw) || (ldx % vw)) return 0;
    for (int i = 0; i < ng; ++i) {
        if (!aligned16(g[i]) || !aligned16(x[i])) return 0;
        if (scale[i] && (!aligned16(scale[i]) || !aligned16(shift[i]))) return 0;
    }
    WArgs a;
    a.N = n; a.K = k; a.O = o; a.ldg = ldg; a.X = nullptr; a.ldx = ldx; a.scale = a.shift = nullptr; a.relu = 0; a.roww = nullptr; a.rws = 0;
    a.per_z = 1;
    bool any_bias = false;
    for (int i = 0; i < WG_MAXG; ++i) {
        const bool on = i < ng;
        a.G[i] = on ? g[i] : nullptr; a.Xz[i] = on ? x[i] : nullptr;
        a.scalez[i] = on ? scale[i] : nullptr; a.shiftz[i] = on ? shift[i] : nullptr; a.reluz[i] = on ? relu[i] : 0;
        a.dW[i] = on ? dw[i] : nullptr; a.db[i] = (on && db) ? db[i] : nullptr;
        any_bias = any_bias || a.db[i] != nullptr;
    }
    const int b = p.b;
    a.rows_per_block = p.rows_per_block;
    a.slab = ws;
    a.bslab = ws + (size_t)p.nblk * p.split * b * b;
    const dim3 grid((unsigned)p.split, (unsigned)((o / b) * (k / b)), (unsigned)ng);
    if (vw == 4) k_wg<4, true, false, MP><<<grid, 256, 0, s>>>(a); else k_wg<2, true, false, MP><<<grid, 256, 0, s>>>(a);
    RArgs r;
    r.slab = a.slab; r.bslab = a.bslab; r.B = b; r.tiles_k = k / b; r.tiles = (o / b) * (k / b); r.otiles = o / b; r.split = (int)p.split; r.K = k; r.O = o;
    for (int i = 0; i < WG_MAXG; ++i) { r.dW[i] = a.dW[i]; r.db[i] = a.db[i]; }
    launch_slab_reduce(r, ng, any_bias, s);
    return 1;
}

#ifdef RL2_MAIN_TU
int stats_rows(long n) { return fwd_row_blocks(n); }
#endif

}
```

Baseline: 13.49 million.

## Fold BatchNorm-backward elementwise pass into the following dgrad GEMM prologue

Adds pdf_rowlin_bnbwd_dgrad, which computes the BN-backward reduction sums first and then runs the dgrad GEMM kernel with a BN-backward prologue. That prologue computes gx (and the residual gradient) per element, writes them out, and feeds them straight into the MFMA accumulation. This removes a separate elementwise BN-backward kernel and a re-read of its output at several block sites (pre, post, linbn). Per-channel-width gating tables select where the fold applies. The cost is more register and shared-memory pressure in the GEMM kernel, plus extra template instantiations.

```diff
diff --git a/include/pdfops.h b/include/pdfops.h
--- a/include/pdfops.h
+++ b/include/pdfops.h
@@ -10,7 +10,7 @@
 #define PDF_ERR_NSAMPLE (-2)
 #define PDF_ERR_UNSUPPORTED (-3)
 
-#define PDF_ABI_VERSION 7
+#define PDF_ABI_VERSION 8
 int pdf_abi_version(void);
 const char *pdf_build_info(void);
 int pdf_dist_fma_mode(void);
@@ -164,6 +164,11 @@
                           float *running_mean, float *running_var, float eps, float momentum, float *coef, int mma_input, void *stream);
 int pdf_bn_act_backward_presummed(long n, int c, const float *gy, const float *x, const float *coef, int training, int relu,
                                   const float *partial, int partial_rows, float *sums, float *gx, void *stream);
+
+int pdf_rowlin_bnbwd_dgrad(long n, int c, int o, const float *gy, const float *bx, const float *res, const float *coef, int relu,
+                           float *partial, int presummed, float *sums, float *gz, float *gres, const float *w, float *y, long ldy,
+                           int accumulate, const float *sbx, const float *sbcoef, int sbrelu, int *partial_rows, int site,
+                           int mma_input, void *stream);
 
 int pdf_bn_coef_eval_or_partial(const float *partial, int rows, long n, int c, const float *gamma, const float *beta,
                                 float *running_mean, float *running_var, int training, float eps, float momentum,
diff --git a/pointcloudpdf_amd/_native.py b/pointcloudpdf_amd/_native.py
--- a/pointcloudpdf_amd/_native.py
+++ b/pointcloudpdf_amd/_native.py
@@ -15,7 +15,7 @@
 
 
 LIB_PATH = library_path(DIST_FMA)
-ABI_VERSION = 7
+ABI_VERSION = 8
 
 c_int = ctypes.c_int
 c_long = ctypes.c_long
@@ -671,6 +671,9 @@
         lib.pdf_rowlin_dgrad_bstats.restype = c_int
         lib.pdf_rowlin_dgrad_bstats.argtypes = [c_long, c_int, c_int, c_int, c_void_p, c_long, c_void_p, c_void_p, c_long, c_void_p, c_long,
                                                 c_void_p, c_int, c_void_p, ctypes.POINTER(c_int), c_int, c_void_p]
+        lib.pdf_rowlin_bnbwd_dgrad.restype = c_int
+        lib.pdf_rowlin_bnbwd_dgrad.argtypes = [c_long, c_int, c_int] + [c_void_p] * 4 + [c_int, c_void_p, c_int] + [c_void_p] * 5 + [c_long, c_int,
+                                               c_void_p, c_void_p, c_int, c_void_p, c_int, c_int, c_void_p]
         lib.pdf_bn_act_backward_presummed.restype = c_int
         lib.pdf_bn_act_backward_presummed.argtypes = [c_long, c_int, c_void_p, c_void_p, c_void_p, c_int, c_int, c_void_p, c_int, c_void_p,
                                                       c_void_p, c_void_p]
@@ -1261,6 +1264,32 @@
             raise PdfOpsError(f"pdf_bn_act_backward_presummed failed with status {rc}")
         return dy, sums[o:], sums[:o]
 
+    def rowlin_bnbwd_dgrad(self, gy, bx, res, coef, relu, w, y=None, need_res=False, presummed=None, sbx=None, sbcoef=None, sbrelu=True, site=-1):
+        n, c = gy.shape
+        o = w.shape[1]
+        require_current_device(gy, bx, w)
+        npart = max(int(self.lib.pdf_bn_partial_floats(n, c)), int(self.lib.pdf_rowlin_partial_floats(n, o)))
+        if presummed is None:
+            partial, prow = self._new(bx, (npart,), torch.float32), 0
+        else:
+            partial, prow = presummed
+        sums = self._new(bx, (2 * c,), torch.float32)
+        gz = torch.full((n, c), float("nan"), dtype=torch.float32, device=bx.device)
+        gres = torch.full((n, c), float("nan"), dtype=torch.float32, device=bx.device) if need_res else None
+        acc = y is not None
+        if y is None:
+            y = self._new(bx, (n, o), torch.float32)
+        rows = c_int(0)
+        P = lambda t: None if t is None else self._ptr(t)
+        rc = self.lib.pdf_rowlin_bnbwd_dgrad(n, c, o, P(gy), P(bx), P(res), P(coef), int(bool(relu)), P(partial), int(prow), P(sums), P(gz), P(gres),
+                                             P(w), P(y), y.stride(0), int(acc), P(sbx), P(sbcoef), int(bool(sbrelu)),
+                                             ctypes.addressof(rows), int(site), current_mma_input(), self._stream())
+        if rc == -3:
+            return None
+        if rc != 0:
+            raise PdfOpsError(f"pdf_rowlin_bnbwd_dgrad failed with status {rc}")
+        return y, gz, gres, sums[c:], sums[:c], ((partial, rows.value) if sbx is not None else None)
+
     def wgrad_workspace(self, n, k, o, ng, device):
         return torch.empty((max(int(self.lib.pdf_rowlin_wgrad_ws_floats(int(n), int(k), int(o), int(ng))), 1),), dtype=torch.float32, device=device)
 
diff --git a/pointcloudpdf_amd/csrc/block.hip b/pointcloudpdf_amd/csrc/block.hip
--- a/pointcloudpdf_amd/csrc/block.hip
+++ b/pointcloudpdf_amd/csrc/block.hip
@@ -39,12 +39,17 @@
     static const bool on = [] { const char *v = getenv("PDFOPS_INKERNEL_BN"); return !(v && v[0] == '0'); }();
     return on;
 }
+static bool bn_bwd_fold() {
+    const char *v = getenv("PDFOPS_BN_BWD_FOLD");
+    return !(v && v[0] == '0');
+}
 static bool dgrad_bstats() {
     static const bool on = [] { const char *v = getenv("PDFOPS_DGRAD_BSTATS"); return !(v && v[0] == '0'); }();
     return on;
 }
 
-static int block_pre_backward(long n, int c, void *const *p, int training, int accumulate_gx, int mma_input, void *stream, bool defer_wgrad = false) {
+static int block_pre_backward(long n, int c, void *const *p, int training, int accumulate_gx, int mma_input, void *stream, bool defer_wgrad = false,
+                              float *dy_raw = nullptr) {
     if (n < 1 || !p || !p[14]) return PDF_ERR_BAD_ARG;
     const float *x = (const float *)p[0], *z1 = (const float *)p[1], *coef1 = (const float *)p[2], *W1 = (const float *)p[3];
     float *gx = (float *)p[10], *grads = (float *)p[11], *dy = (float *)p[12], *partial = (float *)p[13], *wslab = (float *)p[14];
@@ -57,6 +62,22 @@
     float *ys[1] = {dy};
     if (!defer_wgrad) e << pdf_rowlin_wgrad_multi(n, c, c, 3, gs, c, z1, c, coef1, coef1 + c, 1, dws, dbs, wslab, mma_input, stream);
     int prow = 0;
+    if (dy_raw && training && defer_wgrad && dgrad_bstats() && bn_bwd_fold()) {
+        int rcd = pdf_rowlin_dgrad_bstats(n, c, c, 3, gs, c, ws, dy_raw, c, z1, c, coef1, 1, partial, &prow, mma_input, stream);
+        if (rcd == PDF_ERR_UNSUPPORTED) {
+            float *yr[1] = {dy_raw};
+            prow = 0;
+            rcd = pdf_rowlin_multi(n, c, c, 3, 1, gs, c, ws, 1, nullptr, nullptr, nullptr, 0, yr, c, 0, mma_input, stream);
+        }
+        e << rcd;
+        const int rcf = pdf_rowlin_bnbwd_dgrad(n, c, c, dy_raw, z1, nullptr, coef1, 1, partial, prow, db1, dy, nullptr, W1, gx, c, accumulate_gx,
+                                               nullptr, nullptr, 0, nullptr, 1, mma_input, stream);
+        if (rcf != PDF_ERR_UNSUPPORTED) { e << rcf; return e.rc; }
+        if (prow > 0) e << pdf_bn_act_backward_presummed(n, c, dy_raw, z1, coef1, training, 1, partial, prow, db1, dy, stream);
+        else e << pdf_bn_act_backward(n, c, dy_raw, z1, nullptr, coef1, training, 1, partial, db1, dy, nullptr, stream);
+        e << pdf_rowlin_forward(n, c, c, dy, c, W1, 1, nullptr, nullptr, nullptr, 0, gx, c, accumulate_gx, nullptr, mma_input, stream);
+        return e.rc;
+    }
     const int rc1 = dgrad_bstats() ? pdf_rowlin_dgrad_bstats(n, c, c, 3, gs, c, ws, dy, c, z1, c, coef1, 1, partial, &prow, mma_input, stream) : PDF_ERR_UNSUPPORTED;
     if (rc1 == PDF_ERR_UNSUPPORTED) {
         e << pdf_rowlin_multi(n, c, c, 3, 1, gs, c, ws, 1, nullptr, nullptr, nullptr, 0, ys, c, 0, mma_input, stream);
@@ -120,6 +141,15 @@
     const long cc = (long)c * c;
     float *dW3 = grads, *db2 = grads + cc, *db3 = db2 + 2 * c;
     Err e;
+    if (training && defer_wgrad && dgrad_bstats() && bn_bwd_fold()) {
+        int prowf = 0;
+        const int rcf = pdf_rowlin_bnbwd_dgrad(n, c, c, gy, z3, x, coef3, 1, partial, 0, db3, da, gres, W3, gt, c, 0, t, coef2, 1, &prowf, 0, mma_input, stream);
+        if (rcf != PDF_ERR_UNSUPPORTED) {
+            e << rcf;
+            e << pdf_bn_act_backward_presummed(n, c, gt, t, coef2, training, 1, partial, prowf, db2, gt, stream);
+            return e.rc;
+        }
+    }
     e << pdf_bn_act_backward(n, c, gy, z3, x, coef3, training, 1, partial, db3, da, gres, stream);
     if (!defer_wgrad) e << pdf_rowlin_wgrad(n, c, c, da, c, t, c, coef2, coef2 + c, 1, dW3, nullptr, (float *)p[12], mma_input, stream);
     int prow = 0;
@@ -175,7 +205,7 @@
                                (float *)p[41], (float *)p[42], (const int *)p[43], (const int *)p[44], entry_base,
                                (float *)p[40], (float *)p[32], storage_bf16, (const int *)p[49], (const double *)p[46], stream);
     void *pre[15] = {p[1], p[2], p[3], p[4], p[5], p[6], p[7], p[35], p[36], p[37], p[29], p[30], p[45], p[40], ws_pre};
-    e << block_pre_backward(n, c, pre, training, 1, mma_input, stream, group);
+    e << block_pre_backward(n, c, pre, training, 1, mma_input, stream, group, (float *)p[33]);
     if (group && e.rc == 0) {
         const long cc = (long)c * c;
         float *gpre = (float *)p[30], *gpost = (float *)p[31];
@@ -220,6 +250,16 @@
     float *grads = (float *)p[6], *gz = (float *)p[7];
     const long ok = (long)o * k;
     Err e;
+    const int rcf = (p[5] && training && bn_bwd_fold())
+                        ? pdf_rowlin_bnbwd_dgrad(n, o, k, (const float *)p[0], (const float *)p[2], nullptr, (const float *)p[3], relu, (float *)p[8], 0,
+                                                 grads + ok + o, gz, nullptr, (const float *)p[4], (float *)p[5], k, 0, nullptr, nullptr, 0, nullptr, 2,
+                                                 mma_input, stream)
+                        : PDF_ERR_UNSUPPORTED;
+    if (rcf != PDF_ERR_UNSUPPORTED) {
+        e << rcf;
+        e << pdf_rowlin_wgrad(n, k, o, gz, o, (const float *)p[1], k, nullptr, nullptr, 0, grads, grads + ok, (float *)p[9], mma_input, stream);
+        return e.rc;
+    }
     e << pdf_bn_act_backward(n, o, (const float *)p[0], (const float *)p[2], nullptr, (const float *)p[3], training, relu, (float *)p[8],
                              grads + ok + o, gz, nullptr, stream);
     if (p[5]) e << pdf_rowlin_forward(n, o, k, gz, o, (const float *)p[4], 1, nullptr, nullptr, nullptr, 0, (float *)p[5], k, 0, nullptr, mma_input, stream);
diff --git a/pointcloudpdf_amd/csrc/pdfops_common.h b/pointcloudpdf_amd/csrc/pdfops_common.h
--- a/pointcloudpdf_amd/csrc/pdfops_common.h
+++ b/pointcloudpdf_amd/csrc/pdfops_common.h
@@ -82,6 +82,25 @@
     const unsigned q = g / PDF_XCDS, r = g % PDF_XCDS, x = b % PDF_XCDS;
     return (x < r ? x * (q + 1) : r * (q + 1) + (x - r) * q) + b / PDF_XCDS;
 }
+
+__device__ __forceinline__ float pdf_bn_bwd_one(float g, float x, float r, float sc, float sh, float mu, float rs, float s1, float s2,
+                                                float inv_n, int relu, float *gm_out) {
+#pragma clang fp contract(off)
+    const float pre = fmaf(x, sc, sh) + r;
+    const float gm = (!relu || pre > 0.f) ? g : 0.f;
+    const float xh = (x - mu) * rs;
+    *gm_out = gm;
+    return sc * fmaf(-(xh * s2), inv_n, fmaf(-s1, inv_n, gm));
+}
+struct PdfBnBwdPro {
+    const float *bx, *res;
+    const float *coef;
+    const float *sums;
+    float inv_n; int relu;
+    float *gx, *gres;
+};
+int pdf_bn_bwd_sums_res(long n, int c, const float *gy, const float *x, const float *res, const float *coef, int relu, float *partial,
+                        int presummed, float *sums, void *stream);
 
 struct PdfRowsBn {
     const float *rows; int nrows; int c; double count;
diff --git a/pointcloudpdf_amd/csrc/pointwise.hip b/pointcloudpdf_amd/csrc/pointwise.hip
--- a/pointcloudpdf_amd/csrc/pointwise.hip
+++ b/pointcloudpdf_amd/csrc/pointwise.hip
@@ -129,13 +129,7 @@
         const float4 s1 = sums[cc], s2 = sums[c4 + cc];
         const float4 r4 = RES ? res[e] : make_float4(0.f, 0.f, 0.f, 0.f);
         float4 gm, o;
-#define PW_ONE(f)                                                                     \
-        {                                                                             \
-            const float pre = x4.f * sc.f + sh.f + r4.f;                              \
-            gm.f = (!relu || pre > 0.f) ? g4.f : 0.f;                                 \
-            const float xh = (x4.f - mu.f) * rs.f;                                    \
-            o.f = sc.f * (gm.f - s1.f * inv_n - xh * s2.f * inv_n);                   \
-        }
+#define PW_ONE(f) o.f = pdf_bn_bwd_one(g4.f, x4.f, r4.f, sc.f, sh.f, mu.f, rs.f, s1.f, s2.f, inv_n, relu, &gm.f);
         PW_ONE(x) PW_ONE(y) PW_ONE(z) PW_ONE(w)
 #undef PW_ONE
         gx[e] = o;
@@ -235,6 +229,22 @@
     return pdf_launch_status();
 }
 
+int pdf_bn_bwd_sums_res(long n, int c, const float *gy, const float *x, const float *res, const float *coef, int relu, float *partial,
+                        int presummed, float *sums, void *stream) {
+    if (n < 1 || !gy || !x || !coef || !partial || !sums) return PDF_ERR_BAD_ARG;
+    if (!pdf_bn_supported(c)) return PDF_ERR_UNSUPPORTED;
+    hipStream_t s = static_cast<hipStream_t>(stream);
+    if (presummed > 0) {
+        fl::launch_colsum(partial, presummed, 2 * c, sums, s);
+    } else {
+        const int g = pw::grid_rows(n, c);
+        (res ? pw::k_bn_bwd_reduce<true> : pw::k_bn_bwd_reduce<false>)<<<g, pw::PB, pw::PB * 8 * sizeof(float), s>>>(
+            n, c, gy, x, res, coef, coef + c, coef + 2 * c, coef + 3 * c, relu, partial);
+        fl::launch_colsum(partial, g, 2 * c, sums, s);
+    }
+    return pdf_launch_status();
+}
+
 extern "C" int pdf_bn_act_backward(long n, int c, const float *gy, const float *x, const float *res, const float *coef,
                                    int training, int relu, float *partial, float *sums, float *gx, float *gres, void *stream) {
     return bn_act_backward(n, c, gy, x, res, coef, training, relu, partial, sums, 0, gx, gres, stream);
diff --git a/pointcloudpdf_amd/csrc/rowlin.hip b/pointcloudpdf_amd/csrc/rowlin.hip
--- a/pointcloudpdf_amd/csrc/rowlin.hip
+++ b/pointcloudpdf_amd/csrc/rowlin.hip
@@ -173,7 +173,8 @@
 int try_forward(long n, int k, int o, int nin, int nout, const float *const *x, long ldx, const float *const *w, int transpose_w,
                 const float *const *bias, const float *scale, const float *shift, int relu, float *const *y, long ldy,
                 int accumulate, float *partial, int mma, hipStream_t s, const float *roww = nullptr, long rws = 0, const float *bx = nullptr,
-                long ldb = 0, const float *bcoef = nullptr, int brelu = 0, int *partial_rows = nullptr, long ldw = 0, void *handoff = nullptr);
+                long ldb = 0, const float *bcoef = nullptr, int brelu = 0, int *partial_rows = nullptr, long ldw = 0, void *handoff = nullptr,
+                const PdfBnBwdPro *bnb = nullptr);
 long stats_rows_floats(long n, int o);
 int try_wgrad(long n, int k, int o, int ng, const float *const *g, long ldg, const float *x, long ldx, const float *scale,
               const float *shift, int relu, float *const *dw, float *const *db, float *ws, int mma, hipStream_t s, const float *roww = nullptr, long rws = 0);
@@ -341,6 +342,40 @@
     return pdf_launch_status();
 }
 
+static bool bnbwd_fold_enabled(int c, int site) {
+    const char *v = getenv("PDFOPS_BN_BWD_FOLD");
+    if (v && v[0] == '0') return false;
+    if (site < 0 || (v && v[0] == '2')) return true;
+    static const unsigned char table[3][5] = {
+        {1, 1, 0, 0, 0},
+        {1, 1, 1, 0, 0},
+        {1, 1, 1, 0, 0},
+    };
+    const int ci = c == 32 ? 0 : c == 64 ? 1 : c == 128 ? 2 : c == 256 ? 3 : c == 512 ? 4 : -1;
+    return ci >= 0 && site < 3 && table[site][ci] != 0;
+}
+extern "C" int pdf_rowlin_bnbwd_dgrad(long n, int c, int o, const float *gy, const float *bx, const float *res, const float *coef, int relu,
+                                      float *partial, int presummed, float *sums, float *gz, float *gres, const float *w, float *y, long ldy,
+                                      int accumulate, const float *sbx, const float *sbcoef, int sbrelu, int *partial_rows, int site,
+                                      int mma_input, void *stream) {
+    if (mma_input < 0 || mma_input > 2) return PDF_ERR_BAD_ARG;
+    if (n < 1 || c < 1 || o < 1 || !gy || !bx || !coef || !partial || !sums || !gz || !w || !y || ldy < o || presummed < 0) return PDF_ERR_BAD_ARG;
+    if (gz == gy || (gres && gres == gy) || (sbx && (!sbcoef || !partial_rows))) return PDF_ERR_BAD_ARG;
+    if (!rowlin_streams(c, o) || !pdf_bn_supported(c) || !bnbwd_fold_enabled(c, site)) return PDF_ERR_UNSUPPORTED;
+    const uintptr_t al = (uintptr_t)gy | (uintptr_t)bx | (uintptr_t)res | (uintptr_t)coef | (uintptr_t)sums | (uintptr_t)gz | (uintptr_t)gres |
+                         (uintptr_t)w | (uintptr_t)y | (uintptr_t)sbx | (uintptr_t)sbcoef;
+    if ((al & 15) || (ldy & 3)) return PDF_ERR_UNSUPPORTED;
+    const int rc = pdf_bn_bwd_sums_res(n, c, gy, bx, res, coef, relu, partial, presummed, sums, stream);
+    if (rc) return rc;
+    PdfBnBwdPro pro;
+    pro.bx = bx; pro.res = res; pro.coef = coef; pro.sums = sums; pro.inv_n = (float)(1.0 / (double)n); pro.relu = relu; pro.gx = gz; pro.gres = gres;
+    float *ys[1] = {y};
+    if (!rl2::try_forward(n, c, o, 1, 1, &gy, c, &w, 1, nullptr, nullptr, nullptr, 0, ys, ldy, accumulate, sbx ? partial : nullptr, mma_input,
+                          static_cast<hipStream_t>(stream), nullptr, 0, sbx, o, sbcoef, sbrelu, partial_rows, 0, nullptr, &pro))
+        return PDF_ERR_BAD_ARG;
+    return pdf_launch_status();
+}
+
 extern "C" int pdf_rowlin_wgrad_multi(long n, int k, int o, int ng, const float *const *g, long ldg, const float *x, long ldx,
                                       const float *scale, const float *shift, int relu, float *const *dw, float *const *db,
                                       float *ws, int mma_input, void *stream) {
diff --git a/pointcloudpdf_amd/csrc/rowlin2.hip b/pointcloudpdf_amd/csrc/rowlin2.hip
--- a/pointcloudpdf_amd/csrc/rowlin2.hip
+++ b/pointcloudpdf_amd/csrc/rowlin2.hip
@@ -4,7 +4,7 @@
 namespace rl2 {
 template int try_forward_mp<0>(long, int, int, int, int, const float *const *, long, const float *const *, int, const float *const *, const float *,
                                const float *, int, float *const *, long, int, float *, hipStream_t, const float *, long, const float *, long,
-                               const float *, int, int *, long, void *);
+                               const float *, int, int *, long, void *, const PdfBnBwdPro *);
 template int try_wgrad_mp<0>(long, int, int, int, const float *const *, long, const float *, long, const float *, const float *, int,
                              float *const *, float *const *, float *, hipStream_t, const float *, long);
 template int try_wgrad_group_mp<0>(long, int, int, int, const float *const *, long, const float *const *, long, const float *const *, const float *const *, const int *,
@@ -15,10 +15,10 @@
                                    float *const *, float *const *, float *, hipStream_t);
 extern template int try_forward_mp<1>(long, int, int, int, int, const float *const *, long, const float *const *, int, const float *const *, const float *,
                                       const float *, int, float *const *, long, int, float *, hipStream_t, const float *, long, const float *, long,
-                                      const float *, int, int *, long, void *);
+                                      const float *, int, int *, long, void *, const PdfBnBwdPro *);
 extern template int try_forward_mp<2>(long, int, int, int, int, const float *const *, long, const float *const *, int, const float *const *, const float *,
                                       const float *, int, float *const *, long, int, float *, hipStream_t, const float *, long, const float *, long,
-                                      const float *, int, int *, long, void *);
+                                      const float *, int, int *, long, void *, const PdfBnBwdPro *);
 extern template int try_wgrad_mp<1>(long, int, int, int, const float *const *, long, const float *, long, const float *, const float *, int,
                                     float *const *, float *const *, float *, hipStream_t, const float *, long);
 extern template int try_wgrad_mp<2>(long, int, int, int, const float *const *, long, const float *, long, const float *, const float *, int,
@@ -27,9 +27,9 @@
 int try_forward(long n, int k, int o, int nin, int nout, const float *const *x, long ldx, const float *const *w, int transpose_w,
                 const float *const *bias, const float *scale, const float *shift, int relu, float *const *y, long ldy,
                 int accumulate, float *partial, int mma, hipStream_t s, const float *roww, long rws, const float *bx, long ldb, const float *bcoef,
-                int brelu, int *partial_rows, long ldw, void *handoff) {
+                int brelu, int *partial_rows, long ldw, void *handoff, const PdfBnBwdPro *bnb) {
 #define RL2_FWD(MP_) try_forward_mp<MP_>(n, k, o, nin, nout, x, ldx, w, transpose_w, bias, scale, shift, relu, y, ldy, accumulate, partial, s, roww, rws, \
-                                         bx, ldb, bcoef, brelu, partial_rows, ldw, handoff)
+                                         bx, ldb, bcoef, brelu, partial_rows, ldw, handoff, bnb)
     switch (mma) {
     case 1: return RL2_FWD(1);
     case 2: return RL2_FWD(2);
diff --git a/pointcloudpdf_amd/csrc/rowlin2_bf16.hip b/pointcloudpdf_amd/csrc/rowlin2_bf16.hip
--- a/pointcloudpdf_amd/csrc/rowlin2_bf16.hip
+++ b/pointcloudpdf_amd/csrc/rowlin2_bf16.hip
@@ -3,7 +3,7 @@
 namespace rl2 {
 template int try_forward_mp<2>(long, int, int, int, int, const float *const *, long, const float *const *, int, const float *const *, const float *,
                                const float *, int, float *const *, long, int, float *, hipStream_t, const float *, long, const float *, long,
-                               const float *, int, int *, long, void *);
+                               const float *, int, int *, long, void *, const PdfBnBwdPro *);
 template int try_wgrad_mp<2>(long, int, int, int, const float *const *, long, const float *, long, const float *, const float *, int,
                              float *const *, float *const *, float *, hipStream_t, const float *, long);
 template int try_wgrad_group_mp<2>(long, int, int, int, const float *const *, long, const float *const *, long, const float *const *, const float *const *, const int *,
diff --git a/pointcloudpdf_amd/csrc/rowlin2_f16.hip b/pointcloudpdf_amd/csrc/rowlin2_f16.hip
--- a/pointcloudpdf_amd/csrc/rowlin2_f16.hip
+++ b/pointcloudpdf_amd/csrc/rowlin2_f16.hip
@@ -3,7 +3,7 @@
 namespace rl2 {
 template int try_forward_mp<1>(long, int, int, int, int, const float *const *, long, const float *const *, int, const float *const *, const float *,
                                const float *, int, float *const *, long, int, float *, hipStream_t, const float *, long, const float *, long,
-                               const float *, int, int *, long, void *);
+                               const float *, int, int *, long, void *, const PdfBnBwdPro *);
 template int try_wgrad_mp<1>(long, int, int, int, const float *const *, long, const float *, long, const float *, const float *, int,
                              float *const *, float *const *, float *, hipStream_t, const float *, long);
 template int try_wgrad_group_mp<1>(long, int, int, int, const float *const *, long, const float *const *, long, const float *const *, const float *const *, const int *,
diff --git a/pointcloudpdf_amd/csrc/rowlin2_impl.h b/pointcloudpdf_amd/csrc/rowlin2_impl.h
--- a/pointcloudpdf_amd/csrc/rowlin2_impl.h
+++ b/pointcloudpdf_amd/csrc/rowlin2_impl.h
@@ -41,6 +41,7 @@
     const float *bx; long ldb; const float *bcoef; int brelu;
     const float *roww; long rws;
     unsigned long long *ho_gran; unsigned *ho_sync;
+    PdfBnBwdPro bnb;
 };
 
 constexpr int FWD_CAP = 1024;
@@ -49,8 +50,9 @@
     return (int)(b < 1 ? 1 : (b > FWD_CAP ? FWD_CAP : b));
 }
 
-template <int K, int NOB, int NIN, bool PRE, int ST, int MP>
+template <int K, int NOB, int NIN, bool PRE, int ST, int MP, int BNB = 0>
 __global__ __launch_bounds__(256) void k_fwd(FwdArgs a) {
+    static_assert(BNB == 0 || (NIN == 1 && !PRE && ST != 1), "BatchNorm-backward prologue: single input, no affine prologue");
     typedef typename Mma<MP>::frag wfrag;
     constexpr bool STATS = ST != 0;
     constexpr int NJ = K / 16;
@@ -115,9 +117,15 @@
         for (int t = threadIdx.x; t < K; t += 256) { pco[0][t] = a.scale[t]; pco[PRE && !COEF_REGS ? 1 : 0][t] = a.shift[t]; }
         __syncthreads();
     }
+    __shared__ __attribute__((aligned(16))) float bpc[BNB != 0 ? 6 : 1][BNB != 0 ? K : 1];
+    if constexpr (BNB != 0) {
+        for (int t = threadIdx.x; t < 6 * K; t += 256) { const int v = t / K, e = t % K; bpc[v][e] = v < 4 ? a.bnb.coef[t] : a.bnb.sums[t - 4 * K]; }
+        __syncthreads();
+    }
     const float relu_lo = a.relu ? 0.f : -INFINITY;
     constexpr int XB0 = NJ < 16 ? NJ : 16;
     constexpr int XB = (K == 256 && NIN == 3) ? 4 : ((ST != 0 && NOB > 1 && NIN * NOB * NJ * 4 >= 128) ? ((PRE && K == 128) ? 2 : XB0 / 2) : XB0);
+    constexpr int XBB = BNB == 0 ? 1 : ((K == 128 && NOB == 2 && ST == 2) ? 1 : (XB / 4 > 2 ? XB / 4 : 2));
     const long ntiles = (a.N + 15) / 16;
     for (long tile = (long)blockIdx.x * 4 + wave; tile < ntiles; tile += (long)gridDim.x * 4) {
         const long n = tile * 16 + li;
@@ -125,6 +133,53 @@
         f32x4 acc[NOB];
 #pragma unroll
         for (int ob = 0; ob < NOB; ++ob) acc[ob] = f32x4{0.f, 0.f, 0.f, 0.f};
+        if constexpr (BNB != 0) {
+            const long roff = (valid ? n : 0) * a.ldx + 4 * kq;
+            const float *gr = a.X[0] + roff, *br = a.bnb.bx + roff, *rr = BNB == 2 ? a.bnb.res + roff : nullptr;
+            const bool wb = valid && blockIdx.y == 0;
+#pragma unroll
+            for (int j0 = 0; j0 < NJ; j0 += XBB) {
+                f32x4 gb[XBB], bb[XBB], rb[BNB == 2 ? XBB : 1];
+#pragma unroll
+                for (int t = 0; t < XBB; ++t) {
+                    gb[t] = *reinterpret_cast<const f32x4 *>(gr + 16 * (j0 + t));
+                    bb[t] = *reinterpret_cast<const f32x4 *>(br + 16 * (j0 + t));
+                    if constexpr (BNB == 2) rb[t] = *reinterpret_cast<const f32x4 *>(rr + 16 * (j0 + t));
+                }
+                __builtin_amdgcn_sched_barrier(0);
+#pragma unroll
+                for (int t = 0; t < XBB; ++t) {
+                    const int j = j0 + t;
+                    f32x4 cf[6];
+#pragma unroll
+                    for (int v = 0; v < 6; ++v)
+                        cf[v] = *reinterpret_cast<const f32x4 *>(&bpc[v][16 * j + 4 * kq]);
+                    f32x4 x4, gm4;
+#pragma unroll
+                    for (int c = 0; c < 4; ++c) {
+                        float gm;
+                        x4[c] = pdf_bn_bwd_one(gb[t][c], bb[t][c], BNB == 2 ? rb[BNB == 2 ? t : 0][c] : 0.f, cf[0][c], cf[1][c], cf[2][c], cf[3][c], cf[4][c],
+                                               cf[5][c], a.bnb.inv_n, a.bnb.relu, &gm);
+                        gm4[c] = gm;
+                    }
+                    if (wb) {
+                        *reinterpret_cast<f32x4 *>(a.bnb.gx + roff + 16 * j) = x4;
+                        if (a.bnb.gres) *reinterpret_cast<f32x4 *>(a.bnb.gres + roff + 16 * j) = gm4;
+                    }
+                    if constexpr (MP == 0) {
+#pragma unroll
+                        for (int c = 0; c < 4; ++c)
+#pragma unroll
+                            for (int ob = 0; ob < NOB; ++ob)
+                                acc[ob] = __builtin_amdgcn_mfma_f32_16x16x4f32(Wr[0][ob][j][c], x4[c], acc[ob], 0, 0, 0);
+                    } else {
+                        const wfrag xh = Mma<MP>::cvt(x4);
+#pragma unroll
+                        for (int ob = 0; ob < NOB; ++ob) acc[ob] = Mma<MP>::mma(Wr[0][ob][j], xh, acc[ob]);
+                    }
+                }
+            }
+        } else {
 #pragma unroll
         for (int in = 0; in < NIN; ++in) {
             const float *xr = a.X[in] + (valid ? n : 0) * a.ldx + 4 * kq;
@@ -158,6 +213,7 @@
                     }
                 }
             }
+        }
         }
 #pragma unroll
         for (int ob = 0; ob < NOB; ++ob) {
@@ -415,6 +471,13 @@
     int gx = fwd_row_blocks(a.N);
     if (!stats || bst) gx = std::max(1, std::min(gx, std::max(8, total / std::max(nslabs, 1))));
     const dim3 grid((unsigned)gx, (unsigned)nslabs);
+    if constexpr (NIN == 1) {
+        if (a.bnb.bx) {
+            if (bst) { if (a.bnb.res) k_fwd<K, NOB, 1, false, 2, MP, 2><<<grid, 256, 0, s>>>(a); else k_fwd<K, NOB, 1, false, 2, MP, 1><<<grid, 256, 0, s>>>(a); }
+            else     { if (a.bnb.res) k_fwd<K, NOB, 1, false, 0, MP, 2><<<grid, 256, 0, s>>>(a); else k_fwd<K, NOB, 1, false, 0, MP, 1><<<grid, 256, 0, s>>>(a); }
+            return gx;
+        }
+    }
     if (bst) {
         k_fwd<K, NOB, NIN, false, 2, MP><<<grid, 256, 0, s>>>(a);
     } else if (NIN == 1 && stats) {
@@ -435,7 +498,13 @@
 int try_forward_mp(long n, int k, int o, int nin, int nout, const float *const *x, long ldx, const float *const *w, int transpose_w,
                    const float *const *bias, const float *scale, const float *shift, int relu, float *const *y, long ldy,
                    int accumulate, float *partial, hipStream_t s, const float *roww, long rws, const float *bx, long ldb, const float *bcoef,
-                   int brelu, int *partial_rows, long ldw, void *handoff) {
+                   int brelu, int *partial_rows, long ldw, void *handoff, const PdfBnBwdPro *bnb) {
+    if (bnb) {
+        if (nin != 1 || nout != 1 || scale || roww || (partial && !bx) || !bnb->bx || !bnb->coef || !bnb->sums || !bnb->gx) return 0;
+        if (!aligned16(bnb->bx) || !aligned16(bnb->coef) || !aligned16(bnb->sums) || !aligned16(bnb->gx)) return 0;
+        if ((bnb->res && !aligned16(bnb->res)) || (bnb->gres && !aligned16(bnb->gres))) return 0;
+        if (bnb->gx == x[0] || bnb->gres == x[0]) return 0;
+    }
     if (nin < 1 || nout < 1 || (nin > 1 && nout > 1) || nin > 3 || nout > 3) return 0;
     if (nin == 2 && (scale || bx)) return 0;
     if (partial && !bx && (nin != 1 || nout != 1)) return 0;
@@ -451,6 +520,7 @@
     a.bx = bx; a.ldb = ldb; a.bcoef = bcoef; a.brelu = brelu;
     a.ho_gran = static_cast<unsigned long long *>(handoff);
     a.ho_sync = handoff ? reinterpret_cast<unsigned *>(a.ho_gran + 2 * (size_t)o) : nullptr;
+    if (bnb) a.bnb = *bnb; else a.bnb = PdfBnBwdPro{nullptr, nullptr, nullptr, nullptr, 0.f, 0, nullptr, nullptr};
     a.wso = transpose_w ? 1 : (ldw ? ldw : k); a.wsk = transpose_w ? o : 1;
     for (int i = 0; i < 3; ++i) {
         a.X[i] = i < nin ? x[i] : nullptr;
```

Result: no change. 13.51 million, median of 2 (+0.1%).
